# willake/cpu-ray-tracer

Hardware: AMD Instinct MI355X
Metric: Mrays/sec (primary+secondary), 1280x720 64spp path trace — pipelined throughput over 878 consecutive 64-spp windows of one progressive render (single_render = one such render alone) (higher is better)
Workload: dtype f32; 1 GPU; bunny_scene.xml FileScene BVH-SAH path tracer, 1280x720, 64 spp/step (passes=1, depthLimit=5); 1 step = 64 frames = the next spp window of a progressive render; the 878 steps are one crt_render job (14 render kernel launch(es), a wavefront per (tile, 128 consecutive frames), + ordered accumulate), one sync at the end; triangles=4968, parallelism=tile-wave x1

## Files before the change

### cpu-ray-tracer_amd/__init__.py

```python
import ctypes as C
import os
import subprocess

import numpy as np

HERE = os.path.dirname(os.path.abspath(__file__))
REPO = os.path.dirname(HERE)
LIB_PATH = os.environ.get("CRT_LIB_PATH") or os.path.join(HERE, "libcrt_amd.so")

SCENE_FILE, SCENE_TLAS = 0, 1
UPDATE_TRANSFORMS, UPDATE_BOUNDS = 1, 2
ACCEL_KDTREE, ACCEL_GRID = 1, 2
KD_NODE_DTYPE = np.dtype([("aabbMin", "<f4", 3), ("left", "<i4"), ("aabbMax", "<f4", 3), ("right", "<i4"), ("splitDistance", "<f4"), ("splitAxis", "<i4"),
                          ("firstTri", "<u4"), ("triCount", "<u4")])


class CrtError(RuntimeError):
    def __init__(self, code, msg):
        super().__init__("crt error %d: %s" % (code, msg))
        self.code = code


class Config(C.Structure):
    _fields_ = [("width", C.c_int32), ("height", C.c_int32), ("depthLimit", C.c_int32), ("device", C.c_int32),
# ... 428 lines not shown

    def sample_resident_lanes(self, accel=0):
        n = C.c_uint32()
        self._ck(self.L.crt_debug_sample_resident_lanes(self.h, int(accel), C.byref(n)))
        return int(n.value)

    def _positions(self, positions, what):
        import torch
        if not isinstance(positions, torch.Tensor) or positions.device != torch.device("cuda", self.device):
            raise ValueError("%s: positions must be a torch tensor on cuda:%d" % (what, self.device))
        if positions.dtype != torch.float32 or not positions.is_contiguous() or positions.dim() < 2 or tuple(positions.shape[1:]) not in ((3, 3), (9,)):
            raise ValueError("%s: positions must be a contiguous float32 tensor of shape [triCount, 3, 3] or [triCount, 9]" % what)
        return C.c_void_p(positions.data_ptr()), C.c_uint32(positions.shape[0])

    def refit_device(self, bvh, positions, stream=None, root_box=True):
        def run(st):
            ptr, n = self._positions(positions, "refit_device")
            box = (C.c_float * 6)()
            self._ck(self.L.crt_refit_device(self.h, C.c_uint32(bvh), ptr, n, C.c_void_p(st.cuda_stream), box if root_box else None))
            return np.array(box[:], np.float32).reshape(2, 3) if root_box else None
        return self._enqueue(stream, run)

    def _transforms(self, T, what):
        import torch
        if not isinstance(T, torch.Tensor) or T.device != torch.device("cuda", self.device):
            raise ValueError("%s: the transforms must be a torch tensor on cuda:%d" % (what, self.device))
        if T.dtype != torch.float32 or not T.is_contiguous() or T.dim() < 2 or tuple(T.shape[1:]) not in ((16,), (4, 4)):
            raise ValueError("%s: the transforms must be a contiguous float32 tensor of shape [N, 16] or [N, 4, 4]" % what)
        return C.c_void_p(T.data_ptr()), C.c_uint32(T.shape[0])

    def update_transforms_device(self, T, stream=None):
        def run(st):
            ptr, n = self._transforms(T, "update_transforms_device")
            nodes = np.zeros(2 * n.value, TLAS_DTYPE)
            self._ck(self.L.crt_update_transforms_device(self.h, ptr, n, C.c_void_p(st.cuda_stream), _p(nodes)))
            return nodes
        return self._enqueue(stream, run)

    def build_grid_device(self, bvh, positions, stream=None):
        def run(st):
            ptr, n = self._positions(positions, "build_grid_device")
            self._ck(self.L.crt_build_grid_device(self.h, C.c_uint32(bvh), ptr, n, C.c_void_p(st.cuda_stream)))
        return self._enqueue(stream, run)

    def get_grid(self, bvh=0):
        res = np.zeros(3, np.int32); f = np.zeros(9, np.float32); cells, refs = C.c_uint32(), C.c_uint32()
        fp = f.ctypes.data
        self._ck(self.L.crt_get_grid(self.h, C.c_uint32(bvh), _p(res), C.c_void_p(fp), C.c_void_p(fp + 12), C.c_void_p(fp + 24), C.byref(cells), C.byref(refs), None, None))
        start = np.zeros(cells.value + 1, np.uint32); r = np.zeros(max(refs.value, 1), np.int32)
        self._ck(self.L.crt_get_grid(self.h, C.c_uint32(bvh), None, None, None, None, None, None, _p(start), _p(r)))
        return dict(resolution=res, cellSize=f[0:3].copy(), boundsMin=f[3:6].copy(), boundsMax=f[6:9].copy(), cellStart=start, refs=r[:refs.value])

    def _enqueue(self, stream, run):
        import torch
        st = stream if stream is not None else torch.cuda.current_stream(self.device)
        if st.cuda_stream != 0:
            with torch.cuda.stream(st):
                return run(st)
        side = getattr(self, "_side_stream", None)
        if side is None:
            side = self._side_stream = torch.cuda.Stream(device=self.device)
        side.wait_stream(st)
        with torch.cuda.stream(side):
            out = run(side)
        st.wait_stream(side)
        for t in (out if isinstance(out, tuple) else (out,)):
            if isinstance(t, torch.Tensor):
                t.record_stream(st)
        return out

    def counters(self):
        c = CountersS()
        self._ck(self.L.crt_get_counters(self.h, C.byref(c)))
        return {n: int(getattr(c, n)) for n, _ in c._fields_}

    def reset_counters(self):
        self._ck(self.L.crt_reset_counters(self.h))

    def timing(self):
        t = TimingS()
        self._ck(self.L.crt_get_timing(self.h, C.byref(t)))
        return dict(render_kernel_ms=t.render_kernel_ms, resolve_kernel_ms=t.resolve_kernel_ms, render_launches=t.render_launches, pool_launches=t.pool_launches, split_launches=t.split_launches)

    def tile_clocks(self, tile_count):
        a = np.zeros((tile_count, 2), np.uint64)
        self._ck(self.L.crt_get_tile_clocks(self.h, _p(a)))
        return a

    def bind_accumulator(self, device_ptr):
        self._ck(self.L.crt_bind_accumulator(self.h, C.c_void_p(device_ptr)))

    def accumulator_device_ptr(self):
        p = C.c_void_p()
        self._ck(self.L.crt_accumulator_device_ptr(self.h, C.byref(p)))
        return p.value

def hit_fields(hits):
    import torch
    i = hits.view(torch.int32)
    return dict(t=hits[:, 0], u=hits[:, 1], v=hits[:, 2], objIdx=i[:, 3], triIdx=i[:, 4], traversed=i[:, 5], tested=i[:, 6])


def hit_info_fields(info):
    import torch
    return dict(I=info[:, 0:3], material=info.view(torch.int32)[:, 3], N=info[:, 4:7], u=info[:, 7], albedo=info[:, 8:11], v=info[:, 11])


class HostScene:

    def __init__(self, xml_path, kind, base_dir=None):
        self.L = lib()
        h = C.c_void_p()
        rc = self.L.crt_host_scene_load(xml_path.encode(), int(kind), (base_dir or "").encode(), C.byref(h))
        if rc != 0:
            raise CrtError(rc, self.L.crt_host_last_error().decode())
        self.h = h
        self.kind = int(kind)

    def close(self):
        if getattr(self, "h", None):
            self.L.crt_host_scene_free(self.h)
            self.h = None

    def __del__(self):
        try:
            self.close()
        except Exception:
            pass

    def _ck(self, rc):
        if rc != 0:
            raise CrtError(rc, self.L.crt_host_last_error().decode())

    def upload(self, ctx):
        self._ck(self.L.crt_host_scene_upload(self.h, ctx.h))

    def triangle_count(self):
        return self.L.crt_host_scene_triangle_count(self.h)

    def bvh_count(self):
        return self.L.crt_host_scene_bvh_count(self.h)

    def bvh(self, i=0):
        nu, tc, md = C.c_uint32(), C.c_uint32(), C.c_uint32()
        self._ck(self.L.crt_host_scene_bvh_info(self.h, i, C.byref(nu), C.byref(tc), C.byref(md)))
        nodes = np.zeros(nu.value, NODE_DTYPE)
        idx = np.zeros(tc.value, np.uint32)
        tris = np.zeros(tc.value, TRI_DTYPE)
        self._ck(self.L.crt_host_scene_bvh_copy(self.h, i, _p(nodes), _p(idx), _p(tris)))
        return dict(nodes=nodes, triIndices=idx, tris=tris, nodesUsed=nu.value, maxDepth=md.value)

    def move_and_refit(self, i, positions):
        positions = np.ascontiguousarray(positions, np.float32)
        self._ck(self.L.crt_host_scene_bvh_move_and_refit(self.h, int(i), _p(positions), C.c_uint32(positions.shape[0])))

    def refit_device(self, ctx, i, positions, stream=None):
        def run(st):
            ptr, n = ctx._positions(positions, "refit_device")
            self._ck(self.L.crt_host_scene_bvh_refit_device(self.h, ctx.h, int(i), ptr, n, C.c_void_p(st.cuda_stream)))
        return ctx._enqueue(stream, run)

    def set_transforms_device(self, ctx, T, stream=None):
        def run(st):
            ptr, n = ctx._transforms(T, "set_transforms_device")
            if n.value != self.bvh_count():
                raise ValueError("set_transforms_device: %d transforms for %d instances" % (n.value, self.bvh_count()))
# ... 174 lines not shown
        return self.L.crt_host_renderer_spp(self.h)

    @property
    def energy(self):
        return float(self.L.crt_host_renderer_energy(self.h))

    def accumulator(self):
        p = self.L.crt_host_renderer_accumulator(self.h)
        return np.ctypeslib.as_array(p, shape=(self.H, self.W, 4)).copy()

    def screen(self):
        p = self.L.crt_host_renderer_screen(self.h)
        return np.ctypeslib.as_array(p, shape=(self.H, self.W)).copy()

    def context(self):
        return Context.borrow(self.L.crt_host_renderer_ctx(self.h), self.W, self.H)


def load_obj(path):
    L = lib()
    n = C.c_uint32()
    pp, pn, pu = C.POINTER(C.c_float)(), C.POINTER(C.c_float)(), C.POINTER(C.c_float)()
    rc = L.crt_host_obj_load(path.encode(), C.byref(n), C.byref(pp), C.byref(pn), C.byref(pu))
    if rc != 0:
        raise CrtError(rc, L.crt_host_last_error().decode())
    pos = np.ctypeslib.as_array(pp, shape=(n.value, 3)).copy()
    nrm = np.ctypeslib.as_array(pn, shape=(n.value, 3)).copy()
    uv = np.ctypeslib.as_array(pu, shape=(n.value, 2)).copy()
    for q in (pp, pn, pu):
        L.crt_host_free(C.cast(q, C.c_void_p))
    return pos, nrm, uv


def load_image(path):
    L = lib()
    w, h = C.c_int(), C.c_int()
    px = C.POINTER(C.c_uint32)()
    rc = L.crt_host_image_load(path.encode(), C.byref(w), C.byref(h), C.byref(px))
    if rc != 0:
        raise CrtError(rc, L.crt_host_last_error().decode())
    a = np.ctypeslib.as_array(px, shape=(h.value, w.value)).copy()
    L.crt_host_free(C.cast(px, C.c_void_p))
    return a


def host_math_probe(inputs):
    inputs = np.ascontiguousarray(inputs, np.float32).reshape(-1, 12)
    out = np.zeros((len(inputs), 120), np.float32)
    lib().crt_host_math_probe(inputs.ctypes.data_as(C.c_void_p), C.c_uint32(len(inputs)), out.ctypes.data_as(C.c_void_p))
    return out


def host_grid_build(positions):
    pos = np.ascontiguousarray(positions, np.float32).reshape(-1, 9)
    L = lib()
    res = np.zeros(3, np.int32); f = np.zeros(9, np.float32); refs = C.c_uint32()

    def ck(rc):
        if rc != 0:
            raise CrtError(rc, L.crt_host_last_error().decode())
    ck(L.crt_host_grid_build(_p(pos), C.c_uint32(len(pos)), _p(res), _p(f), C.byref(refs), None, None))
    start = np.zeros(int(res.prod()) + 1, np.uint32); r = np.zeros(max(refs.value, 1), np.int32)
    ck(L.crt_host_grid_build(_p(pos), C.c_uint32(len(pos)), None, None, None, _p(start), _p(r)))
    return dict(resolution=res, cellSize=f[0:3].copy(), boundsMin=f[3:6].copy(), boundsMax=f[6:9].copy(), cellStart=start, refs=r[:refs.value])


def host_vertex_dedup(v8):
    v8 = np.ascontiguousarray(v8, np.float32).reshape(-1, 8)
    idx = np.zeros(len(v8), np.uint32); uniq = np.zeros((len(v8), 8), np.float32)
    L = lib(); L.crt_host_vertex_dedup.restype = C.c_uint32
    n = L.crt_host_vertex_dedup(v8.ctypes.data_as(C.c_void_p), C.c_uint32(len(v8)), idx.ctypes.data_as(C.c_void_p), uniq.ctypes.data_as(C.c_void_p))
    return idx, uniq[:n].copy()


def spp_window(rank, frames_per_rank, first_spp=1):
    return first_spp + rank * frames_per_rank


def tile_partition(rank, world, n_tiles):
    count = (n_tiles - rank + world - 1) // world if rank < n_tiles else 0
    return rank, world, count


def reduce_accumulator(tensor, dist, dst=0):
    dist.reduce(tensor, dst=dst, op=dist.ReduceOp.SUM)
    return tensor


def allreduce_accumulator(tensor, dist):
    dist.all_reduce(tensor, op=dist.ReduceOp.SUM)
    return tensor
```

### cpu-ray-tracer_amd/csrc/abi.cpp

```cpp
#include "../../include/crt_abi.h"
#include "device/launch.h"
#include "host/grid_resolution.h"

#include <cmath>
#include <cstdarg>
#include <cstddef>
#include <cstdio>
#include <cstdlib>
#include <cstring>
#include <deque>
#include <string>
#include <algorithm>
#include <vector>
#include <chrono>

static_assert(sizeof(crt_bvh_node) == 32 && sizeof(crt_tri) == 112 && sizeof(crt_tlas_node) == 32, "reference layouts");
static_assert(sizeof(crt::NodePair) == 64 && sizeof(crt::LeafTri) == 48 && sizeof(crt::ShadeTri) == 64 && sizeof(crt::TlasNode) == 32 &&
              sizeof(crt::Instance) == 128 && sizeof(crt::Material) == 32 && offsetof(crt::Instance, T) == 64, "device layouts");
static_assert(sizeof(crt_counters) == sizeof(crt::Counters), "counter layout");
static_assert(sizeof(crt_kd_node) == 48 && sizeof(crt::KdNode) == sizeof(crt_kd_node) && sizeof(crt::AltTri) == 48, "flat KD node (uploaded as it comes), alternative accelerators' triangle record");
static_assert(offsetof(crt::PrimDev, red) == 536 && sizeof(crt::PrimDev) == 552, "PrimDev: 134 floats, then the two texel pointers");
static_assert(sizeof(crt::BlasAltDesc) == 72, "BLAS descriptor");
static_assert(sizeof(crt_shadow_ray) == 28 && sizeof(crt_ray) == 28 && sizeof(crt_hit) == 28, "query records");
static_assert(sizeof(crt_hit_info) == 48 && offsetof(crt_hit_info, material) == 12 && offsetof(crt_hit_info, N) == 16 && offsetof(crt_hit_info, albedo) == 32 && offsetof(crt_hit_info, v) == 44, "crt_hit_info: three 16-byte pieces");
static_assert(sizeof(crt::Instance) == 128 && offsetof(crt::Instance, triCount) == 112, "Instance record");

namespace {

thread_local std::string g_createError;

bool g_hooks = false;
inline const char* hook(const char* name) { return g_hooks ? getenv(name) : nullptr; }

struct EventPair { hipEvent_t a, b; int mode = -1; bool seen = false; };

}

extern "C" uint32_t crt_debug_query_grid(void)
{
    const char* e = hook("CRT_DEBUG_QUERY_GRID");
    const long k = e ? strtol(e, nullptr, 10) : 0;
    return k > 0 ? (uint32_t)(k > 0x7fffffffL ? 0x7fffffffL : k) : 0u;
}

struct crt_ctx {
    crt_config cfg{};
    std::string err;
    hipStream_t stream = nullptr;
    int tilesX = 0, tilesY = 0;
    uint32_t tileFirst = 0, tileStride = 1, tileCount = 0;
    void* dAccOwned = nullptr; void* dAcc = nullptr;
    std::vector<hipStream_t> streams; uint64_t launchSeq = 0;
    struct Region { size_t off, bytes; hipEvent_t freed; bool held = false; };
    std::deque<Region> inflight;
    char* pool = nullptr; size_t poolBytes = 0, poolHead = 0; bool poolCapped = false;
    hipEvent_t mustWait = nullptr;
    std::vector<hipEvent_t> freeEvents;
    std::vector<hipEvent_t> doneEvents;
    struct Ahead { hipEvent_t end; size_t off; const char* slab; uint64_t epoch; uint32_t sppFirst, nf, passes, used; };
    std::deque<Ahead> ahead;
    uint64_t epoch = 1;
    uint64_t tickEpoch = 0; uint32_t tickNextSpp = 0, tickPasses = 0;
    uint32_t aheadFrames = 0;
    hipStream_t aheadStream = nullptr;
    crt::Scene hScene{};
    crt::Counters* dCounters = nullptr;
    uint32_t* dQueryCursor = nullptr;
    int32_t* dInspectCounts = nullptr; void* dInspectWork = nullptr; size_t inspectCap = 0;
    uint32_t* dPixels = nullptr; float* dTileSums = nullptr;
    unsigned long long* dTileClocks = nullptr;
    std::vector<void*> sceneAllocs;
    float meshLo[3] = {0, 0, 0}, meshHi[3] = {0, 0, 0}; bool orderDirty = true;
    uint32_t* dTileOrder = nullptr;
    uint32_t* hTileOrder[2] = {nullptr, nullptr}; hipEvent_t orderCopied[2] = {nullptr, nullptr}; hipEvent_t orderReady = nullptr; int orderFlip = 0;
    bool haveScene = false;
    struct Flat { int32_t kind = 0; uint64_t leafOff = 0, tlasOff = 0, tlasPairOff = 0, instOff = 0, shadeOff = 0; uint32_t tlasNodeCount = 0, maxHeight = 0;
                  uint32_t objects = 0;
                  std::vector<uint64_t> pairBase, triBase; std::vector<uint32_t> nodesUsed, triCount; std::vector<char> geom;
                  std::vector<float> rootBox; } flat;
    char* hStage[2] = {nullptr, nullptr}; size_t stageBytes[2] = {0, 0}; hipEvent_t stageCopied[2] = {nullptr, nullptr}; int stageFlip = 0;
    hipEvent_t sceneReady = nullptr, writeFence = nullptr;
    bool havePrim = false; crt::PrimDev prim{}; uint32_t* dPrimTex = nullptr;
    int renderAccel = 0;
    crt::AltAccelDev alt{}; bool haveKd = false, haveGrid = false; std::vector<void*> altAllocs[2]; crt::AltTri* altTris = nullptr; uint32_t altTriCount = 0;
    crt::TlasAltDev blasAlt[2]{}; bool haveBlas[2] = {false, false}; std::vector<void*> blasAllocs[2];
    bool hasAlt(int kind) const { return (kind == CRT_ACCEL_KDTREE && (haveKd || haveBlas[0])) || (kind == CRT_ACCEL_GRID && (haveGrid || haveBlas[1])); }
    char* dStage = nullptr; size_t stageCap = 0;
    static constexpr int kQuerySlots = 64;
    uint32_t* dQuerySlots = nullptr;
    struct QuerySlot { hipEvent_t done = nullptr; bool pending = false; } qslot[kQuerySlots];
    int qslotNext = 0;
    struct RefitPlan { void* dPlan = nullptr; uint32_t* dLevelOff = nullptr; uint32_t levels = 0, rootCode = 0; bool built = false; };
    std::vector<RefitPlan> refitPlans; std::vector<void*> refitAllocs;
    struct Refit {
        float* dBack = nullptr; float* hBack = nullptr; hipEvent_t done = nullptr;
        void release() { if (done) (void)hipEventDestroy(done); (void)hipFree(dBack); (void)hipHostFree(hBack); *this = Refit{}; }
    } refit;
    float* dRootBox = nullptr;
    struct TlasBuild {
        char* dBuild = nullptr; char* hBack = nullptr; size_t bytes = 0;
        hipEvent_t back = nullptr, done = nullptr, t0 = nullptr, t1 = nullptr; bool timed = false;
        void release() { for (hipEvent_t e : {back, done, t0, t1}) if (e) (void)hipEventDestroy(e); (void)hipFree(dBuild); (void)hipHostFree(hBack); *this = TlasBuild{}; }
    } tlasBuild;
    struct GridBuild {
        crt::GridBuildState* dState = nullptr; crt::GridBuildState* hState = nullptr;
        unsigned long long* dChunks = nullptr; uint32_t* dCursor = nullptr; int32_t* dUnsorted = nullptr; size_t cursorCap = 0, unsortedCap = 0;
        hipEvent_t back = nullptr, done = nullptr, t0 = nullptr, t1 = nullptr; bool built = false, timed = false; uint32_t blocks = 0;
        double waitMs[2] = {0, 0};
        void release() { for (hipEvent_t e : {back, done, t0, t1}) if (e) (void)hipEventDestroy(e); for (void* p : {(void*)dState, (void*)dChunks, (void*)dCursor, (void*)dUnsorted}) (void)hipFree(p); (void)hipHostFree(hState); *this = GridBuild{}; }
    } gridBuild;
    struct Retired { std::vector<void*> ptrs; void* pinned = nullptr; hipEvent_t unread = nullptr; };
    std::deque<Retired> retired; std::vector<hipEvent_t> retiredEvents;
    uint32_t gridRefCount = 0;
    struct BlasGrid { std::vector<crt::BlasAltDesc> desc; std::vector<uint32_t> cells, refs; std::vector<uint8_t> current; bool held = false; } blasGrid;
    hipEvent_t altReady = nullptr;
    static constexpr int kLatStages = 4;
    double tuneMs[kLatStages + 1] = {}; int tuneCount[kLatStages + 1] = {};
    hipEvent_t lastRenderEnd = nullptr;
    int latStage = 0;
    int latBest = 0;
    bool latDone = false;
    bool latConfirming = false; std::vector<int> latQueue;
    bool latWarm = false;
    uint32_t latSlots = 0;
    bool latProbed = false;
    std::vector<uint8_t> latL[kLatStages + 1];
    std::vector<uint32_t> latCost[kLatStages + 1];
    uint32_t* dTileCost = nullptr; uint32_t* hTileCost = nullptr; hipEvent_t costCopied = nullptr; bool costPending = false; int costStage = 0;
    uint32_t* dBlockDesc = nullptr; uint32_t* hBlockDesc = nullptr; uint32_t nBlocks = 0, descCap = 0; hipEvent_t descReady = nullptr;
    uint32_t* dJobCost = nullptr; uint32_t* hJobCost = nullptr; hipEvent_t jobCostCopied = nullptr; bool jobCostPending = false, jobCostValid = false;
    uint32_t recWaves = 0, recResident = 0, recWindows = 0; bool recPool = false;
    double poolWindowTicks = 0;
    std::vector<uint32_t> jobCost;
    std::vector<uint32_t> jobOrder;
    uint32_t* dJobDesc = nullptr; uint32_t* hJobDesc = nullptr; uint32_t jobDescCap = 0, jobBlocks = 0, jobHead = 0; hipEvent_t jobDescReady = nullptr;
    uint32_t planWindows = 0, planFrames = 0; bool planPool = false, planValid = false;
    double jobTrialMs[2] = {0, 0};
    uint32_t jobWaveOff = 0, jobWaveBlocks = 0, jobLongFrames = 0, jobLongWaves = 0, lastLongWaves = 0;
    std::vector<hipEvent_t> splitEvents;
    size_t splitSeq = 0; uint32_t splitLaunches = 0;
    uint64_t poolMinWaves = 65000;
    bool usePool = true;
    uint32_t ldsBytes = 0;
    std::vector<EventPair> evPool; size_t evUsedRender = 0, evUsedAcc = 0;
    std::deque<EventPair> evRender, evAcc;
    double foldedRenderMs = 0, foldedAccMs = 0; uint32_t foldedLaunches = 0, poolLaunches = 0;

    int fail(int code, const char* fmt, ...)
    {
        char buf[1024];
        va_list ap; va_start(ap, fmt); vsnprintf(buf, sizeof(buf), fmt, ap); va_end(ap);
        err = buf; return code;
    }
    int hip(hipError_t e, const char* what)
    {
        if (e == hipSuccess) return 0;
        return fail(CRT_ERR_DEVICE, "%s: %s", what, hipGetErrorString(e));
// ... 15 lines not shown
            for (void* p : r.ptrs) (void)hipFree(p);
            if (r.pinned) (void)hipHostFree(r.pinned);
            retiredEvents.push_back(r.unread); retired.pop_front();
        }
    }
    void freeScene()
    {
        for (void* p : sceneAllocs) (void)hipFree(p);
        sceneAllocs.clear(); haveScene = false; dRootBox = nullptr;
        for (void* p : refitAllocs) (void)hipFree(p);
        refitAllocs.clear(); refitPlans.clear();
        if (dPrimTex) { (void)hipFree(dPrimTex); dPrimTex = nullptr; }
        havePrim = false;
        freeAlt();
    }
};

#define HIPCK(ctx, call) do { hipError_t e_ = (call); if (e_ != hipSuccess) return (ctx)->hip(e_, #call); } while (0)

namespace {

template <class T>
int upload(crt_ctx* c, const std::vector<T>& v, const T** out)
{
    *out = nullptr;
    if (v.empty()) return 0;
    void* d = nullptr;
    HIPCK(c, hipMalloc(&d, v.size() * sizeof(T)));
    c->sceneAllocs.push_back(d);
    HIPCK(c, hipMemcpyAsync(d, v.data(), v.size() * sizeof(T), hipMemcpyHostToDevice, c->stream));
    HIPCK(c, hipStreamSynchronize(c->stream));
    *out = reinterpret_cast<const T*>(d);
    return 0;
}

template <class T>
int upload_array(crt_ctx* c, std::vector<void*>& allocs, const void* src, size_t bytes, const T** out)
{
    *out = nullptr; if (!bytes) return 0;
    void* d = nullptr; HIPCK(c, hipMalloc(&d, bytes)); allocs.push_back(d);
    HIPCK(c, hipMemcpy(d, src, bytes, hipMemcpyHostToDevice)); *out = static_cast<const T*>(d); return 0;
}

int bvh_height(crt_ctx* c, const crt_bvh& b, uint32_t* heightOut)
{
    std::vector<std::pair<uint32_t, uint32_t>> st; st.push_back({0u, 0u});
    uint32_t h = 0; size_t visited = 0;
    while (!st.empty()) {
        auto [n, d] = st.back(); st.pop_back();
        if (++visited > (size_t)b.nodesUsed) return c->fail(CRT_ERR_INVALID, "BVH node graph is not a tree");
        const crt_bvh_node& nd = b.nodes[n];
        if (nd.triCount > 0) { if (d > h) h = d; continue; }
        if (nd.leftFirst == 0 || nd.leftFirst + 1 >= b.nodesUsed) return c->fail(CRT_ERR_INVALID, "BVH child index out of range (node %u)", n);
        st.push_back({nd.leftFirst, d + 1}); st.push_back({nd.leftFirst + 1, d + 1});
    }
    *heightOut = h;
    return 0;
}

int wait_queries(crt_ctx* c)
{
    for (auto& q : c->qslot) if (q.pending) { HIPCK(c, hipEventSynchronize(q.done)); q.pending = false; }
    return 0;
}

hipError_t ensure_event(hipEvent_t* e, unsigned flags = hipEventDisableTiming) { return *e ? hipSuccess : hipEventCreateWithFlags(e, flags); }

int drain_all(crt_ctx* c)
{
    for (auto st : c->streams) HIPCK(c, hipStreamSynchronize(st));
    if (c->aheadStream) HIPCK(c, hipStreamSynchronize(c->aheadStream));
    HIPCK(c, hipStreamSynchronize(c->stream));
    return wait_queries(c);
}

}

extern "C" {

int crt_abi_version(void) { return CRT_ABI_VERSION; }

void crt_debug_enable_hooks(int on) { g_hooks = on != 0; }

int crt_device_count(void)
{
    int n = 0;
    if (hipGetDeviceCount(&n) != hipSuccess) return 0;
    return n;
}

const char* crt_last_error(crt_ctx* ctx) { return ctx ? ctx->err.c_str() : g_createError.c_str(); }

int crt_create(crt_ctx** out, const crt_config* cfg)
{
    if (!out || !cfg) { g_createError = "crt_create: null argument"; return CRT_ERR_INVALID; }
    *out = nullptr;
    setenv("GPU_MAX_HW_QUEUES", "16", 0);
    if (cfg->width < 16 || cfg->height < 16) { g_createError = "crt_create: width and height must be at least one 16x16 tile"; return CRT_ERR_INVALID; }
    int ndev = 0;
    hipError_t e = hipGetDeviceCount(&ndev);
    if (e != hipSuccess || ndev == 0) {
        g_createError = "crt_create: no HIP device visible (this library has no CPU path)";
        return CRT_ERR_NO_DEVICE;
    }
    if (cfg->device < 0 || cfg->device >= ndev) { g_createError = "crt_create: device ordinal out of range"; return CRT_ERR_INVALID; }
    crt_ctx* c = new crt_ctx();
    c->cfg = *cfg;
    if (const char* k = hook("CRT_RENDER_KERNEL")) {
        c->usePool = strcmp(k, "tiles") != 0;
        if (!strcmp(k, "pool_always")) c->poolMinWaves = 0;
    }
    if (c->cfg.depthLimit < 0) c->cfg.depthLimit = 5;
    if (c->cfg.depthLimit > 5) { g_createError = "crt_create: depthLimit > 5 unsupported (throughput stack holds 5 factors; reference default is 5)"; delete c; return CRT_ERR_UNSUPPORTED; }
    if (c->cfg.maxFramesPerLaunch <= 0) c->cfg.maxFramesPerLaunch = c->cfg.collectStats ? 64 : 4096;
    if (c->cfg.maxFramesPerLaunch > 64) c->cfg.maxFramesPerLaunch = c->cfg.maxFramesPerLaunch / 64 * 64;
    if (c->cfg.renderStreams < 0) c->cfg.renderStreams = 0;
    c->tilesX = cfg->width / 16; c->tilesY = cfg->height / 16;
    const int tiles = c->tilesX * c->tilesY;
    int first = cfg->tileFirst, stride = cfg->tileStride <= 0 ? 1 : cfg->tileStride, count = cfg->tileCount;
    if (count < 0) { first = 0; stride = 1; count = tiles; }
    if (first < 0 || (count > 0 && (long long)first + (long long)(count - 1) * stride >= tiles)) {
        g_createError = "crt_create: tile range exceeds the image"; delete c; return CRT_ERR_INVALID;
    }
    c->tileFirst = (uint32_t)first; c->tileStride = (uint32_t)stride; c->tileCount = (uint32_t)count;

    auto bail = [&](hipError_t he, const char* what) {
        g_createError = std::string("crt_create: ") + what + ": " + hipGetErrorString(he);
        crt_destroy(c); return CRT_ERR_DEVICE;
    };
    if ((e = hipSetDevice(cfg->device)) != hipSuccess) return bail(e, "hipSetDevice");
    if ((e = hipStreamCreateWithFlags(&c->stream, hipStreamNonBlocking)) != hipSuccess) return bail(e, "hipStreamCreate");
    const size_t px = (size_t)cfg->width * cfg->height;
    if ((e = hipMalloc(&c->dAccOwned, px * 16)) != hipSuccess) return bail(e, "hipMalloc(accumulator)");
    c->dAcc = c->dAccOwned;
    if ((e = hipMemsetAsync(c->dAcc, 0, px * 16, c->stream)) != hipSuccess) return bail(e, "hipMemset(accumulator)");
    if ((e = hipMalloc((void**)&c->dPixels, px * 4)) != hipSuccess) return bail(e, "hipMalloc(pixels)");
    if ((e = hipMemsetAsync(c->dPixels, 0, px * 4, c->stream)) != hipSuccess) return bail(e, "hipMemset(pixels)");
    if ((e = hipMalloc((void**)&c->dTileSums, (size_t)tiles * 4)) != hipSuccess) return bail(e, "hipMalloc(tileSums)");
    if ((e = hipMemsetAsync(c->dTileSums, 0, (size_t)tiles * 4, c->stream)) != hipSuccess) return bail(e, "hipMemset(tileSums)");
    if ((e = hipMalloc((void**)&c->dCounters, sizeof(crt::Counters))) != hipSuccess) return bail(e, "hipMalloc(counters)");
    if ((e = hipMemsetAsync(c->dCounters, 0, sizeof(crt::Counters), c->stream)) != hipSuccess) return bail(e, "hipMemset(counters)");
    if ((e = hipMalloc((void**)&c->dQueryCursor, 64)) != hipSuccess) return bail(e, "hipMalloc(query cursor)");
    if ((e = hipMalloc((void**)&c->dQuerySlots, crt_ctx::kQuerySlots * 64)) != hipSuccess) return bail(e, "hipMalloc(query cursor slots)");
    if (c->cfg.collectStats && count > 0) {
        if ((e = hipMalloc((void**)&c->dTileClocks, (size_t)count * 144)) != hipSuccess) return bail(e, "hipMalloc(tileClocks)");
        if ((e = hipMemsetAsync(c->dTileClocks, 0, (size_t)count * 144, c->stream)) != hipSuccess) return bail(e, "hipMemset(tileClocks)");
    }
    memset(&c->hScene, 0, sizeof(c->hScene));
    const float aspect = (float)cfg->width / (float)cfg->height;
    crt::Scene& s = c->hScene;
    s.camPos[0] = 0; s.camPos[1] = 0; s.camPos[2] = -2;
    s.topLeft[0] = -aspect; s.topLeft[1] = 1; s.topLeft[2] = 0;
    s.topRight[0] = aspect; s.topRight[1] = 1; s.topRight[2] = 0;
    s.bottomLeft[0] = -aspect; s.bottomLeft[1] = -1; s.bottomLeft[2] = 0;
    s.W = cfg->width; s.H = cfg->height; s.invW = 1.0f / cfg->width; s.invH = 1.0f / cfg->height;
    s.depthLimit = c->cfg.depthLimit;
    crt::set_primary(s);
    if ((e = hipStreamSynchronize(c->stream)) != hipSuccess) return bail(e, "hipStreamSynchronize");
    *out = c;
    return CRT_OK;
}

void crt_destroy(crt_ctx* c)
{
    if (!c) return;
    (void)hipSetDevice(c->cfg.device);
    for (auto st : c->streams) (void)hipStreamSynchronize(st);
    if (c->aheadStream) (void)hipStreamSynchronize(c->aheadStream);
    if (c->stream) (void)hipStreamSynchronize(c->stream);
    for (auto& q : c->qslot) if (q.done) { if (q.pending) (void)hipEventSynchronize(q.done); (void)hipEventDestroy(q.done); }
    if (c->dQuerySlots) (void)hipFree(c->dQuerySlots);
    if (c->altReady) (void)hipEventDestroy(c->altReady);
    if (c->writeFence) (void)hipEventDestroy(c->writeFence);
    c->refit.release(); c->tlasBuild.release();
    c->freeScene();
    c->gridBuild.release();
    for (hipEvent_t e : c->retiredEvents) (void)hipEventDestroy(e);
    for (auto& a : c->ahead) (void)hipEventDestroy(a.end);
    if (c->aheadStream) (void)hipStreamDestroy(c->aheadStream);
    for (auto& ev : c->evPool) { (void)hipEventDestroy(ev.a); (void)hipEventDestroy(ev.b); }
    for (auto& ev : c->evRender) { (void)hipEventDestroy(ev.a); (void)hipEventDestroy(ev.b); }
    for (auto& ev : c->evAcc) { (void)hipEventDestroy(ev.a); (void)hipEventDestroy(ev.b); }
    if (c->dAccOwned) (void)hipFree(c->dAccOwned);
    for (auto st : c->streams) { (void)hipStreamSynchronize(st); (void)hipStreamDestroy(st); }
    for (auto& r : c->inflight) (void)hipEventDestroy(r.freed);
    for (auto e : c->freeEvents) (void)hipEventDestroy(e);
    if (c->mustWait) (void)hipEventDestroy(c->mustWait);
    if (c->pool) (void)hipFree(c->pool);
    for (auto e : c->doneEvents) (void)hipEventDestroy(e);
    if (c->dPixels) (void)hipFree(c->dPixels);
    if (c->dTileSums) (void)hipFree(c->dTileSums);
    if (c->dCounters) (void)hipFree(c->dCounters);
    if (c->dQueryCursor) (void)hipFree(c->dQueryCursor);
    if (c->dInspectCounts) (void)hipFree(c->dInspectCounts);
    if (c->dInspectWork) (void)hipFree(c->dInspectWork);
    if (c->dTileClocks) (void)hipFree(c->dTileClocks);
    if (c->dTileOrder) (void)hipFree(c->dTileOrder);
    if (c->dTileCost) (void)hipFree(c->dTileCost);
    if (c->dJobCost) (void)hipFree(c->dJobCost);
    if (c->dJobDesc) (void)hipFree(c->dJobDesc);
    if (c->hJobDesc) (void)hipHostFree(c->hJobDesc);
    if (c->jobDescReady) (void)hipEventDestroy(c->jobDescReady);
    if (c->hJobCost) (void)hipHostFree(c->hJobCost);
    if (c->jobCostCopied) (void)hipEventDestroy(c->jobCostCopied);
    for (auto e : c->splitEvents) (void)hipEventDestroy(e);
    if (c->hTileCost) (void)hipHostFree(c->hTileCost);
    if (c->costCopied) (void)hipEventDestroy(c->costCopied);
    if (c->dBlockDesc) (void)hipFree(c->dBlockDesc);
    if (c->hBlockDesc) (void)hipHostFree(c->hBlockDesc);
    if (c->descReady) (void)hipEventDestroy(c->descReady);
    if (c->dStage) (void)hipFree(c->dStage);
    for (int k = 0; k < 2; k++) { if (c->hTileOrder[k]) (void)hipHostFree(c->hTileOrder[k]); if (c->orderCopied[k]) (void)hipEventDestroy(c->orderCopied[k]); }
    for (int k = 0; k < 2; k++) { if (c->hStage[k]) (void)hipHostFree(c->hStage[k]); if (c->stageCopied[k]) (void)hipEventDestroy(c->stageCopied[k]); }
    if (c->stream) (void)hipStreamDestroy(c->stream);
    delete c;
}

int crt_upload_scene(crt_ctx* c, const crt_scene_desc* sd)
{
    if (!c || !sd) return CRT_ERR_INVALID;
    c->epoch++;
    HIPCK(c, hipSetDevice(c->cfg.device));
    if (sd->kind != CRT_SCENE_FILE && sd->kind != CRT_SCENE_TLAS) return c->fail(CRT_ERR_INVALID, "unknown scene kind %d", sd->kind);
    if (!sd->bvhs || sd->bvhCount == 0) return c->fail(CRT_ERR_INVALID, "scene has no acceleration structure");
    if (sd->kind == CRT_SCENE_FILE && sd->bvhCount != 1) return c->fail(CRT_ERR_INVALID, "CRT_SCENE_FILE takes exactly one BVH (FileScene::acc)");
    if (sd->kind == CRT_SCENE_TLAS && (sd->bvhCount > 256 || !sd->tlasNodes || sd->tlasNodeCount < 2 * sd->bvhCount))
        return c->fail(CRT_ERR_INVALID, "TLAS scene needs <= 256 BLAS (tlas_bvh.cpp:21) and 2*blasCount TLAS nodes");
    if (sd->textureCount == 0 || !sd->textures) return c->fail(CRT_ERR_INVALID, "floor and skydome textures are required");
    if (sd->floorTexture < 0 || sd->floorTexture >= (int)sd->textureCount || sd->skyTexture < 0 || sd->skyTexture >= (int)sd->textureCount)
        return c->fail(CRT_ERR_INVALID, "floor/sky texture index out of range");
    for (uint32_t i = 0; i < sd->textureCount; i++)
        if (!sd->textures[i].pixels || sd->textures[i].width <= 0 || sd->textures[i].height <= 0) return c->fail(CRT_ERR_INVALID, "texture %u is empty", i);
    if (sd->materialCount > 0 && !sd->materials) return c->fail(CRT_ERR_INVALID, "materialCount is %u but materials is NULL", sd->materialCount);
    for (uint32_t i = 0; i < sd->materialCount; i++)
        if (sd->materials[i].texture >= (int)sd->textureCount) return c->fail(CRT_ERR_INVALID, "material %u: texture index out of range", i);
    if (sd->kind == CRT_SCENE_FILE) {
        if (!sd->objMatIdx || sd->objCount == 0) return c->fail(CRT_ERR_INVALID, "CRT_SCENE_FILE needs objMatIdx");
        for (uint32_t i = 0; i < sd->objCount; i++)
            if (sd->objMatIdx[i] < 0 || sd->objMatIdx[i] >= (int)sd->materialCount) return c->fail(CRT_ERR_INVALID, "objMatIdx entry out of range");
    }

    uint64_t nPairs = 0, nTris = 0;
    uint32_t maxHeight = 0;
    for (uint32_t bi = 0; bi < sd->bvhCount; bi++) {
        const crt_bvh& b = sd->bvhs[bi];
        if (!b.nodes || !b.triangles || !b.triangleIndices || b.nodesUsed == 0 || b.triCount == 0) return c->fail(CRT_ERR_INVALID, "BVH %u is empty", bi);
        if ((b.nodesUsed & 1u) == 0) return c->fail(CRT_ERR_INVALID, "BVH %u: nodesUsed must be odd (root + child pairs)", bi);
        if (sd->kind == CRT_SCENE_TLAS && (b.matIdx < 0 || b.matIdx >= (int)sd->materialCount)) return c->fail(CRT_ERR_INVALID, "BLAS %u: matIdx out of range", bi);
        if (sd->kind == CRT_SCENE_TLAS && b.objIdx != (int)bi + 2)
            return c->fail(CRT_ERR_INVALID, "BLAS %u: objIdx must be %u (TLASFileScene numbers objects from 2, tlas_file_scene.cpp:13,51-53)", bi, bi + 2);
        uint32_t h = 0; int r = bvh_height(c, b, &h); if (r) return r;
        if (h > maxHeight) maxHeight = h;
        nPairs += b.nodesUsed / 2; nTris += b.triCount;
    }
    const uint64_t pairBytes = nPairs ? nPairs * 64 : 64;
    const uint64_t leafOffB = pairBytes, leafBytes = (nTris + 1) * 48;
    const uint64_t tlasOffB = (leafOffB + leafBytes + 63) & ~63ull;
    const uint64_t tlasBytes = (sd->kind == CRT_SCENE_TLAS) ? (uint64_t)sd->tlasNodeCount * 32 : 0;
    const uint64_t tlasPairOffB = (tlasOffB + tlasBytes + 63) & ~63ull;
    const uint64_t tlasPairBytes = (sd->kind == CRT_SCENE_TLAS) ? (uint64_t)sd->tlasNodeCount * 32 : 0;
    const uint64_t instOffB = (tlasPairOffB + tlasPairBytes + 127) & ~127ull;
    const uint64_t instBytes = (sd->kind == CRT_SCENE_TLAS) ? (uint64_t)sd->bvhCount * 128 : 0;
    const uint64_t shadeOffB = (instOffB + instBytes + 63) & ~63ull;
    const uint64_t total = shadeOffB + nTris * 64;
    if (total >= crt::kMaxGeomBytes) return c->fail(CRT_ERR_UNSUPPORTED, "scene geometry needs %llu bytes; this build addresses 4 GiB", (unsigned long long)total);
    if (sd->kind == CRT_SCENE_TLAS && sd->tlasNodeCount > 0x7fffu) return c->fail(CRT_ERR_UNSUPPORTED, "TLAS node index exceeds 15 bits");

    std::vector<char> geom((size_t)total, 0);
    crt::NodePair* pairs = reinterpret_cast<crt::NodePair*>(geom.data());
    crt::LeafTri* leaf = reinterpret_cast<crt::LeafTri*>(geom.data() + leafOffB);
    crt::TlasNode* tlas = reinterpret_cast<crt::TlasNode*>(geom.data() + tlasOffB);
    crt::NodePair* tlasPairs = reinterpret_cast<crt::NodePair*>(geom.data() + tlasPairOffB);
    bool ref16ok = nPairs <= crt::kRef16MaxIndex && nTris < crt::kRef16MaxIndex;
    crt::Instance* inst = reinterpret_cast<crt::Instance*>(geom.data() + instOffB);
    crt::ShadeTri* shade = reinterpret_cast<crt::ShadeTri*>(geom.data() + shadeOffB);

    uint64_t pairBase = 0, triBase = 0; uint32_t rootRef0 = 0, rootRef0_16 = 0;
    for (uint32_t bi = 0; bi < sd->bvhCount; bi++) {
        const crt_bvh& b = sd->bvhs[bi];
        auto ref_of = [&](uint32_t n, uint32_t* ref) -> int {
            const crt_bvh_node& nd = b.nodes[n];
            if (nd.triCount > 0) {
                if ((uint64_t)nd.leftFirst + nd.triCount > b.triCount) return c->fail(CRT_ERR_INVALID, "leaf range out of bounds (BVH %u node %u)", bi, n);
                *ref = (uint32_t)((leafOffB + (triBase + nd.leftFirst) * 48) >> 4);
            } else {
                if ((nd.leftFirst & 1u) == 0) return c->fail(CRT_ERR_INVALID, "interior node %u: children must be allocated pairwise starting at an odd index", n);
                *ref = crt::kRefInterior | (uint32_t)(((pairBase + ((nd.leftFirst - 1u) >> 1)) * 64) >> 4);
            }
            return 0;
        };
        auto ref16_of = [&](uint32_t n) -> uint32_t {
            const crt_bvh_node& nd = b.nodes[n];
            if (nd.triCount > 0) return (uint32_t)((triBase + nd.leftFirst + 1) & crt::kRef16IndexMask);
            return crt::kRef16Interior | (uint32_t)((pairBase + ((nd.leftFirst - 1u) >> 1)) & crt::kRef16IndexMask);
        };
// ... 72 lines not shown
        }
        tlasRoot = tlas[0].ref; tlasRoot16 = tlas[0].ref16;
    }
    std::vector<uint32_t> texOff(sd->textureCount); uint64_t texels = 0;
    for (uint32_t i = 0; i < sd->textureCount; i++) {
        texOff[i] = (uint32_t)texels;
        texels += (uint64_t)sd->textures[i].width * sd->textures[i].height;
        if (texels > 0xffffffffull) return c->fail(CRT_ERR_UNSUPPORTED, "texture pool exceeds 2^32 texels");
    }
    auto bindTex = [&](crt::Material& m, int t) {
        if (t < 0) { m.texOffset = 0; m.texW = 0; m.texH = 0; }
        else { m.texOffset = texOff[t]; m.texW = sd->textures[t].width; m.texH = sd->textures[t].height; }
    };
    std::vector<crt::Material> mats(2 + sd->materialCount);
    memset(mats.data(), 0, mats.size() * sizeof(crt::Material));
    bindTex(mats[0], -1);
    bindTex(mats[1], sd->floorTexture);
    for (uint32_t i = 0; i < sd->materialCount; i++) {
        crt::Material& m = mats[2 + i];
        m.reflectivity = sd->materials[i].reflectivity; m.refractivity = sd->materials[i].refractivity;
        memcpy(m.absorption, sd->materials[i].absorption, 12);
        bindTex(m, sd->materials[i].texture);
    }

    { const int r = drain_all(c); if (r) return r; }
    c->freeScene();
    uint32_t* dTexels = nullptr;
    HIPCK(c, hipMalloc((void**)&dTexels, (size_t)texels * 4)); c->sceneAllocs.push_back(dTexels);
    for (uint32_t i = 0; i < sd->textureCount; i++)
        HIPCK(c, hipMemcpyAsync(dTexels + texOff[i], sd->textures[i].pixels, (size_t)sd->textures[i].width * sd->textures[i].height * 4, hipMemcpyHostToDevice, c->stream));
    HIPCK(c, hipStreamSynchronize(c->stream));

    crt::Scene& s = c->hScene;
    s.kind = sd->kind;
    memcpy(s.lightInvT, sd->lightInvT, 48);
    s.lightNrm[0] = -sd->lightT[1]; s.lightNrm[1] = -sd->lightT[5]; s.lightNrm[2] = -sd->lightT[9];
    s.lightSize = sd->lightSize;
    {
        const float* m = sd->lightT;
        const float ax = -0.5f, ay = 0.0f, az = -0.5f, bx = 0.5f, by = 0.0f, bz = 0.5f;
        const float c1[3] = {m[0] * ax + m[1] * ay + m[2] * az + m[3] * 1.0f, m[4] * ax + m[5] * ay + m[6] * az + m[7] * 1.0f, m[8] * ax + m[9] * ay + m[10] * az + m[11] * 1.0f};
        const float c2[3] = {m[0] * bx + m[1] * by + m[2] * bz + m[3] * 1.0f, m[4] * bx + m[5] * by + m[6] * bz + m[7] * 1.0f, m[8] * bx + m[9] * by + m[10] * bz + m[11] * 1.0f};
        s.lightPos[0] = (c1[0] + c2[0]) * 0.5f - 0.0f; s.lightPos[1] = (c1[1] + c2[1]) * 0.5f - 0.01f; s.lightPos[2] = (c1[2] + c2[2]) * 0.5f - 0.0f;
    }
    memcpy(s.floorN, sd->floorN, 12); s.floorD = sd->floorD; s.floorInvto = sd->floorInvto;
    {
        const float* m = sd->lightInvT;
        s.lightAxis = (m[0] == 1.0f && m[1] == 0.0f && m[2] == 0.0f && m[4] == 0.0f && m[5] == 1.0f && m[6] == 0.0f && m[8] == 0.0f && m[9] == 0.0f && m[10] == 1.0f) ? 1u : 0u;
        s.floorAxisY = (sd->floorN[0] == 0.0f && sd->floorN[1] == 1.0f && sd->floorN[2] == 0.0f) ? 1u : 0u;
        if (hook("CRT_DEBUG_GENERAL_PRIMS")) s.lightAxis = s.floorAxisY = 0u;
    }
    s.floorMat = mats[1];
    s.skyOffset = texOff[sd->skyTexture]; s.skyW = sd->textures[sd->skyTexture].width; s.skyH = sd->textures[sd->skyTexture].height;
    s.texels = dTexels;
    int r;
    const char* dGeom = nullptr;
    if ((r = upload(c, geom, &dGeom))) return r;
    s.geom = dGeom;
    s.tlasOff = (uint32_t)tlasOffB; s.instOff = (uint32_t)instOffB; s.shadeOff = (uint32_t)shadeOffB;
    s.leafOff = (uint32_t)leafOffB; s.tlasPairOff = (uint32_t)tlasPairOffB;
    s.rootRef16 = (sd->kind == CRT_SCENE_TLAS) ? tlasRoot16 : rootRef0_16;
    s.ref16ok = (ref16ok && !hook("CRT_DEBUG_NO_REF16")) ? 1u : 0u;
    if ((r = upload(c, mats, &s.mats))) return r;
    if (sd->kind == CRT_SCENE_TLAS) {
        std::vector<float> boxes;
        for (uint32_t bi = 0; bi < sd->bvhCount; bi++) { const crt_bvh_node& n0 = sd->bvhs[bi].nodes[0]; boxes.insert(boxes.end(), n0.aabbMin, n0.aabbMin + 3); boxes.insert(boxes.end(), n0.aabbMax, n0.aabbMax + 3); }
        const float* d = nullptr;
        if ((r = upload(c, boxes, &d))) return r;
        c->dRootBox = const_cast<float*>(d);
    }
    s.rootRef = (sd->kind == CRT_SCENE_TLAS) ? tlasRoot : rootRef0;
    s.bvhStack = maxHeight > 0 ? maxHeight : 1;
    s.rootIsPair = 0; memset(s.rootPair, 0, sizeof(s.rootPair));
    if (sd->kind == CRT_SCENE_TLAS) {
        if ((tlasRoot & 0xC0000000u) == crt::kRefTlasInterior) {
            memcpy(s.rootPair, &tlas[tlasRoot & 0x7fffu], 32); memcpy(s.rootPair + 8, &tlas[(tlasRoot >> 15) & 0x7fffu], 32);
            s.rootIsPair = 1;
        }
    } else if (rootRef0 & crt::kRefInterior) {
        memcpy(s.rootPair, geom.data() + ((size_t)(rootRef0 & crt::kRefOffsetMask) << 4), 64);
        s.rootIsPair = 1;
    }
    if (hook("CRT_DEBUG_NO_ROOTPAIR")) s.rootIsPair = 0;
    crt::set_primary(s);
    s.stackDepth = s.bvhStack + ((sd->kind == CRT_SCENE_TLAS) ? tlasHeight + 1 : 0);
    c->ldsBytes = s.stackDepth * 64u * 4u; c->latSlots = 0;
    if (const char* e = hook("CRT_DEBUG_EXTRA_LDS")) c->ldsBytes += (uint32_t)atoi(e);
    if (c->ldsBytes + 15u * 256u > 64u * 1024u) return c->fail(CRT_ERR_UNSUPPORTED, "tree height %u (+TLAS %u) needs %u bytes of LDS traversal stack per wave (> 64 KiB)", maxHeight, tlasHeight, c->ldsBytes);
    {
        float lo[3] = {1e30f, 1e30f, 1e30f}, hi[3] = {-1e30f, -1e30f, -1e30f};
        auto grow = [&](const float* mn, const float* mx) { for (int k = 0; k < 3; k++) { if (mn[k] < lo[k]) lo[k] = mn[k]; if (mx[k] > hi[k]) hi[k] = mx[k]; } };
        if (sd->kind == CRT_SCENE_TLAS) grow(sd->tlasNodes[0].aabbMin, sd->tlasNodes[0].aabbMax);
        else grow(sd->bvhs[0].nodes[0].aabbMin, sd->bvhs[0].nodes[0].aabbMax);
        memcpy(c->meshLo, lo, 12); memcpy(c->meshHi, hi, 12); c->orderDirty = true;
    }
    {
        crt_ctx::Flat& f = c->flat;
        f.kind = sd->kind; f.leafOff = leafOffB; f.tlasOff = tlasOffB; f.tlasPairOff = tlasPairOffB; f.instOff = instOffB; f.shadeOff = shadeOffB;
        f.tlasNodeCount = (sd->kind == CRT_SCENE_TLAS) ? sd->tlasNodeCount : 0; f.maxHeight = maxHeight;
        f.objects = (sd->kind == CRT_SCENE_TLAS) ? sd->bvhCount : sd->objCount;
        f.pairBase.clear(); f.triBase.clear(); f.nodesUsed.clear(); f.triCount.clear(); f.rootBox.clear();
        for (uint32_t bi = 0; bi < sd->bvhCount; bi++) { const crt_bvh_node& r = sd->bvhs[bi].nodes[0]; f.rootBox.insert(f.rootBox.end(), r.aabbMin, r.aabbMin + 3); f.rootBox.insert(f.rootBox.end(), r.aabbMax, r.aabbMax + 3); }
        uint64_t pb = 0, tb = 0;
        for (uint32_t bi = 0; bi < sd->bvhCount; bi++) { f.pairBase.push_back(pb); f.triBase.push_back(tb); f.nodesUsed.push_back(sd->bvhs[bi].nodesUsed); f.triCount.push_back(sd->bvhs[bi].triCount); pb += sd->bvhs[bi].nodesUsed / 2; tb += sd->bvhs[bi].triCount; }
        f.geom.swap(geom);
    }
    c->haveScene = true;
    return CRT_OK;
}


static int order_behind_ahead(crt_ctx* c)
{
    for (const auto& a : c->ahead) HIPCK(c, hipStreamWaitEvent(c->stream, a.end, 0));
    return 0;
}

static int order_behind_queries(crt_ctx* c)
{
    for (auto& q : c->qslot) {
        if (!q.pending) continue;
        const hipError_t e = hipEventQuery(q.done);
        if (e == hipSuccess) { q.pending = false; continue; }
        if (e != hipErrorNotReady) return c->hip(e, "hipEventQuery(query)");
        HIPCK(c, hipStreamWaitEvent(c->stream, q.done, 0));
    }
    return 0;
}

static int wait_scene(crt_ctx* c, hipStream_t st)
{
    if (c->sceneReady) HIPCK(c, hipStreamWaitEvent(st, c->sceneReady, 0));
    return 0;
}

static int order_behind_readers(crt_ctx* c)
{
    int r;
    if ((r = order_behind_ahead(c)) || (r = order_behind_queries(c))) return r;
    c->epoch++;
    return 0;
}

static int begin_scene_write(crt_ctx* c, hipStream_t st)
{
    const int r = order_behind_readers(c);
    if (r || st == c->stream) return r;
    HIPCK(c, ensure_event(&c->writeFence));
    HIPCK(c, hipEventRecord(c->writeFence, c->stream));
    HIPCK(c, hipStreamWaitEvent(st, c->writeFence, 0));
    return wait_scene(c, st);
}

static int publish_scene_write(crt_ctx* c, hipStream_t st, hipEvent_t done)
{
    c->sceneReady = done;
    if (st != c->stream) HIPCK(c, hipStreamWaitEvent(c->stream, done, 0));
    return 0;
}

static int end_scene_write(crt_ctx* c, hipStream_t st, hipEvent_t done)
{
    HIPCK(c, hipEventRecord(done, st));
    return publish_scene_write(c, st, done);
}

static int flatten_tlas(crt_ctx* c, const crt_tlas_node* nodes, uint32_t count, uint32_t bvhCount, crt::TlasNode* tlas, crt::NodePair* tlasPairs, uint32_t* heightOut)
{
    uint32_t nTlasPairs = 0;
    for (uint32_t i = 0; i < count; i++) {
        const crt_tlas_node& nd = nodes[i];
        memcpy(tlas[i].lo, nd.aabbMin, 12); memcpy(tlas[i].hi, nd.aabbMax, 12);
        tlas[i].ref = nd.leftRight ? (crt::kRefTlasInterior | (nd.leftRight & 0x7fffu) | (((nd.leftRight >> 16) & 0x7fffu) << 15))
                                   : (crt::kRefTlasLeaf | (nd.BLAS & 0xffffu));
        tlas[i].ref16 = nd.leftRight ? (crt::kRef16TlasBit | nTlasPairs++) : (crt::kRef16TlasLeaf | (nd.BLAS & crt::kRef16IndexMask));
    }
    std::vector<std::pair<uint32_t, uint32_t>> st; st.push_back({0u, 0u}); size_t visited = 0; uint32_t height = 0;
    while (!st.empty()) {
        auto [n, d] = st.back(); st.pop_back();
        if (++visited > (size_t)count) return c->fail(CRT_ERR_INVALID, "TLAS node graph is not a tree");
        const crt_tlas_node& nd = nodes[n];
        if (nd.leftRight == 0) { if (nd.BLAS >= bvhCount) return c->fail(CRT_ERR_INVALID, "TLAS leaf references BLAS %u", nd.BLAS); if (d > height) height = d; continue; }
        const uint32_t l = nd.leftRight & 0xffffu, r = nd.leftRight >> 16;
        if (l >= count || r >= count) return c->fail(CRT_ERR_INVALID, "TLAS child index out of range");
        st.push_back({l, d + 1}); st.push_back({r, d + 1});
    }
    for (uint32_t i = 0; i < count; i++) {
        const crt_tlas_node& nd = nodes[i];
        if (nd.leftRight == 0) continue;
        crt::NodePair& p = tlasPairs[tlas[i].ref16 & crt::kRef16IndexMask];
        memcpy(&p.c[0], &tlas[nd.leftRight & 0xffffu], 32); memcpy(&p.c[1], &tlas[nd.leftRight >> 16], 32);
    }
    *heightOut = height;
    return 0;
}

static void set_root(crt_ctx* c, int kind, const float* lo, const float* hi)
{
    crt::Scene& s = c->hScene; const crt_ctx::Flat& f = c->flat;
    s.rootIsPair = 0; memset(s.rootPair, 0, sizeof(s.rootPair));
    if (kind == CRT_SCENE_TLAS) {
        const crt::TlasNode* tlas = reinterpret_cast<const crt::TlasNode*>(f.geom.data() + f.tlasOff);
        const uint32_t root = tlas[0].ref;
        s.rootRef = root; s.rootRef16 = tlas[0].ref16;
        if ((root & 0xC0000000u) == crt::kRefTlasInterior) { memcpy(s.rootPair, &tlas[root & 0x7fffu], 32); memcpy(s.rootPair + 8, &tlas[(root >> 15) & 0x7fffu], 32); s.rootIsPair = 1; }
    } else if (s.rootRef & crt::kRefInterior) {
        memcpy(s.rootPair, f.geom.data() + ((size_t)(s.rootRef & crt::kRefOffsetMask) << 4), 64);
        s.rootIsPair = 1;
    }
    if (hook("CRT_DEBUG_NO_ROOTPAIR")) s.rootIsPair = 0;
    crt::set_primary(s);
    memcpy(c->meshLo, lo, 12); memcpy(c->meshHi, hi, 12); c->orderDirty = true;
}

static int check_tlas_height(crt_ctx* c, uint32_t tlasHeight)
{
    if ((c->hScene.bvhStack + tlasHeight + 1) * 64u * 4u + 15u * 256u > 64u * 1024u)
        return c->fail(CRT_ERR_UNSUPPORTED, "TLAS height %u needs %u bytes of LDS traversal stack per wave (> 64 KiB)", tlasHeight, (c->hScene.bvhStack + tlasHeight + 1) * 256u);
    return 0;
}

static void adopt_tlas(crt_ctx* c, uint32_t tlasHeight, const float* lo, const float* hi)
{
    crt::Scene& s = c->hScene;
    s.stackDepth = s.bvhStack + tlasHeight + 1;
    c->ldsBytes = s.stackDepth * 64u * 4u; c->latSlots = 0;
    set_root(c, CRT_SCENE_TLAS, lo, hi);
}

static void drop_blas_sets(crt_ctx* c)
{
    for (int k = 0; k < 2; k++) if (c->haveBlas[k]) { c->haveBlas[k] = false; if (c->renderAccel == k + 1) c->renderAccel = 0; }
}

int crt_update_scene(crt_ctx* c, const crt_scene_desc* sd, uint32_t what)
{
    if (!c || !sd) return CRT_ERR_INVALID;
    if (!c->haveScene) return c->fail(CRT_ERR_STATE, "crt_update_scene before crt_upload_scene");
    crt_ctx::Flat& f = c->flat;
    if (sd->kind != f.kind || sd->bvhCount != f.nodesUsed.size() || !sd->bvhs) return c->fail(CRT_ERR_INVALID, "crt_update_scene: scene kind / BVH count differ from the uploaded scene");
    if ((what & ~(uint32_t)(CRT_UPDATE_TRANSFORMS | CRT_UPDATE_BOUNDS)) || what == 0) return c->fail(CRT_ERR_INVALID, "crt_update_scene: unknown update flags");
    if ((what & CRT_UPDATE_TRANSFORMS) && f.kind != CRT_SCENE_TLAS) return c->fail(CRT_ERR_INVALID, "CRT_UPDATE_TRANSFORMS applies to two-level scenes (a FileScene bakes its transforms into the triangles)");
    HIPCK(c, hipSetDevice(c->cfg.device));
    for (uint32_t bi = 0; bi < sd->bvhCount; bi++)
        if (sd->bvhs[bi].nodesUsed != f.nodesUsed[bi] || sd->bvhs[bi].triCount != f.triCount[bi] || !sd->bvhs[bi].nodes || !sd->bvhs[bi].triangles || !sd->bvhs[bi].triangleIndices)
            return c->fail(CRT_ERR_INVALID, "crt_update_scene: BVH %u changed its topology (node / triangle count); upload the scene again", bi);
    if (f.kind == CRT_SCENE_TLAS && (!sd->tlasNodes || sd->tlasNodeCount != f.tlasNodeCount))
        return c->fail(CRT_ERR_INVALID, "crt_update_scene: a two-level scene needs the node array of the TLASBVH::Build that followed the change (tlasNodes, %u nodes as uploaded)", f.tlasNodeCount);
    if (what & CRT_UPDATE_BOUNDS) {
        const crt::LeafTri* leaf = reinterpret_cast<const crt::LeafTri*>(f.geom.data() + f.leafOff);
        for (uint32_t bi = 0; bi < sd->bvhCount; bi++) {
            const crt_bvh& b = sd->bvhs[bi];
            for (uint32_t j = 0; j < b.triCount; j++) {
                const uint32_t ti = b.triangleIndices[j];
                if (ti >= b.triCount) return c->fail(CRT_ERR_INVALID, "BVH %u: triangleIndices[%u] out of range", bi, j);
                if (leaf[f.triBase[bi] + j].shadeIdx != (uint32_t)(f.triBase[bi] + ti)) return c->fail(CRT_ERR_INVALID, "BVH %u: triangleIndices changed; Refit keeps the leaf order — upload the scene again", bi);
            }
        }
    }
    uint32_t tlasHeight = 0;
    std::vector<char> tlasImage;
    if (f.kind == CRT_SCENE_TLAS) {
        tlasImage.assign((size_t)(f.instOff - f.tlasOff), 0);
        int r = flatten_tlas(c, sd->tlasNodes, sd->tlasNodeCount, sd->bvhCount, reinterpret_cast<crt::TlasNode*>(tlasImage.data()),
                             reinterpret_cast<crt::NodePair*>(tlasImage.data() + (f.tlasPairOff - f.tlasOff)), &tlasHeight);
        if (r || (r = check_tlas_height(c, tlasHeight))) return r;
    }
    size_t lo = SIZE_MAX, hi = 0;
    auto touch = [&](size_t a, size_t b) { if (a < lo) lo = a; if (b > hi) hi = b; };
    if (what & CRT_UPDATE_BOUNDS) {
        crt::NodePair* pairs = reinterpret_cast<crt::NodePair*>(f.geom.data());
        crt::LeafTri* leaf = reinterpret_cast<crt::LeafTri*>(f.geom.data() + f.leafOff);
        for (uint32_t bi = 0; bi < sd->bvhCount; bi++) {
            const crt_bvh& b = sd->bvhs[bi];
            for (uint32_t n = 1; n + 1 < b.nodesUsed; n += 2) {
                crt::NodePair& p = pairs[f.pairBase[bi] + ((n - 1) >> 1)];
                for (int k = 0; k < 2; k++) { memcpy(p.c[k].lo, b.nodes[n + k].aabbMin, 12); memcpy(p.c[k].hi, b.nodes[n + k].aabbMax, 12); }
            }
            for (uint32_t j = 0; j < b.triCount; j++) {
                const crt_tri& t = b.triangles[b.triangleIndices[j]];
                crt::LeafTri& lt = leaf[f.triBase[bi] + j];
                for (int k = 0; k < 3; k++) { lt.v0[k] = t.vertex0[k]; lt.e1[k] = t.vertex1[k] - t.vertex0[k]; lt.e2[k] = t.vertex2[k] - t.vertex0[k]; }
            }
        }
        touch(0, (size_t)f.tlasOff);
        for (uint32_t bi = 0; bi < sd->bvhCount; bi++) { memcpy(&f.rootBox[6 * bi], sd->bvhs[bi].nodes[0].aabbMin, 12); memcpy(&f.rootBox[6 * bi + 3], sd->bvhs[bi].nodes[0].aabbMax, 12); }
    }
    if (f.kind == CRT_SCENE_TLAS) {
        if (what & CRT_UPDATE_TRANSFORMS) {
            crt::Instance* inst = reinterpret_cast<crt::Instance*>(f.geom.data() + f.instOff);
            for (uint32_t bi = 0; bi < sd->bvhCount; bi++) { memcpy(inst[bi].invT, sd->bvhs[bi].invT, 48); memcpy(inst[bi].T, sd->bvhs[bi].T, 48); }
        }
        memcpy(f.geom.data() + f.tlasOff, tlasImage.data(), tlasImage.size());
        touch((size_t)f.tlasOff, (size_t)f.shadeOff);
    }
    if (lo >= hi) return CRT_OK;
    const int k = c->stageFlip ^= 1;
    const size_t boxBytes = ((what & CRT_UPDATE_BOUNDS) && c->dRootBox) ? f.rootBox.size() * 4u : 0u;
    const size_t geomBytes = hi - lo, bytes = geomBytes + boxBytes;
    if (c->stageBytes[k] < bytes) {
        if (c->hStage[k]) { HIPCK(c, hipEventSynchronize(c->stageCopied[k])); HIPCK(c, hipHostFree(c->hStage[k])); c->hStage[k] = nullptr; }
        HIPCK(c, hipHostMalloc((void**)&c->hStage[k], bytes, hipHostMallocDefault)); c->stageBytes[k] = bytes;
        HIPCK(c, ensure_event(&c->stageCopied[k]));
    } else HIPCK(c, hipEventSynchronize(c->stageCopied[k]));
    memcpy(c->hStage[k], f.geom.data() + lo, geomBytes);
    if (boxBytes) memcpy(c->hStage[k] + geomBytes, f.rootBox.data(), boxBytes);
    { const int r = begin_scene_write(c, c->stream); if (r) return r; }
    if (what & CRT_UPDATE_BOUNDS) {
        std::fill(c->blasGrid.current.begin(), c->blasGrid.current.end(), (uint8_t)0);
        drop_blas_sets(c);
    }
    HIPCK(c, hipMemcpyAsync(const_cast<char*>(c->hScene.geom) + lo, c->hStage[k], geomBytes, hipMemcpyHostToDevice, c->stream));
    if (boxBytes) HIPCK(c, hipMemcpyAsync(c->dRootBox, c->hStage[k] + geomBytes, boxBytes, hipMemcpyHostToDevice, c->stream));
    { const int r = end_scene_write(c, c->stream, c->stageCopied[k]); if (r) return r; }
    if (f.kind == CRT_SCENE_TLAS) adopt_tlas(c, tlasHeight, sd->tlasNodes[0].aabbMin, sd->tlasNodes[0].aabbMax);
    else set_root(c, f.kind, sd->bvhs[0].nodes[0].aabbMin, sd->bvhs[0].nodes[0].aabbMax);
    return CRT_OK;
}

int crt_set_camera(crt_ctx* c, const float camPos[3], const float tl[3], const float tr[3], const float bl[3])
{
    if (!c || !camPos || !tl || !tr || !bl) return CRT_ERR_INVALID;
    HIPCK(c, hipSetDevice(c->cfg.device));
    crt::Scene& s = c->hScene;
    if (!memcmp(s.camPos, camPos, 12) && !memcmp(s.topLeft, tl, 12) && !memcmp(s.topRight, tr, 12) && !memcmp(s.bottomLeft, bl, 12)) return CRT_OK;
    memcpy(s.camPos, camPos, 12); memcpy(s.topLeft, tl, 12); memcpy(s.topRight, tr, 12); memcpy(s.bottomLeft, bl, 12);
    crt::set_primary(s);
    c->orderDirty = true; c->epoch++;
    return CRT_OK;
}

static int upload_tile_order(crt_ctx* c, const std::vector<uint32_t>& order)
{
    if (!c->dTileOrder) HIPCK(c, hipMalloc((void**)&c->dTileOrder, (size_t)c->tileCount * 4));
    { const int r = order_behind_ahead(c); if (r) return r; }
    const int k = c->orderFlip ^= 1;
    if (!c->hTileOrder[k]) {
        HIPCK(c, hipHostMalloc((void**)&c->hTileOrder[k], (size_t)c->tileCount * 4, hipHostMallocDefault));
        HIPCK(c, ensure_event(&c->orderCopied[k]));
    } else HIPCK(c, hipEventSynchronize(c->orderCopied[k]));
    memcpy(c->hTileOrder[k], order.data(), order.size() * 4);
    HIPCK(c, hipMemcpyAsync(c->dTileOrder, c->hTileOrder[k], order.size() * 4, hipMemcpyHostToDevice, c->stream));
    HIPCK(c, hipEventRecord(c->orderCopied[k], c->stream));
    c->orderReady = c->orderCopied[k];
    return 0;
}

static int update_tile_order(crt_ctx* c)
{
    if (!c->orderDirty || c->tileCount == 0) return 0;
    const crt::Scene& s = c->hScene;
    double R[3], Dn[3], N[3];
    for (int k = 0; k < 3; k++) { R[k] = (double)s.topRight[k] - s.topLeft[k]; Dn[k] = (double)s.bottomLeft[k] - s.topLeft[k]; }
    N[0] = R[1] * Dn[2] - R[2] * Dn[1]; N[1] = R[2] * Dn[0] - R[0] * Dn[2]; N[2] = R[0] * Dn[1] - R[1] * Dn[0];
    const double rr = R[0] * R[0] + R[1] * R[1] + R[2] * R[2], dd = Dn[0] * Dn[0] + Dn[1] * Dn[1] + Dn[2] * Dn[2];
    double E[3]; for (int k = 0; k < 3; k++) E[k] = (double)s.topLeft[k] - s.camPos[k];
    const double num = E[0] * N[0] + E[1] * N[1] + E[2] * N[2];
    auto rect_of = [&](const float* P8, int r[4]) -> bool {
        double u0 = 1e30, u1 = -1e30, v0 = 1e30, v1 = -1e30;
        for (int i = 0; i < 8; i++) {
            const float* P = P8 + 3 * i;
            double d[3] = {P[0] - s.camPos[0], P[1] - s.camPos[1], P[2] - s.camPos[2]};
            const double den = d[0] * N[0] + d[1] * N[1] + d[2] * N[2];
            const double t = den != 0 ? num / den : -1;
            if (!(t > 0) || rr == 0 || dd == 0) return false;
            double Q[3]; for (int k = 0; k < 3; k++) Q[k] = s.camPos[k] + t * d[k] - s.topLeft[k];
            const double u = (Q[0] * R[0] + Q[1] * R[1] + Q[2] * R[2]) / rr, v = (Q[0] * Dn[0] + Q[1] * Dn[1] + Q[2] * Dn[2]) / dd;
            if (u < u0) u0 = u; if (u > u1) u1 = u; if (v < v0) v0 = v; if (v > v1) v1 = v;
        }
        r[0] = (int)floor(u0 * c->cfg.width / 16.0) - 1; r[1] = (int)floor(u1 * c->cfg.width / 16.0) + 1;
        r[2] = (int)floor(v0 * c->cfg.height / 16.0) - 1; r[3] = (int)floor(v1 * c->cfg.height / 16.0) + 1;
        return true;
    };
    float world[24];
    for (int i = 0; i < 8; i++) { world[3 * i] = (i & 1) ? c->meshHi[0] : c->meshLo[0]; world[3 * i + 1] = (i & 2) ? c->meshHi[1] : c->meshLo[1]; world[3 * i + 2] = (i & 4) ? c->meshHi[2] : c->meshLo[2]; }
    int wr[4] = {0, c->tilesX - 1, 0, c->tilesY - 1};
    (void)rect_of(world, wr);
    std::vector<uint32_t> first, second, rest;
    for (uint32_t i = 0; i < c->tileCount; i++) {
        const uint32_t tile = c->tileFirst + i * c->tileStride;
        const int tx = (int)(tile % (uint32_t)c->tilesX), ty = (int)(tile / (uint32_t)c->tilesX);
        const bool inRect = tx >= wr[0] && tx <= wr[1] && ty >= wr[2] && ty <= wr[3];
        if (inRect) first.push_back(i); else rest.push_back(i);
    }
    for (int k = 0; k <= crt_ctx::kLatStages; k++) { c->tuneCount[k] = 0; c->tuneMs[k] = 0; }
    c->latStage = 0; c->latBest = 0; c->latDone = false; c->latWarm = false; c->latConfirming = false; c->latQueue.clear(); c->costPending = false; c->latProbed = false;
    first.insert(first.end(), rest.begin(), rest.end());
    c->jobCostValid = false; c->jobCostPending = false; c->planValid = false;
    { const int r = upload_tile_order(c, first); if (r) return r; }
    c->orderDirty = false;
    return 0;
}

static size_t sample_bytes_per_window(const crt_ctx* c, uint32_t passes) { return (size_t)c->tileCount * 256u * 64u * passes * 16u; }
static size_t window_bytes(const crt_ctx* c, uint32_t passes) { return sample_bytes_per_window(c, passes) + (c->usePool ? crt_pool_scratch_bytes_per_window(c->tileCount) : 0); }

static uint32_t block_desc(uint32_t tile, uint32_t laneBase, uint32_t lanes, uint32_t window) { uint32_t lg = 0; while ((1u << lg) < lanes) lg++; return tile | (laneBase << 16) | (lg << 22) | (window << 25); }
static const uint32_t kLatLanes[7] = {64u, 32u, 16u, 8u, 4u, 2u, 1u};
static const double kLatG[7] = {1.0, 0.93, 0.88, 0.79, 0.69, 0.57, 0.48};
static int lat_index(uint32_t L) { int k = 0; while (k < 6 && kLatLanes[k] != L) k++; return k; }

static uint8_t next_lanes(uint8_t lanes, uint32_t cost, double T)
{
    int k = lat_index(lanes); const double unit = (double)cost / kLatG[k];
    while (k < 6 && unit * kLatG[k] > T) k++;
    while (k > 0 && unit * kLatG[k - 1] <= 0.9 * T) k--;
    return (uint8_t)kLatLanes[k];
}
extern "C" int crt_debug_next_lanes(const uint8_t* lanes, const uint32_t* cost, uint32_t n, double T, uint8_t* out)
{
    if (!lanes || !cost || !out) return CRT_ERR_INVALID;
    for (uint32_t i = 0; i < n; i++) { if (lanes[i] == 0 || lanes[i] > 64 || (64 % lanes[i]) != 0) return CRT_ERR_INVALID; out[i] = next_lanes(lanes[i], cost[i], T); }
    return CRT_OK;
}

static double solve_block_table(const std::vector<uint8_t>& lanes, const std::vector<uint32_t>& cost, double budget, std::vector<uint8_t>& out)
{
    const size_t n = cost.size();
    double topUnit = 0; for (size_t i = 0; i < n; i++) topUnit = std::max(topUnit, (double)cost[i] / kLatG[lat_index(lanes[i])]);
    out.assign(n, 64);
    if (topUnit <= 0) return 0;
    auto waves = [&](double T) { double w = 0; for (size_t i = 0; i < n; i++) w += 64.0 / next_lanes(lanes[i], cost[i], T); return w; };
    double lo = kLatG[6] * topUnit, hi = topUnit;
    if (waves(lo) > budget) { for (int it = 0; it < 14; it++) { const double mid = 0.5 * (lo + hi); if (waves(mid) <= budget) hi = mid; else lo = mid; } lo = hi; }
    for (size_t i = 0; i < n; i++) out[i] = next_lanes(lanes[i], cost[i], lo);
    return lo;
}
extern "C" int crt_debug_solve_block_table(const uint8_t* lanes, const uint32_t* cost, uint32_t n, double budget, uint8_t* out, double* T)
{
    if (!lanes || !cost || !out) return CRT_ERR_INVALID;
    for (uint32_t i = 0; i < n; i++) if (lanes[i] == 0 || lanes[i] > 64 || (64 % lanes[i]) != 0) return CRT_ERR_INVALID;
    std::vector<uint8_t> L; const double t = solve_block_table(std::vector<uint8_t>(lanes, lanes + n), std::vector<uint32_t>(cost, cost + n), budget, L);
    if (n) memcpy(out, L.data(), n);
    if (T) *T = t;
    return CRT_OK;
}
static double lat_budget(crt_ctx* c)
{
    if (!c->latSlots) c->latSlots = crt_render_resident_waves(c->cfg.device, c->hScene.kind, c->ldsBytes);
    double share = 0.98;
    if (const char* e = hook("CRT_LAT_BUDGET")) { const double v = atof(e); if (v > 0) share = v; }
    return share * (double)c->latSlots;
}

static int upload_block_table(crt_ctx* c, const std::vector<uint8_t>& lanes, const std::vector<uint32_t>& cost)
{
    const uint32_t n = c->tileCount;
    std::vector<uint32_t> order(n);
    for (uint32_t i = 0; i < n; i++) order[i] = i;
    std::stable_sort(order.begin(), order.end(), [&](uint32_t a, uint32_t b) { return cost[a] > cost[b]; });
    std::vector<uint32_t> table; table.reserve((size_t)n * 2);
    for (uint32_t r = 0; r < n; r++) {
        const uint32_t tl = order[r], L = lanes[tl];
        for (uint32_t base = 0; base < 64u; base += L) table.push_back(block_desc(tl, base, L, 0u));
    }
    if (table.size() > 0x7fffffffull) return c->fail(CRT_ERR_INVALID, "block table too large");
    if (hook("CRT_LAT_VERBOSE")) fprintf(stderr, "[crt] latency table: %zu wavefronts for %u tiles (slowest tile of the base stage %.2f ms)\n", table.size(), n, n ? cost[order[0]] * 1e-5 : 0.0);
    if (c->descCap < table.size()) {
        if (c->dBlockDesc) (void)hipFree(c->dBlockDesc);
        if (c->hBlockDesc) (void)hipHostFree(c->hBlockDesc);
        c->dBlockDesc = nullptr; c->hBlockDesc = nullptr; c->descCap = 0;
        const size_t cap = table.size() + table.size() / 2;
        HIPCK(c, hipMalloc((void**)&c->dBlockDesc, cap * 4));
        HIPCK(c, hipHostMalloc((void**)&c->hBlockDesc, cap * 4, hipHostMallocDefault));
        c->descCap = (uint32_t)cap;
    } else if (c->descReady) HIPCK(c, hipEventSynchronize(c->descReady));
    HIPCK(c, ensure_event(&c->descReady));
    memcpy(c->hBlockDesc, table.data(), table.size() * 4);
    { const int r = order_behind_ahead(c); if (r) return r; }
    HIPCK(c, hipMemcpyAsync(c->dBlockDesc, c->hBlockDesc, table.size() * 4, hipMemcpyHostToDevice, c->stream));
    HIPCK(c, hipEventRecord(c->descReady, c->stream));
    c->nBlocks = (uint32_t)table.size();
    return 0;
// ... 392 lines not shown
        c->evRender.back().mode = c->latDone ? -1 : stage;
        if (L.wantCost && !c->latDone) c->costStage = stage;
    }
    if (L.wantCost) {
        if (!c->dTileCost) {
            HIPCK(c, hipMalloc((void**)&c->dTileCost, (size_t)c->tileCount * 4));
            HIPCK(c, hipHostMalloc((void**)&c->hTileCost, (size_t)c->tileCount * 4, hipHostMallocDefault));
            HIPCK(c, ensure_event(&c->costCopied));
        }
        else HIPCK(c, hipStreamWaitEvent(L.st, c->costCopied, 0));
        HIPCK(c, hipMemsetAsync(c->dTileCost, 0, (size_t)c->tileCount * 4, L.st));
    }
    return 0;
}

static int planner_prepare(crt_ctx* c, Launch& L)
{
    int r;
    if (L.nf > 64u && !c->cfg.collectStats) {
        if (c->jobCostPending && hipEventQuery(c->jobCostCopied) == hipSuccess) { c->jobCostPending = false; if ((r = adopt_job_costs(c))) return r; HIPCK(c, hipStreamWaitEvent(L.st, c->orderReady, 0)); }
        L.wantJobCost = !c->jobCostValid && !c->jobCostPending && L.nf >= 128u;
        if (L.wantJobCost) {
            if (!c->dJobCost) {
                HIPCK(c, hipMalloc((void**)&c->dJobCost, job_cost_bytes(c)));
                HIPCK(c, hipHostMalloc((void**)&c->hJobCost, job_cost_bytes(c), hipHostMallocDefault));
                HIPCK(c, ensure_event(&c->jobCostCopied));
            } else HIPCK(c, hipStreamWaitEvent(L.st, c->jobCostCopied, 0));
            HIPCK(c, hipMemsetAsync(c->dJobCost, 0, job_cost_bytes(c), L.st));
        }
    }
    const uint64_t minWaves = c->poolMinWaves != 65000u ? c->poolMinWaves : (c->jobCostValid ? 43000u : 65000u);
    L.pool = c->usePool && c->hScene.ref16ok && (uint64_t)c->tileCount * L.windows >= minWaves && (c->poolMinWaves == 0 || L.nf > 64u);
    if (L.nf > 64u && c->jobCostValid) {
        if ((r = install_job_plan(c, L.windows, L.nf, L.pool))) return r;
        int use = 1;
        if ((c->jobBlocks || c->jobLongWaves) && !hook("CRT_PLAN_NO_TRIAL")) {
            if (c->jobTrialMs[1] > 0 && c->jobTrialMs[0] > 0) use = c->jobTrialMs[1] <= c->jobTrialMs[0] ? 1 : 0;
            else if (c->jobTrialMs[1] > 0 && c->jobTrialMs[0] == 0) use = 0;
            c->evRender.back().mode = 100 + use;
        }
        if (use) { L.head = c->jobHead; L.jobBlocks = c->jobBlocks; if (L.pool && c->jobLongWaves) { L.waveTab = c->dJobDesc + c->jobWaveOff; L.waveBlocks = c->jobWaveBlocks; L.longFrames = c->jobLongFrames; L.longWaves = c->jobLongWaves; } }
    }
    if (L.pool) if (const uint32_t S = crt_pool_streams(L.nf); const uint32_t n = forced_wave_frames(S)) {
        L.waveFrames = n; L.waveTab = nullptr; L.waveBlocks = 0;
        L.longWaves = n > S ? (c->tileCount - L.head) * (L.nf / n + ((L.nf % n) > S ? 1u : 0u)) : 0u;
    }
    if (L.jobBlocks || L.waveTab) HIPCK(c, hipStreamWaitEvent(L.st, c->jobDescReady, 0));
    if (L.wantJobCost) {
        L.jobClk = reinterpret_cast<unsigned long long*>(reinterpret_cast<char*>(c->dJobCost) + job_cost_clk_offset(c));
        c->recPool = L.pool; c->recWindows = L.windows;
        const uint32_t perWave = L.pool ? std::max(crt_pool_streams(L.nf), L.waveFrames) : 64u;
        c->recWaves = L.pool ? c->tileCount * ((L.nf + perWave - 1u) / perWave) : c->tileCount * L.windows;
        c->recResident = L.pool ? 4096u : 5120u;
    }
    return 0;
}

static hipError_t launch_render_kernels(crt_ctx* c, const Launch& L)
{
    hipStream_t st = L.st;
    hipError_t le = hipSuccess;
    auto join = [&](hipStream_t other) -> hipError_t {
        if (other == st) return hipSuccess;
        hipError_t e = hipSuccess;
        if (c->splitEvents.size() < 32) { hipEvent_t ne; e = hipEventCreateWithFlags(&ne, hipEventDisableTiming); if (e == hipSuccess) c->splitEvents.push_back(ne); }
        if (e == hipSuccess) { hipEvent_t je = c->splitEvents[c->splitSeq++ % c->splitEvents.size()]; e = hipEventRecord(je, other); if (e == hipSuccess) e = hipStreamWaitEvent(st, je, 0); }
        return e;
    };
    auto launch_table = [&](const uint32_t* desc, uint32_t nBlocks, uint32_t* cost) -> hipError_t {
        return crt_launch_render(&c->hScene, L.slab, c->dCounters, c->dTileClocks, c->dTileOrder, c->tileFirst, c->tileStride, c->tileCount, (uint32_t)c->tilesX,
                                 L.sppFirst, L.nf, L.passes, c->ldsBytes, 0, desc, nBlocks, cost, 0u, nullptr, st);
    };
    if (L.pool) {
        void* scratch = (char*)L.slab + (size_t)L.windows * sample_bytes_per_window(c, L.passes);
        hipStream_t st2 = st;
        if (L.jobBlocks) {
            le = launch_table(c->dJobDesc, L.jobBlocks, nullptr);
            st2 = c->streams[(size_t)(c->launchSeq++ % c->streams.size())];
            if (le == hipSuccess && st2 != st) le = hipStreamWaitEvent(st2, L.ev.a, 0);
        }
        if (le == hipSuccess)
            le = crt_launch_render_pool(&c->hScene, L.slab, scratch, c->dCounters, c->dTileClocks, c->dTileOrder, c->tileFirst, c->tileStride, c->tileCount, (uint32_t)c->tilesX,
                                        L.sppFirst, L.nf, L.passes, c->cfg.collectStats, L.jobBlocks ? L.head : 0u, L.waveFrames, L.waveTab, L.waveBlocks, L.longFrames,
                                        L.wantJobCost ? c->dJobCost : nullptr, L.jobClk, st2);
        if (le == hipSuccess) c->lastLongWaves = L.longWaves;
        if (L.jobBlocks && le == hipSuccess) le = join(st2);
    } else if (L.jobBlocks) {
        le = launch_table(c->dJobDesc, L.jobBlocks, nullptr);
    } else if (L.blockDesc && L.nBlocks) {
        le = launch_table(L.blockDesc, L.nBlocks, L.wantCost ? c->dTileCost : nullptr);
    } else {
        le = crt_launch_render(&c->hScene, L.slab, c->dCounters, c->dTileClocks, c->dTileOrder, c->tileFirst, c->tileStride, c->tileCount, (uint32_t)c->tilesX,
                               L.sppFirst, L.nf, L.passes, c->ldsBytes, c->cfg.collectStats, nullptr, 0u,
                               L.wantCost ? c->dTileCost : (L.wantJobCost ? c->dJobCost : nullptr), 0u, L.jobClk, st);
    }
    if (L.jobBlocks && le == hipSuccess) c->splitLaunches++;
    return le;
}

static int probe_tile_costs(crt_ctx* c, hipStream_t st)
{
    const uint32_t n = c->tileCount;
    if (!c->dTileCost) {
        HIPCK(c, hipMalloc((void**)&c->dTileCost, (size_t)n * 4));
        HIPCK(c, hipHostMalloc((void**)&c->hTileCost, (size_t)n * 4, hipHostMallocDefault));
        HIPCK(c, ensure_event(&c->costCopied));
    } else HIPCK(c, hipEventSynchronize(c->costCopied));
    const auto tp0 = std::chrono::steady_clock::now();
    HIPCK(c, crt_launch_probe(&c->hScene, c->tileFirst, c->tileStride, n, (uint32_t)c->tilesX, c->dTileCost, st));
    HIPCK(c, hipMemcpyAsync(c->hTileCost, c->dTileCost, (size_t)n * 4, hipMemcpyDeviceToHost, st));
    HIPCK(c, hipEventRecord(c->costCopied, st));
    HIPCK(c, hipStreamSynchronize(st));
    const auto tp1 = std::chrono::steady_clock::now();
    std::vector<uint32_t>& est = c->latCost[0]; est.assign(c->hTileCost, c->hTileCost + n);
    for (uint32_t i = 0; i < n; i++) est[i] += 18u * crt_probe_paths();
    std::vector<uint8_t>& L = c->latL[0]; L.assign(n, 64);
    solve_block_table(std::vector<uint8_t>(n, 64), est, lat_budget(c), L);
    c->latProbed = true;
    bool any = false; for (uint32_t i = 0; i < n; i++) any = any || L[i] != 64;
    if (!any) { c->latProbed = false; return 0; }
    const auto tp2 = std::chrono::steady_clock::now();
    const int r = upload_block_table(c, L, est);
    if (hook("CRT_LAT_VERBOSE")) { const auto tp3 = std::chrono::steady_clock::now(); auto ms = [](auto a, auto b) { return std::chrono::duration<double, std::milli>(b - a).count(); };
        fprintf(stderr, "[crt] cost probe: launch + wait %.3f ms, table solved in %.3f ms, uploaded in %.3f ms\n", ms(tp0, tp1), ms(tp1, tp2), ms(tp2, tp3)); }
    return r;
}

static int launch_frames(crt_ctx* c, uint32_t sppFirst, uint32_t nf, uint32_t passes, hipStream_t st, crt_ctx::Ahead* ahead)
{
    const size_t windowBytes = window_bytes(c, passes);
    size_t off = 0; int r;
    if ((r = take_region(c, (size_t)((nf + 63u) / 64u) * windowBytes, st, &off))) return r;
    if (c->orderReady) HIPCK(c, hipStreamWaitEvent(st, c->orderReady, 0));
    if ((r = wait_scene(c, st))) return r;
    void* slab = c->pool + off;
    EventPair ev;
    harvest_tuning(c);
    fold_completed(c, c->evRender, &c->foldedRenderMs, &c->foldedLaunches); fold_completed(c, c->evAcc, &c->foldedAccMs, nullptr);
    if ((r = take_event(c, c->evRender, &ev))) return r;
    struct PairGuard { crt_ctx* c; bool armed; ~PairGuard() { if (armed && !c->evRender.empty()) { c->evPool.push_back(c->evRender.back()); c->evRender.pop_back(); } } } pairGuard{c, true};
    Launch L; L.st = st; L.ev = ev; L.slab = slab; L.sppFirst = sppFirst; L.nf = nf; L.passes = passes; L.windows = (nf + 63u) / 64u;
    if ((r = tuner_prepare(c, L))) return r;
    if ((r = planner_prepare(c, L))) return r;
    HIPCK(c, hipEventRecord(ev.a, st));
    const bool pool = L.pool, wantCost = L.wantCost, wantJobCost = L.wantJobCost;
    const hipError_t le = hook("CRT_DEBUG_FAIL_LAUNCH") ? hipErrorInvalidConfiguration  : launch_render_kernels(c, L);
    if (le != hipSuccess) {
        return c->hip(le, pool ? "launch of render_pool_kernel" : "launch of render_tiles_kernel");
    }
    if (pool) c->poolLaunches++;
    HIPCK(c, hipEventRecord(ev.b, st));
    pairGuard.armed = false;
    c->lastRenderEnd = ev.b;
    if (wantJobCost) {
        HIPCK(c, hipMemcpyAsync(c->hJobCost, c->dJobCost, job_cost_bytes(c), hipMemcpyDeviceToHost, st));
        HIPCK(c, hipEventRecord(c->jobCostCopied, st));
        c->jobCostPending = true;
    }
    if (wantCost && !pool && !c->latDone) {
        HIPCK(c, hipMemcpyAsync(c->hTileCost, c->dTileCost, (size_t)c->tileCount * 4, hipMemcpyDeviceToHost, st));
        HIPCK(c, hipEventRecord(c->costCopied, st));
        c->costPending = true;
    }
    crt_ctx::Region reg; reg.off = off; reg.bytes = (size_t)((nf + 63u) / 64u) * windowBytes;
    if (c->freeEvents.empty()) HIPCK(c, hipEventCreateWithFlags(&reg.freed, hipEventDisableTiming));
    else { reg.freed = c->freeEvents.back(); c->freeEvents.pop_back(); }
    if (ahead) {
        hipEvent_t end = nullptr;
        if (c->doneEvents.empty()) { const hipError_t e = hipEventCreateWithFlags(&end, hipEventDisableTiming); if (e != hipSuccess) { c->freeEvents.push_back(reg.freed); return c->hip(e, "hipEventCreate"); } }
        else { end = c->doneEvents.back(); c->doneEvents.pop_back(); }
        const hipError_t e = hipEventRecord(end, st);
        if (e != hipSuccess) { c->doneEvents.push_back(end); c->freeEvents.push_back(reg.freed); return c->hip(e, "hipEventRecord"); }
        reg.held = true;
        c->inflight.push_back(reg);
        *ahead = crt_ctx::Ahead{end, off, (const char*)slab, c->epoch, sppFirst, nf, passes, 0u};
        return 0;
    }
    HIPCK(c, hipStreamWaitEvent(c->stream, ev.b, 0));
    if ((r = take_event(c, c->evAcc, &ev))) return r;
    HIPCK(c, hipEventRecord(ev.a, c->stream));
    HIPCK(c, crt_launch_accumulate(slab, c->dAcc, c->tileFirst, c->tileStride, c->tileCount, (uint32_t)c->tilesX, (uint32_t)c->cfg.width, nf, passes, c->stream));
    HIPCK(c, hipEventRecord(ev.b, c->stream));
    HIPCK(c, hipEventRecord(reg.freed, c->stream));
    c->inflight.push_back(reg);
    return 0;
}

int crt_render(crt_ctx* c, uint32_t spp_first, uint32_t frames, uint32_t passes)
{
    if (!c) return CRT_ERR_INVALID;
    if (!c->haveScene && !c->havePrim) return c->fail(CRT_ERR_STATE, "crt_render before crt_upload_scene");
    if (passes < 1 || passes > 4) return c->fail(CRT_ERR_INVALID, "passes must be 1..4 (the reference's UI range, renderer.cpp:178)");
    HIPCK(c, hipSetDevice(c->cfg.device));
    { int r = discard_ahead(c); if (r) return r; }
    if (c->tileCount == 0 || frames == 0) return CRT_OK;
    { int r = update_tile_order(c); if (r) return r; }
    if (c->streams.empty()) {
        int n = c->cfg.renderStreams;
        if (n <= 0) n = 7;
        if (n > 16) n = 16;
        if (c->cfg.collectStats) n = 1;
        c->streams.resize((size_t)n);
        for (auto& st : c->streams) HIPCK(c, hipStreamCreateWithFlags(&st, hipStreamNonBlocking));
    }
    uint32_t maxF = 0;
    { int r = ensure_pool(c, frames, passes, &maxF); if (r) return r; }
    const size_t windowBytes = window_bytes(c, passes);
    if (c->renderAccel != 0 || c->havePrim) {
        for (uint32_t f0 = 0; f0 < frames; f0 += maxF) {
            const uint32_t nf = (frames - f0 < maxF) ? frames - f0 : maxF;
            size_t off = 0; int r;
            if ((r = take_region(c, (size_t)((nf + 63u) / 64u) * windowBytes, c->stream, &off))) return r;
            if ((r = wait_scene(c, c->stream))) return r;
            void* slab = c->pool + off;
            if (c->havePrim) HIPCK(c, crt_launch_render_prim(&c->hScene, &c->prim, slab, c->dCounters, c->tileFirst, c->tileStride, c->tileCount, (uint32_t)c->tilesX, spp_first + f0 * passes, nf, passes, c->stream));
            else HIPCK(c, crt_launch_render_alt(c->renderAccel, &c->hScene, &c->alt, &c->blasAlt[c->renderAccel - 1], slab, c->dCounters, c->tileFirst, c->tileStride, c->tileCount, (uint32_t)c->tilesX, spp_first + f0 * passes, nf, passes, c->stream));
            HIPCK(c, crt_launch_accumulate(slab, c->dAcc, c->tileFirst, c->tileStride, c->tileCount, (uint32_t)c->tilesX, (uint32_t)c->cfg.width, nf, passes, c->stream));
            crt_ctx::Region reg; reg.off = off; reg.bytes = (size_t)((nf + 63u) / 64u) * windowBytes;
            if (c->freeEvents.empty()) HIPCK(c, hipEventCreateWithFlags(&reg.freed, hipEventDisableTiming));
            else { reg.freed = c->freeEvents.back(); c->freeEvents.pop_back(); }
            HIPCK(c, hipEventRecord(reg.freed, c->stream));
            c->inflight.push_back(reg);
        }
        return CRT_OK;
    }
    for (uint32_t f0 = 0; f0 < frames; f0 += maxF) {
        const uint32_t nf = (frames - f0 < maxF) ? frames - f0 : maxF;
        const int r = launch_frames(c, spp_first + f0 * passes, nf, passes, c->streams[(size_t)(c->launchSeq++ % c->streams.size())], nullptr);
        if (r) return r > 0 ? c->fail(CRT_ERR_DEVICE, "slab ring blocked by a render-ahead region") : r;
    }
    return CRT_OK;
}

int crt_sync(crt_ctx* c)
{
    if (!c) return CRT_ERR_INVALID;
    HIPCK(c, hipSetDevice(c->cfg.device));
    HIPCK(c, hipStreamSynchronize(c->stream));
    for (auto st : c->streams) HIPCK(c, hipStreamSynchronize(st));
    if (c->aheadStream) HIPCK(c, hipStreamSynchronize(c->aheadStream));
    return CRT_OK;
}

int crt_clear(crt_ctx* c)
{
    if (!c) return CRT_ERR_INVALID;
    HIPCK(c, hipSetDevice(c->cfg.device));
    HIPCK(c, hipMemsetAsync(c->dAcc, 0, (size_t)c->cfg.width * c->cfg.height * 16, c->stream));
    return CRT_OK;
}

int crt_read_accumulator(crt_ctx* c, float* host)
{
    if (!c || !host) return CRT_ERR_INVALID;
    HIPCK(c, hipSetDevice(c->cfg.device));
    HIPCK(c, hipMemcpyAsync(host, c->dAcc, (size_t)c->cfg.width * c->cfg.height * 16, hipMemcpyDeviceToHost, c->stream));
    HIPCK(c, hipStreamSynchronize(c->stream));
    return CRT_OK;
}

static int read_screen(crt_ctx* c, uint32_t* hostPixels, float* energy)
{
    const int tiles = c->tilesX * c->tilesY;
    if (hostPixels) HIPCK(c, hipMemcpyAsync(hostPixels, c->dPixels, (size_t)c->cfg.width * c->cfg.height * 4, hipMemcpyDeviceToHost, c->stream));
    std::vector<float> sums(tiles);
    HIPCK(c, hipMemcpyAsync(sums.data(), c->dTileSums, (size_t)tiles * 4, hipMemcpyDeviceToHost, c->stream));
    HIPCK(c, hipStreamSynchronize(c->stream));
    if (energy) { float e = 0; for (int i = 0; i < tiles; i++) e += sums[i]; *energy = e; }
    return CRT_OK;
}

int crt_resolve_screen(crt_ctx* c, float scale, uint32_t* hostPixels, float* energy)
{
    if (!c) return CRT_ERR_INVALID;
    HIPCK(c, hipSetDevice(c->cfg.device));
    HIPCK(c, crt_launch_resolve(c->dAcc, c->dPixels, c->dTileSums, c->tileFirst, c->tileStride, c->tileCount, (uint32_t)c->tilesX, (uint32_t)c->cfg.width, scale, c->stream));
    return read_screen(c, hostPixels, energy);
}

// ... 991 lines not shown
    for (auto st : c->streams) HIPCK(c, hipStreamSynchronize(st));
    if (c->aheadStream) HIPCK(c, hipStreamSynchronize(c->aheadStream));
    harvest_tuning(c);
    memset(out, 0, sizeof(*out));
    out->render_kernel_ms = (float)c->foldedRenderMs; out->resolve_kernel_ms = (float)c->foldedAccMs;
    for (auto& ev : c->evRender) { float ms = 0; HIPCK(c, hipEventElapsedTime(&ms, ev.a, ev.b)); out->render_kernel_ms += ms; }
    for (auto& ev : c->evAcc) { float ms = 0; HIPCK(c, hipEventElapsedTime(&ms, ev.a, ev.b)); out->resolve_kernel_ms += ms; }
    out->render_launches = (uint32_t)c->evRender.size() + c->foldedLaunches;
    out->pool_launches = c->poolLaunches; out->split_launches = c->splitLaunches;
    c->foldedRenderMs = c->foldedAccMs = 0; c->foldedLaunches = 0; c->poolLaunches = 0; c->splitLaunches = 0;
    for (auto& ev : c->evRender) c->evPool.push_back(ev);
    for (auto& ev : c->evAcc) c->evPool.push_back(ev);
    c->evRender.clear(); c->evAcc.clear();
    return CRT_OK;
}

int crt_get_tile_clocks(crt_ctx* c, uint64_t* out)
{
    if (!c || !out) return CRT_ERR_INVALID;
    if (!c->dTileClocks) return c->fail(CRT_ERR_STATE, "tile clocks are recorded only by a collectStats context");
    HIPCK(c, hipSetDevice(c->cfg.device));
    HIPCK(c, hipMemcpyAsync(out, c->dTileClocks, (size_t)c->tileCount * 16, hipMemcpyDeviceToHost, c->stream));
    HIPCK(c, hipStreamSynchronize(c->stream));
    return CRT_OK;
}

extern "C" int crt_debug_live_events(crt_ctx* c) { return c ? (int)(2 * (c->evRender.size() + c->evAcc.size() + c->evPool.size())) : -1; }

extern "C" int crt_debug_check_reciprocals(crt_ctx* c, uint64_t* out)
{
    if (!c || !out) return CRT_ERR_INVALID;
    HIPCK(c, hipSetDevice(c->cfg.device));
    unsigned long long* d = nullptr;
    HIPCK(c, hipMalloc(&d, 32));
    hipError_t e = hipMemsetAsync(d, 0, 32, c->stream);
    if (e == hipSuccess) e = crt_launch_check_reciprocals(d, c->stream);
    if (e == hipSuccess) e = hipMemcpyAsync(out, d, 32, hipMemcpyDeviceToHost, c->stream);
    if (e == hipSuccess) e = hipStreamSynchronize(c->stream);
    (void)hipFree(d);
    HIPCK(c, e);
    return CRT_OK;
}

extern "C" int crt_debug_check_sqrt(crt_ctx* c, uint64_t* out)
{
    if (!c || !out) return CRT_ERR_INVALID;
    HIPCK(c, hipSetDevice(c->cfg.device));
    unsigned long long* d = nullptr;
    HIPCK(c, hipMalloc(&d, 16));
    hipError_t e = hipMemsetAsync(d, 0, 16, c->stream);
    if (e == hipSuccess) e = crt_launch_check_sqrt(d, c->stream);
    if (e == hipSuccess) e = hipMemcpyAsync(out, d, 16, hipMemcpyDeviceToHost, c->stream);
    if (e == hipSuccess) e = hipStreamSynchronize(c->stream);
    (void)hipFree(d);
    HIPCK(c, e);
    return CRT_OK;
}

extern "C" int crt_debug_primary_block(crt_ctx* c, float* out, float* camera, float* lightFloor)
{
    if (!c || !out) return CRT_ERR_INVALID;
    const crt::Scene& s = c->hScene;
    static_assert(offsetof(crt::Scene, primRoot) == offsetof(crt::Scene, rootPair) + 64 && offsetof(crt::Scene, primDown) + 12 == offsetof(crt::Scene, rootPair) + 64 + 4 * crt::kPrimFloats, "primary block");
    memcpy(out, s.rootPair, 64 + 4 * crt::kPrimFloats);
    if (camera) memcpy(camera, s.camPos, 48);
    if (lightFloor) { lightFloor[0] = s.lightInvT[7]; lightFloor[1] = s.lightInvT[3]; lightFloor[2] = s.lightInvT[11]; lightFloor[3] = s.floorD; }
    return CRT_OK;
}
extern "C" int crt_debug_primary_block_host(int op, const float* in, float* out)
{
    static crt::Scene s{};
    if (!in || !out || op < 0 || op > 2) return CRT_ERR_INVALID;
    if (op == 0) {
        s = crt::Scene{};
        s.camPos[2] = -2; s.topLeft[0] = -1; s.topLeft[1] = 1; s.topRight[0] = 1; s.topRight[1] = 1; s.bottomLeft[0] = -1; s.bottomLeft[1] = -1;
        memcpy(s.lightInvT, in, 48); s.floorD = in[12]; memcpy(s.rootPair, in + 13, 64); s.rootIsPair = 1;
    } else if (op == 1) { memcpy(s.camPos, in, 12); memcpy(s.topLeft, in + 3, 12); memcpy(s.topRight, in + 6, 12); memcpy(s.bottomLeft, in + 9, 12); }
    else memcpy(s.rootPair, in, 64);
    crt::set_primary(s);
    memcpy(out, s.rootPair, 64 + 4 * crt::kPrimFloats);
    return CRT_OK;
}

static int device_probe(crt_ctx* c, int op, const void* in, void* out, uint32_t n)
{
    static const uint8_t words[18][2] = {{1, 1}, {1, 1}, {2, 1}, {1, 1}, {2, 1}, {6, 7}, {1, 18}, {4, 1}, {5, 3}, {13, 2}, {16, 4}, {2, 2}, {2, 2}, {2, 2}, {2, 2}, {4, 2}, {2, 1}, {5, 3}};
    if (!c || !in || !out || op < 0 || op > 17 || n > (1u << 25)) return CRT_ERR_INVALID;
    if (n == 0) return CRT_OK;
    const size_t inBytes = (size_t)n * words[op][0] * 4, outBytes = (size_t)n * words[op][1] * 4;
    HIPCK(c, hipSetDevice(c->cfg.device));
    char* d = nullptr;
    HIPCK(c, hipMalloc((void**)&d, inBytes + outBytes));
    hipError_t e = hipMemcpyAsync(d, in, inBytes, hipMemcpyHostToDevice, c->stream);
    if (e == hipSuccess) e = (op <= 10 || op == 17) ? crt_launch_probe_f32(op, d, d + inBytes, n, c->stream) : crt_launch_probe_f64(op, d, d + inBytes, n, c->stream);
    if (e == hipSuccess) e = hipMemcpyAsync(out, d + inBytes, outBytes, hipMemcpyDeviceToHost, c->stream);
    if (e == hipSuccess) e = hipStreamSynchronize(c->stream);
    (void)hipFree(d);
    HIPCK(c, e);
    return CRT_OK;
}
extern "C" int crt_debug_device_probe(crt_ctx* c, int op, const void* in, void* out, uint32_t n) { return (op > 16) ? CRT_ERR_INVALID : device_probe(c, op, in, out, n); }
extern "C" int crt_debug_sky_probe(crt_ctx* c, const void* in, void* out, uint32_t n) { return device_probe(c, 17, in, out, n); }

extern "C" int crt_debug_plan_job(const uint32_t* cost, uint32_t n, uint32_t windows, uint32_t frames, int pool, double poolWindowTicks,
                                  uint32_t* table, uint32_t tableCap, uint32_t* head, uint32_t* order)
{
    if (!cost || !n || !table || !head || !order) return CRT_ERR_INVALID;
    crt_ctx c;
    c.tileCount = n; c.jobCostValid = true; c.poolWindowTicks = poolWindowTicks;
    c.streams.assign(2, nullptr);
    c.jobCost.assign(cost, cost + n);
    c.jobOrder.resize(n);
    for (uint32_t i = 0; i < n; i++) c.jobOrder[i] = i;
    std::stable_sort(c.jobOrder.begin(), c.jobOrder.end(), [&](uint32_t a, uint32_t b) { return c.jobCost[a] > c.jobCost[b]; });
    std::vector<uint32_t> t; uint32_t h = 0;
    plan_job(&c, windows, frames, pool != 0, t, &h);
    c.streams.clear();
    if (t.size() > tableCap) return CRT_ERR_INVALID;
    memcpy(table, t.data(), t.size() * 4); memcpy(order, c.jobOrder.data(), (size_t)n * 4); *head = h;
    return (int)t.size();
}

extern "C" long long crt_debug_pool_wave_plan(const uint32_t* cost, uint32_t nr, uint32_t frames, double perCost, double startTicks, uint32_t resident, double safety, double guard,
                                              double share, uint32_t* wf, uint32_t* longFrames, double* start, double* aim)
{
    if (!nr || !frames || !wf || !longFrames) return CRT_ERR_INVALID;
    PoolWaveTerms tm; if (safety > 0) tm.safety = safety; if (guard > 0) tm.guard = guard; if (share > 0) tm.share = share;
    std::vector<uint32_t> w; std::vector<double> st;
    const uint64_t waves = pool_wave_plan(cost, nr, frames, crt_pool_streams(frames), perCost, startTicks, resident, tm, w, longFrames, &st, aim);
    memcpy(wf, w.data(), (size_t)nr * 4);
    if (start) memcpy(start, st.data(), (size_t)nr * 8);
    return (long long)waves;
}
extern "C" int crt_debug_pool_long_waves(crt_ctx* c) { return c ? (int)c->lastLongWaves : -1; }
extern "C" void crt_debug_pool_wave_terms(double* out) { const PoolWaveTerms tm; out[0] = tm.poolLong; out[1] = tm.load; out[2] = tm.safety; out[3] = tm.guard; out[4] = tm.share; }

extern "C" int crt_debug_tile_costs(crt_ctx* c, uint32_t* out)
{
    if (!c || !out || !c->dTileCost) return CRT_ERR_INVALID;
    HIPCK(c, hipSetDevice(c->cfg.device));
    HIPCK(c, hipDeviceSynchronize());
    HIPCK(c, hipMemcpy(out, c->dTileCost, (size_t)c->tileCount * 4, hipMemcpyDeviceToHost));
    return CRT_OK;
}

extern "C" int crt_debug_lat_stage(crt_ctx* c, int stage, uint8_t* lanes, uint32_t* cost)
{
    if (!c || stage < 0 || stage > crt_ctx::kLatStages) return CRT_ERR_INVALID;
    if (c->latL[stage].size() != c->tileCount || c->latCost[stage].size() != c->tileCount) return CRT_ERR_STATE;
    if (lanes) memcpy(lanes, c->latL[stage].data(), c->tileCount);
    if (cost) memcpy(cost, c->latCost[stage].data(), (size_t)c->tileCount * 4);
    return c->latStage;
}

extern "C" int crt_debug_tile_stamps(crt_ctx* c, uint64_t* out)
{
    if (!c || !out || !c->dTileClocks) return CRT_ERR_INVALID;
    HIPCK(c, hipSetDevice(c->cfg.device));
    HIPCK(c, hipMemcpyAsync(out, c->dTileClocks + 2 * (size_t)c->tileCount, (size_t)c->tileCount * 128, hipMemcpyDeviceToHost, c->stream));
    HIPCK(c, hipStreamSynchronize(c->stream));
    return CRT_OK;
}

int crt_bind_accumulator(crt_ctx* c, void* p)
{
    if (!c) return CRT_ERR_INVALID;
// ... 15 lines not shown
```

### cpu-ray-tracer_amd/csrc/device/dev_common.h

```cpp
#pragma once
#include <hip/hip_runtime.h>
#include <stddef.h>
#include <stdint.h>
#include "layout.h"

namespace crt {

struct f3 { float x, y, z; };
__device__ __forceinline__ f3 mk3(float x, float y, float z) { f3 r; r.x = x; r.y = y; r.z = z; return r; }
__device__ __forceinline__ f3 operator+(f3 a, f3 b) { return mk3(a.x + b.x, a.y + b.y, a.z + b.z); }
__device__ __forceinline__ f3 operator-(f3 a, f3 b) { return mk3(a.x - b.x, a.y - b.y, a.z - b.z); }
__device__ __forceinline__ f3 operator-(f3 a) { return mk3(-a.x, -a.y, -a.z); }
__device__ __forceinline__ f3 operator*(f3 a, f3 b) { return mk3(a.x * b.x, a.y * b.y, a.z * b.z); }
__device__ __forceinline__ f3 operator*(f3 a, float b) { return mk3(a.x * b, a.y * b, a.z * b); }
__device__ __forceinline__ f3 operator*(float b, f3 a) { return mk3(b * a.x, b * a.y, b * a.z); }
__device__ __forceinline__ float dot3(f3 a, f3 b) { return a.x * b.x + a.y * b.y + a.z * b.z; }
__device__ __forceinline__ f3 cross3(f3 a, f3 b) { return mk3(a.y * b.z - a.z * b.y, a.z * b.x - a.x * b.z, a.x * b.y - a.y * b.x); }
#ifdef CRT_IEEE_DIV
__device__ __forceinline__ float rcp_nr(float x) { return 1.0f / x; }
#else
__device__ __forceinline__ float rcp_nr(float x) { const float r = __builtin_amdgcn_rcpf(x); return __builtin_fmaf(__builtin_fmaf(-x, r, 1.0f), r, r); }
#endif
__device__ __forceinline__ float rcp_exact(float x)
{
// ... 147 lines not shown
}
__device__ __forceinline__ uint32_t init_seed(uint32_t base) { return wang_hash((base + 1u) * 17u); }
__device__ __forceinline__ float rnd(uint32_t& s)
{
    s ^= s << 13; s ^= s >> 17; s ^= s << 5;
    return (float)s * 2.3283064365387e-10f;
}
__device__ __forceinline__ float rnd_pm1(uint32_t& s)
{
    s ^= s << 13; s ^= s >> 17; s ^= s << 5;
    return __builtin_fmaf((float)s, 4.656612873077392578125e-10f, -1.0f);
}


struct Hit { float t, u, v; int objIdx, triIdx; };
struct Cnt { uint32_t rays, primary, interior, leaf, tri, tlas, visits, meshhits; };

typedef float rec4 __attribute__((ext_vector_type(4)));
__device__ __forceinline__ rec4 ld4(const void* p) { return *reinterpret_cast<const rec4*>(p); }
__device__ __forceinline__ rec4 ldg(const char* __restrict__ base, uint32_t byteOff) { return *reinterpret_cast<const rec4*>(base + byteOff); }
static_assert(kMaxGeomBytes == (1ull << 32), "ldp: byteOff + 63 < 2^32");
template <uint32_t PIECE> __device__ __forceinline__ rec4 ldp(const char* __restrict__ base, uint32_t byteOff)
{
#ifndef CRT_DIET_NO_RECPTR
    __builtin_assume(byteOff <= 0xffffffffu - 63u);
#endif
    return ldg(base, byteOff + 16u * PIECE);
}
__device__ __forceinline__ bool finite3(f3 v)
{
    const uint32_t m = 0x7f800000u;
    return ((asu(v.x) & m) != m) && ((asu(v.y) & m) != m) && ((asu(v.z) & m) != m);
}

__device__ __forceinline__ float box_exact_rel(f3 lo, f3 hi, f3 rD, float tray)
{
    float tx1 = lo.x * rD.x, tx2 = hi.x * rD.x;
    float tmin = min_std(tx1, tx2), tmax = max_std(tx1, tx2);
    float ty1 = lo.y * rD.y, ty2 = hi.y * rD.y;
    tmin = max_std(tmin, min_std(ty1, ty2)); tmax = min_std(tmax, max_std(ty1, ty2));
    float tz1 = lo.z * rD.z, tz2 = hi.z * rD.z;
    tmin = max_std(tmin, min_std(tz1, tz2)); tmax = min_std(tmax, max_std(tz1, tz2));
    return (tmax >= tmin && tmin < tray && tmax > 0) ? tmin : 1e30f;
}
__device__ __forceinline__ float box_exact(rec4 lo, rec4 hi, f3 O, f3 rD, float tray)
{
    return box_exact_rel(mk3(lo.x - O.x, lo.y - O.y, lo.z - O.z), mk3(hi.x - O.x, hi.y - O.y, hi.z - O.z), rD, tray);
}
__device__ __forceinline__ float vmin(float a, float b) { float r; asm("v_min_f32 %0, %1, %2" : "=v"(r) : "v"(a), "v"(b)); return r; }
__device__ __forceinline__ float vmax(float a, float b) { float r; asm("v_max_f32 %0, %1, %2" : "=v"(r) : "v"(a), "v"(b)); return r; }
__device__ __forceinline__ float vmin3(float a, float b, float c) { float r; asm("v_min3_f32 %0, %1, %2, %3" : "=v"(r) : "v"(a), "v"(b), "v"(c)); return r; }
__device__ __forceinline__ float vmax3(float a, float b, float c) { float r; asm("v_max3_f32 %0, %1, %2, %3" : "=v"(r) : "v"(a), "v"(b), "v"(c)); return r; }
__device__ __forceinline__ float box_fast_rel(f3 lo, f3 hi, f3 rD, float tray)
{
    float tx1 = lo.x * rD.x, tx2 = hi.x * rD.x;
    float ty1 = lo.y * rD.y, ty2 = hi.y * rD.y;
    float tz1 = lo.z * rD.z, tz2 = hi.z * rD.z;
    float tmin = vmax3(vmin(tx1, tx2), vmin(ty1, ty2), vmin(tz1, tz2));
    float tmax = vmin3(vmax(tx1, tx2), vmax(ty1, ty2), vmax(tz1, tz2));
    return (tmax >= tmin && tmin < tray && tmax > 0) ? tmin : 1e30f;
}
__device__ __forceinline__ float box_fast(rec4 lo, rec4 hi, f3 O, f3 rD, float tray)
{
    return box_fast_rel(mk3(lo.x - O.x, lo.y - O.y, lo.z - O.z), mk3(hi.x - O.x, hi.y - O.y, hi.z - O.z), rD, tray);
}

__device__ __forceinline__ void hit_tri(rec4 a, rec4 b, rec4 c, f3 O, f3 D, Hit& h)
{
    const f3 v0 = mk3(a.x, a.y, a.z), e1 = mk3(b.x, b.y, b.z), e2 = mk3(c.x, c.y, c.z);
    const f3 hh = cross3(D, e2);
    const float det = dot3(e1, hh);
    const float f = rcp_exact_large(det);
    const f3 s = O - v0;
    const float u = f * dot3(s, hh);
    const f3 q = cross3(s, e1);
    const float v = f * dot3(D, q);
    const float t = f * dot3(e2, q);
    const bool ok = !(det > -0.0001f && det < 0.0001f) && !(u < 0 || u > 1) && !(v < 0 || u + v > 1) && (t > 0.0001f) && (t < h.t);
    if (ok) { h.t = t; h.u = u; h.v = v; h.triIdx = (int)asu(a.w); h.objIdx = (int)asu(b.w); }
}

struct LightFloor { float lightInvT[12]; float lightSize; uint32_t lightAxis, floorAxisY; float floorN[3]; float floorD; float preOy, preOx, preOz, preNum; };
template <bool PRE = false>
__device__ __forceinline__ void hit_light_floor(const LightFloor& sc, f3 O, f3 D, Hit& h)
{
    {
        const float* c = sc.lightInvT;
        float Oy, Dy;
        if (sc.lightAxis) { Oy = PRE ? sc.preOy : O.y + c[7]; Dy = D.y; }
        else { Oy = c[4] * O.x + c[5] * O.y + c[6] * O.z + c[7]; Dy = c[4] * D.x + c[5] * D.y + c[6] * D.z; }
        const float t = Oy / -Dy;
        if (t < h.t && t > 0) {
            float Ox, Oz, Dx, Dz;
            if (sc.lightAxis) { Ox = PRE ? sc.preOx : O.x + c[3]; Oz = PRE ? sc.preOz : O.z + c[11]; Dx = D.x; Dz = D.z; }
            else {
                Ox = c[0] * O.x + c[1] * O.y + c[2] * O.z + c[3];
                Oz = c[8] * O.x + c[9] * O.y + c[10] * O.z + c[11];
                Dx = c[0] * D.x + c[1] * D.y + c[2] * D.z;
                Dz = c[8] * D.x + c[9] * D.y + c[10] * D.z;
            }
            const float Ix = Ox + t * Dx, Iz = Oz + t * Dz;
            const float size = sc.lightSize;
            if (Ix > -size && Ix < size && Iz > -size && Iz < size) { h.t = t; h.objIdx = 0; }
        }
    }
    {
        float num, den;
        if (sc.floorAxisY) { num = PRE ? sc.preNum : O.y + sc.floorD; den = D.y; }
        else { const f3 N = mk3(sc.floorN[0], sc.floorN[1], sc.floorN[2]); num = dot3(O, N) + sc.floorD; den = dot3(D, N); }
        const float t = -num / den;
        if (t < h.t && t > 0) { h.t = t; h.objIdx = 1; }
    }
}

__device__ __forceinline__ void hit_light_floor(const Scene& sc, f3 O, f3 D, Hit& h)
{
    LightFloor lf;
#pragma unroll
    for (int i = 0; i < 12; i++) lf.lightInvT[i] = sc.lightInvT[i];
    lf.lightSize = sc.lightSize; lf.lightAxis = sc.lightAxis; lf.floorAxisY = sc.floorAxisY;
    lf.floorN[0] = sc.floorN[0]; lf.floorN[1] = sc.floorN[1]; lf.floorN[2] = sc.floorN[2]; lf.floorD = sc.floorD;
    lf.preOy = lf.preOx = lf.preOz = lf.preNum = 0.0f;
    hit_light_floor(lf, O, D, h);
}

__device__ __forceinline__ bool quad_occluded(const Scene& sc, f3 O, f3 D, float tmax)
{
    const float* c = sc.lightInvT;
    const float Oy = c[4] * O.x + c[5] * O.y + c[6] * O.z + c[7];
    const float Dy = c[4] * D.x + c[5] * D.y + c[6] * D.z;
    const float t = Oy / -Dy;
    if (!(t < tmax && t > 0)) return false;
    const float Ox = c[0] * O.x + c[1] * O.y + c[2] * O.z + c[3];
    const float Oz = c[8] * O.x + c[9] * O.y + c[10] * O.z + c[11];
    const float Dx = c[0] * D.x + c[1] * D.y + c[2] * D.z;
    const float Dz = c[8] * D.x + c[9] * D.y + c[10] * D.z;
    const float Ix = Ox + t * Dx, Iz = Oz + t * Dz;
    const float size = sc.lightSize;
    return Ix > -size && Ix < size && Iz > -size && Iz < size;
}

static_assert(offsetof(Scene, topLeft) == offsetof(Scene, camPos) + 12 && offsetof(Scene, bottomLeft) == offsetof(Scene, camPos) + 36 && offsetof(Scene, invW) == offsetof(Scene, camPos) + 48 && offsetof(Scene, invH) == offsetof(Scene, camPos) + 52, "camera block");
static_assert(offsetof(Scene, lightSize) == offsetof(Scene, lightInvT) + 60 && offsetof(Scene, floorN) == offsetof(Scene, lightInvT) + 76 && offsetof(Scene, floorD) == offsetof(Scene, lightInvT) + 88 && offsetof(Scene, floorInvto) == offsetof(Scene, floorN) + 16, "light / floor block");
static_assert(offsetof(Scene, floorAxisY) == offsetof(Scene, lightAxis) + 4 && offsetof(Scene, skyW) == offsetof(Scene, skyOffset) + 4 && offsetof(Scene, skyH) == offsetof(Scene, skyOffset) + 8, "flag / sky words");
static_assert(offsetof(Scene, primRoot) == offsetof(Scene, rootPair) + 64 && offsetof(Scene, primFloor) == offsetof(Scene, primLight) + 12 && offsetof(Scene, primDown) == offsetof(Scene, primRight) + 12, "camera-relative block");
static_assert(offsetof(Material, absorption) == 8 && offsetof(Material, texOffset) == 20 && offsetof(Material, texW) == 24 && offsetof(Material, texH) == 28, "Material words");
typedef const float __attribute__((address_space(4)))* kernarg_f;
__device__ __forceinline__ kernarg_f scene_floats(size_t byteOffset)
{
    const char __attribute__((address_space(4)))* p = (const char __attribute__((address_space(4)))*)__builtin_amdgcn_kernarg_segment_ptr() + byteOffset;
    asm volatile("" : "+s"(p));
    return (kernarg_f)p;
}

__device__ __forceinline__ void to_object_space(rec4 r0, rec4 r1, rec4 r2, f3 O, f3 D, f3& Oo, f3& Do, f3& rDo)
{
    Oo = mk3((O.x * r0.x + O.y * r0.y) + (O.z * r0.z + 1.0f * r0.w),
             (O.x * r1.x + O.y * r1.y) + (O.z * r1.z + 1.0f * r1.w),
             (O.x * r2.x + O.y * r2.y) + (O.z * r2.z + 1.0f * r2.w));
    Do = mk3((D.x * r0.x + D.y * r0.y) + D.z * r0.z,
             (D.x * r1.x + D.y * r1.y) + D.z * r1.z,
             (D.x * r2.x + D.y * r2.y) + D.z * r2.z);
    rDo = rcp_exact3(Do);
}

__device__ __forceinline__ void traverse_bvh_seq(const Scene& sc, uint32_t rootRef, f3 O, f3 D, f3 rD, Hit& h, uint32_t* stk, Cnt& cn,
                                                 int& traversed, int& tested)
{
    const char* __restrict__ g = sc.geom;
    uint32_t cur = rootRef, sp = 0;
    for (;;) {
        traversed++;
        const uint32_t off = (cur & kRefOffsetMask) << 4;
        if (cur & kRefInterior) {
            cn.interior++;
            const rec4 alo = ldg(g, off), ahi = ldg(g, off + 16), blo = ldg(g, off + 32), bhi = ldg(g, off + 48);
            float d1 = box_exact(alo, ahi, O, rD, h.t), d2 = box_exact(blo, bhi, O, rD, h.t);
            uint32_t r1 = asu(alo.w), r2 = asu(blo.w);
            if (d1 > d2) { float td = d1; d1 = d2; d2 = td; uint32_t tr = r1; r1 = r2; r2 = tr; }
            if (d1 == 1e30f) { if (sp == 0) break; cur = stk[(--sp) * 64]; }
            else { cur = r1; if (d2 != 1e30f) { stk[sp * 64] = r2; sp++; } }
        } else {
            cn.leaf++;
            uint32_t o = off;
            for (;;) {
                const rec4 a = ldg(g, o), b = ldg(g, o + 16), c = ldg(g, o + 32);
                tested++; cn.tri++;
                hit_tri(a, b, c, O, D, h);
                if (asu(c.w) <= 1u) break;
// ... 83 lines not shown
```

### cpu-ray-tracer_amd/csrc/device/launch.h

```cpp
#pragma once
#include "layout.h"

#include <hip/hip_runtime.h>

extern "C" {

hipError_t crt_launch_check_reciprocals(unsigned long long* out, hipStream_t stream);
hipError_t crt_launch_check_sqrt(unsigned long long* out, hipStream_t stream);
hipError_t crt_launch_render(const crt::Scene* sc, void* slab, crt::Counters* counters, unsigned long long* tileClocks, const uint32_t* tileOrder, uint32_t tileFirst, uint32_t tileStride,
    uint32_t tileCount, uint32_t tilesX, uint32_t sppFirst, uint32_t frames, uint32_t passes, uint32_t ldsBytes, int collectStats, const uint32_t* blockDesc, uint32_t nBlocks, uint32_t* tileCost,
    uint32_t rankCount, unsigned long long* launchClk, hipStream_t stream);
uint32_t crt_render_resident_waves(int device, int kind, uint32_t ldsBytes);
hipError_t crt_launch_accumulate(const void* slab, void* acc, uint32_t tileFirst, uint32_t tileStride, uint32_t tileCount, uint32_t tilesX, uint32_t W, uint32_t frames, uint32_t passes,
    hipStream_t stream);
hipError_t crt_launch_find_nearest(const crt::Scene* sc, const void* rays, void* hits, uint32_t n, crt::Counters* counters, uint32_t ldsBytes, uint32_t* cursor, hipStream_t stream);
hipError_t crt_launch_is_occluded(const crt::Scene* sc, const void* rays, int32_t* occluded, uint32_t n, uint32_t ldsBytes, uint32_t* cursor, hipStream_t stream);
hipError_t crt_launch_whitted(const crt::Scene* sc, int accel, const crt::AltAccelDev* alt, const crt::TlasAltDev* tl, void* acc, uint32_t* pixels, crt::Counters* counters, uint32_t ldsBytes,
    hipStream_t stream);
size_t crt_whitted_inspect_work_bytes(uint32_t pixelCount);
hipError_t crt_launch_whitted_inspect(const crt::Scene* sc, int accel, const crt::AltAccelDev* alt, const crt::TlasAltDev* tl, int inspect, int32_t peakIn, void* acc, uint32_t* pixels,
    crt::Counters* counters, int32_t* trav, int32_t* tested, void* work, uint32_t ldsBytes, hipStream_t stream);
hipError_t crt_launch_resolve(const void* acc, uint32_t* pixels, float* tileSums, uint32_t tileFirst, uint32_t tileStride, uint32_t tileCount, uint32_t tilesX, uint32_t W, float scale,
    hipStream_t stream);
hipError_t crt_launch_commit_frame(const void* slabWindow, uint32_t frameInWindow, uint32_t passes, void* acc, uint32_t* pixels, float* tileSums, uint32_t tileFirst, uint32_t tileStride,
    uint32_t tileCount, uint32_t tilesX, uint32_t W, float scale, hipStream_t stream);

uint32_t crt_pool_streams(uint32_t frames);
size_t crt_pool_scratch_bytes_per_window(uint32_t tileCount);
hipError_t crt_launch_render_pool(const crt::Scene* sc, void* slab, void* facScratch, crt::Counters* counters, unsigned long long* tileClocks, const uint32_t* tileOrder, uint32_t tileFirst,
    uint32_t tileStride, uint32_t tileCount, uint32_t tilesX, uint32_t sppFirst, uint32_t frames, uint32_t passes, int collectStats, uint32_t rankFirst, uint32_t waveFrames,
    const uint32_t* waveTab, uint32_t tabBlocks, uint32_t longFrames, uint32_t* tileCost, unsigned long long* launchClk, hipStream_t stream);
uint32_t crt_pool_lds_bytes(uint32_t stackDepth, uint32_t streams);
int crt_debug_pool_stamps(unsigned long long* out, int reset);
int crt_debug_pool_density(unsigned long long* out, int reset);
size_t crt_debug_pool_timeline(unsigned long long* out, size_t cap);

uint32_t crt_probe_paths(void);
hipError_t crt_launch_probe(const crt::Scene* sc, uint32_t tileFirst, uint32_t tileStride, uint32_t tileCount, uint32_t tilesX, uint32_t* tileCost, hipStream_t stream);
hipError_t crt_launch_render_alt(int accel, const crt::Scene* sc, const crt::AltAccelDev* acc, const crt::TlasAltDev* tl, void* slab, crt::Counters* counters, uint32_t tileFirst, uint32_t tileStride,
    uint32_t tileCount, uint32_t tilesX, uint32_t sppFirst, uint32_t frames, uint32_t passes, hipStream_t stream);
hipError_t crt_launch_sample_query(int accel, const crt::Scene* sc, const crt::AltAccelDev* acc, const crt::TlasAltDev* tl, const void* rays, uint32_t* seeds, float* rgb, uint32_t n,
    crt::Counters* counters, uint32_t* cursor, uint32_t* residentLanes, hipStream_t stream);

hipError_t crt_launch_find_nearest_prim(const crt::PrimDev* p, const void* rays, void* hits, uint32_t n, hipStream_t stream);
hipError_t crt_launch_render_prim(const crt::Scene* sc, const crt::PrimDev* p, void* slab, crt::Counters* counters, uint32_t tileFirst, uint32_t tileStride, uint32_t tileCount, uint32_t tilesX,
    uint32_t sppFirst, uint32_t frames, uint32_t passes, hipStream_t stream);
hipError_t crt_launch_sample_query_prim(const crt::Scene* sc, const crt::PrimDev* p, const void* rays, uint32_t* seeds, float* rgb, uint32_t n, crt::Counters* counters, uint32_t* cursor,
    uint32_t* residentLanes, hipStream_t stream);
hipError_t crt_launch_probe_f64(int op, const void* in, void* out, uint32_t n, hipStream_t stream);

hipError_t crt_launch_find_nearest_alt(int kind, const crt::Scene* sc, const crt::AltAccelDev* acc, const void* rays, void* hits, uint32_t n, uint32_t* cursor, hipStream_t stream);
hipError_t crt_launch_is_occluded_alt(int kind, const crt::Scene* sc, const crt::AltAccelDev* acc, const void* rays, int32_t* occluded, uint32_t n, uint32_t* cursor, hipStream_t stream);
hipError_t crt_launch_tlas_alt_query(int kind, bool occl, const crt::Scene* sc, const crt::TlasAltDev* tl, const void* rays, void* out, uint32_t n, uint32_t* cursor, hipStream_t stream);

hipError_t crt_launch_hit_info(const crt::Scene* sc, const void* rays, const void* hits, void* out, uint32_t n, uint32_t objects, uint32_t fileTris, hipStream_t stream);
hipError_t crt_launch_sky_color(const crt::Scene* sc, const void* rays, float* rgb, uint32_t n, hipStream_t stream);
hipError_t crt_launch_refit(char* geom, uint32_t leafOff, uint32_t pairBase, uint32_t triBase, uint32_t triCount, const float* pos, const void* plan, const uint32_t* levelOff, uint32_t levels,
    uint32_t rootCode, float* out, hipStream_t stream);
hipError_t crt_launch_probe_f32(int op, const void* in, void* out, uint32_t n, hipStream_t stream);

uint32_t crt_grid_build_blocks(int device);
size_t crt_grid_scan_chunks(uint32_t cells);
hipError_t crt_launch_grid_bounds(const float* pos, uint32_t triCount, crt::GridBuildState* state, uint32_t maxBlocks, hipStream_t stream);
hipError_t crt_launch_grid_count(const float* pos, uint32_t triCount, const crt::GridParams* g, uint32_t cells, uint32_t* counts, unsigned long long* chunkSums, crt::GridBuildState* state,
    uint32_t maxBlocks, hipStream_t stream);
hipError_t crt_launch_grid_fill(const float* pos, uint32_t triCount, const crt::GridParams* g, uint32_t cells, const uint32_t* cellStart, uint32_t* cursor, int32_t* unsorted, int32_t* refs,
    uint32_t total, const char* geom, uint32_t leafOff, uint32_t triBase, int globalIdx, crt::AltTri* tris, uint32_t maxBlocks, hipStream_t stream);

hipError_t crt_launch_tlas_build(const char* geom, uint32_t instOff, const float* T, const float* rootBox, uint32_t blasCount, uint32_t pairRel, uint32_t instRel, void* out,
    hipStream_t stream);

uint32_t crt_debug_query_grid(void);

}

namespace crt {

inline uint32_t bounded_query_grid(uint32_t grid) { const uint32_t k = crt_debug_query_grid(); return (k != 0u && k < grid) ? k : grid; }

inline uint32_t query_grid(uint32_t n, uint32_t ldsBytes)
{
    uint32_t perCu = ldsBytes ? (160u * 1024u) / ldsBytes : 16u; if (perCu > 16u) perCu = 16u; if (perCu < 4u) perCu = 4u;
    const uint32_t need = (n + 63u) / 64u, fill = 256u * perCu;
    return bounded_query_grid(need < fill ? need : fill);
}

inline bool query_launch_begin(uint32_t n, uint32_t* cursor, hipStream_t stream, hipError_t* status)
{
    *status = hipSuccess;
    if (n == 0) return false;
    if (!cursor) { *status = hipErrorInvalidValue; return false; }
    if (hipMemsetAsync(cursor, 0, 4, stream) != hipSuccess) { *status = hipGetLastError(); return false; }
    return true;
}

}
```

### cpu-ray-tracer_amd/csrc/device/layout.h

```cpp
#pragma once
#include <stdint.h>

namespace crt {

constexpr uint32_t kRefInterior = 0x80000000u;
constexpr uint32_t kRefTlasBit = 0x40000000u;
constexpr uint32_t kRefTlasInterior = 0x40000000u;
constexpr uint32_t kRefTlasLeaf = 0xC0000000u;
constexpr uint32_t kRefReturn = 0xFFFFFFFFu;
constexpr uint32_t kRefDone = 0u;
constexpr uint32_t kRefOffsetMask = 0x3fffffffu;
constexpr uint64_t kMaxGeomBytes = 1ull << 32;

constexpr uint32_t kRef16Interior = 0x8000u, kRef16TlasBit = 0x4000u, kRef16TlasLeaf = 0xC000u, kRef16TagMask = 0xC000u, kRef16IndexMask = 0x3fffu;
constexpr uint32_t kRef16Return = 0xFFFFu, kRef16MaxIndex = 0x3ffeu;

struct alignas(16) NodeChild { float lo[3]; uint32_t ref; float hi[3]; uint32_t ref16; };
struct alignas(64) NodePair { NodeChild c[2]; };

struct alignas(16) LeafTri {
    float v0[3]; uint32_t shadeIdx;
    float e1[3]; int32_t objIdx;
    float e2[3]; uint32_t remain;
};

struct alignas(16) ShadeTri {
    float n0[3], n1[3], n2[3];
    float uv0[2], uv1[2], uv2[2];
    int32_t mat;
};

struct alignas(16) TlasNode { float lo[3]; uint32_t ref; float hi[3]; uint32_t ref16; };

struct alignas(16) Instance {
    float invT[12];
    uint32_t shadeBase;
    uint32_t rootRef16;
    uint32_t rootRef;
    int32_t objIdx;
    float T[12];
    uint32_t triCount;
    uint32_t pad[3];
};

struct alignas(16) Material {
    float reflectivity, refractivity;
    float absorption[3];
    uint32_t texOffset;
    int32_t texW, texH;
};

struct Scene {
    int32_t kind;
    int32_t depthLimit;
    float camPos[3], topLeft[3], topRight[3], bottomLeft[3];
    float invW, invH;
    int32_t W, H;
    float lightInvT[12]; float lightNrm[3]; float lightSize;
    float lightPos[3];
    float floorN[3]; float floorD; float floorInvto;
    Material floorMat;
    uint32_t skyOffset; int32_t skyW, skyH;
    const char* geom;
    uint32_t tlasOff, instOff, shadeOff;
    uint32_t leafOff, tlasPairOff;
    uint32_t rootRef16, ref16ok;
    const uint32_t* texels;
    const Material* mats;
    uint32_t rootRef;
    uint32_t stackDepth;
    uint32_t bvhStack;
    uint32_t lightAxis, floorAxisY;
    uint32_t rootIsPair;
    float rootPair[16];
    float primRoot[12];
    float primLight[3];
    float primFloor;
    float primRight[3], primDown[3];
};
constexpr uint32_t kPrimFloats = 22u;

inline void set_primary(Scene& s)
{
    const float* O = s.camPos;
    for (int c = 0; c < 2; c++)
        for (int k = 0; k < 3; k++) {
            s.primRoot[6 * c + k] = s.rootPair[8 * c + k] - O[k];
            s.primRoot[6 * c + 3 + k] = s.rootPair[8 * c + 4 + k] - O[k];
        }
    s.primLight[0] = O[1] + s.lightInvT[7]; s.primLight[1] = O[0] + s.lightInvT[3]; s.primLight[2] = O[2] + s.lightInvT[11];
    s.primFloor = O[1] + s.floorD;
    for (int k = 0; k < 3; k++) { s.primRight[k] = s.topRight[k] - s.topLeft[k]; s.primDown[k] = s.bottomLeft[k] - s.topLeft[k]; }
}

struct Counters { unsigned long long v[8]; };

struct alignas(16) RefitPlanRec { uint32_t pair, child[2], pad; };
constexpr uint32_t kPlanInterior = 0x80000000u;

struct alignas(64) TlasBuildHeader {
    uint32_t status;
    uint32_t step;
    uint32_t height;
    uint32_t searches;
    uint32_t staleA;
    uint32_t pad[11];
};
constexpr uint32_t kTlasBuildOk = 0u, kTlasBuildNoCandidate = 1u, kTlasBuildNoEnd = 2u;
constexpr uint32_t kTlasMaxBlas = 256u;

#if defined(__HIPCC__)
#define CRT_HOST_DEVICE __host__ __device__
#else
#define CRT_HOST_DEVICE
#endif
template <class TriCountOf>
CRT_HOST_DEVICE inline bool hit_record_ok(int32_t objIdx, int32_t triIdx, uint32_t objects, TriCountOf&& triCountOf)
{
    if (objIdx < 2) return objIdx >= -1;
    if ((uint32_t)(objIdx - 2) >= objects) return false;
    return triIdx >= 0 && (uint32_t)triIdx < triCountOf((uint32_t)(objIdx - 2));
}

struct KdNode { float lo[3]; int32_t left; float hi[3]; int32_t right; float splitDistance; int32_t splitAxis; uint32_t firstTri, triCount; };
struct AltTri { float v0[3]; uint32_t triIdx; float e1[3]; int32_t objIdx; float e2[3]; uint32_t pad; };
struct AltAccelDev {
    const KdNode* kdNodes; const uint32_t* kdRefs; uint32_t kdStack;
    const AltTri* tris;
    int32_t res[3]; float cell[3]; float lo[3], hi[3]; const uint32_t* cellStart; const int32_t* cellRefs;
};

struct BlasAltDesc {
    uint32_t nodeBase, refBase, triBase;
    uint32_t cellBase, cellRefBase;
    int32_t objIdx;
    int32_t res[3]; float cell[3]; float lo[3], hi[3];
};
struct TlasAltDev {
    const BlasAltDesc* desc;
    const void* kdNodes; const uint32_t* kdRefs; const void* tris;
    const uint32_t* cellStart; const int32_t* cellRefs;
    uint32_t kdStack;
};

struct GridParams { int32_t res[3]; float cell[3]; float lo[3]; };
struct alignas(16) GridBuildState { unsigned long long key[6]; unsigned long long total; uint32_t nonFinite; uint32_t pad; };

struct PrimDev {
    float quadInvT[12], quadNrm[3], quadSize;
    float spherePos[3], pad0;
    float cubeInvM[12], cubeM[12], cubeMin[3], cubeMax[3];
    float torusInvT[12], torusT[12], rt2, rc2, r2, pad1;
    float refl[11], refr[11], absorb[33];
    float pad2;
    const uint32_t* red; const uint32_t* blue;
};

}
```

### cpu-ray-tracer_amd/csrc/device/render_pool.hip

```cpp
#include <type_traits>
#include "dev_common.h"
#include "launch.h"

namespace crt {

enum : uint32_t {
    F_OX = 0, F_OY, F_OZ, F_DX, F_DY, F_DZ,
    F_RX, F_RY, F_RZ,
    F_T,
    F_SEED, F_META,
    F_U, F_V,
    F_COUNT,
    F_CUR = F_U, F_PEND = F_V,
    F_TRI = F_RX
};
constexpr uint32_t kMetaItemMask = 0x7ffu, kMetaDepthShift = 11u, kMetaInside = 1u << 14, kMetaFresh = 1u << 15, kMetaObjShift = 16u, kMetaLowMask = 0xffffu;
constexpr uint32_t kQueueMask = 127u;

#ifndef CRT_POOL_MIN_WAVES
#define CRT_POOL_MIN_WAVES 4
#endif
#ifndef CRT_POOL_SHADE_MIN
#define CRT_POOL_SHADE_MIN 64
#endif
#ifndef CRT_POOL_NODE_STEPS
#define CRT_POOL_NODE_STEPS 2
#endif
#ifndef CRT_POOL_NODE2_MIN
#define CRT_POOL_NODE2_MIN 16
#endif
#ifndef CRT_POOL_STARVE
#define CRT_POOL_STARVE 40
#endif

#ifdef CRT_POOL_STAMPS
__device__ unsigned long long g_poolStamps[16];
#define CRT_PSTAMP(var) unsigned long long var; asm volatile("s_memtime %0\n\ts_waitcnt lgkmcnt(0)" : "=s"(var) :: "memory")
#define CRT_PACC(i, a, b) (pst[i] += (b) - (a))
#else
#define CRT_PSTAMP(var)
#define CRT_PACC(i, a, b)
#endif
#ifdef CRT_POOL_DENS
__device__ unsigned long long g_poolDens[48];
#define CRT_DENS(i, v) (dens[i] += (uint32_t)(v))
#define CRT_DENS_MASK(i, pred) (dens[i] += (uint32_t)__popcll(__builtin_amdgcn_ballot_w64(pred)))
#define CRT_LIVE_BUCKET(n) ((n) >= 112u ? 0u : (n) >= 96u ? 1u : (n) >= 64u ? 2u : 3u)
#else
#define CRT_DENS(i, v)
#define CRT_DENS_MASK(i, pred)
#endif
#ifdef CRT_POOL_TIMELINE
__device__ unsigned long long* g_poolTimeline = nullptr;
#endif
__device__ __forceinline__ bool lane_in(uint64_t m) { return __builtin_amdgcn_inverse_ballot_w64(m); }
__device__ __forceinline__ uint64_t finite3_mask(f3 v)
{
#ifdef CRT_DIET_NO_MASKS
    const uint32_t m = 0x7f800000u;
    return __builtin_amdgcn_ballot_w64((asu(v.x) & m) != m) & __builtin_amdgcn_ballot_w64((asu(v.y) & m) != m) & __builtin_amdgcn_ballot_w64((asu(v.z) & m) != m);
#else
    const float inf = __builtin_inff();
    return __builtin_amdgcn_fcmpf(__builtin_fabsf(v.x), inf, 4) & __builtin_amdgcn_fcmpf(__builtin_fabsf(v.y), inf, 4) & __builtin_amdgcn_fcmpf(__builtin_fabsf(v.z), inf, 4);
#endif
}
__device__ __forceinline__ uint32_t rank_in(uint64_t m) { return __builtin_amdgcn_mbcnt_hi((uint32_t)(m >> 32), __builtin_amdgcn_mbcnt_lo((uint32_t)m, 0u)); }

template <int KIND, bool COUNT, int S>
__global__ __launch_bounds__(64, CRT_POOL_MIN_WAVES) void render_pool_kernel(const Scene sc, float4* __restrict__ slab, float* __restrict__ facScratch, Counters* __restrict__ counters,
                                                             unsigned long long* __restrict__ tileClocks, const uint32_t* __restrict__ tileOrder,
                                                             uint32_t tileFirst, uint32_t tileStride, uint32_t tileCount, uint32_t tilesX,
                                                             uint32_t sppFirst, uint32_t frames, uint32_t passes, uint32_t groups, uint32_t waveFrames, const uint32_t* __restrict__ waveTab, uint32_t tabBlocks, uint32_t longFrames,
                                                             uint32_t rankFirst, uint32_t* __restrict__ tileCost, unsigned long long* __restrict__ launchClk)
{
    extern __shared__ uint32_t lds[];
    const uint32_t lane = threadIdx.x;
#ifdef CRT_POOL_TIMELINE
    const unsigned long long tl0 = wall_clock64();
#endif
    const unsigned long long clk0 = (COUNT || tileCost) ? wall_clock64() : 0ull;
    if (launchClk && lane == 0) { atomicMax(&launchClk[0], ~clk0); atomicMax(&launchClk[1], clk0); }
    uint32_t rank0, grp, wf = waveFrames, first = 0u, limit = frames;
    if (waveTab) {
        if (blockIdx.x < tabBlocks) {
            uint32_t lo = 0u, hi = tileCount - rankFirst;
            while (hi - lo > 1u) { const uint32_t mid = (lo + hi) >> 1; if (waveTab[2u * mid] <= blockIdx.x) lo = mid; else hi = mid; }
            rank0 = lo; grp = blockIdx.x - waveTab[2u * lo]; wf = waveTab[2u * lo + 1u]; limit = longFrames;
        } else { const uint32_t b = blockIdx.x - tabBlocks; rank0 = b / groups; grp = b - rank0 * groups; wf = (uint32_t)S; first = longFrames; }
    } else { rank0 = blockIdx.x / groups; grp = blockIdx.x - rank0 * groups; }
    const uint32_t rank = rank0 + rankFirst;
    if (rank >= tileCount) return;
    const uint32_t tl = tileOrder ? tileOrder[rank] : rank;
    const uint32_t frame0 = first + grp * wf;
    if (frame0 >= limit) return;
    const uint32_t nOwn = (limit - frame0 < wf) ? limit - frame0 : wf;
    const uint32_t nStreams = nOwn < (uint32_t)S ? nOwn : (uint32_t)S;
    const uint32_t tile = tileFirst + tl * tileStride;
    const uint32_t tx = tile % tilesX, ty = tile / tilesX;
    const char* __restrict__ geom = sc.geom;
    float* __restrict__ fac = facScratch + (size_t)blockIdx.x * (15u * (uint32_t)S);

    char* const ldsB = reinterpret_cast<char*>(lds);
    const uint32_t laneB = lane * 2u;
    uint32_t* st = lds + (sc.stackDepth + 1u) * 32u;
    float* stf = reinterpret_cast<float*>(st);
    uint8_t* qEnd = reinterpret_cast<uint8_t*>(st + F_COUNT * S);
    uint8_t* qBnc = qEnd + 128, * qRdy = qEnd + 256;
    uint16_t* slotFrame = reinterpret_cast<uint16_t*>(qEnd + 384);
    auto stk_top = [&](uint32_t at) -> uint32_t { return *reinterpret_cast<const uint16_t*>(ldsB + at); };
    auto stk_put = [&](uint32_t at, uint32_t v) { *reinterpret_cast<uint16_t*>(ldsB + at) = (uint16_t)v; };

    Cnt cn; cn.rays = cn.primary = cn.interior = cn.leaf = cn.tri = cn.tlas = cn.visits = cn.meshhits = 0;
    uint32_t trips = 0;
#ifdef CRT_POOL_DENS
    uint32_t dens[48]; for (int i = 0; i < 48; i++) dens[i] = 0;
    uint32_t live = nStreams; unsigned long long liveClk = wall_clock64();
#endif
    const uint32_t items = 256u * passes;
    const uint32_t rowLen = 64u * passes;
    const f3 nil3 = mk3(0.0f, 0.0f, 0.0f);

    for (uint32_t s = lane; s < nStreams; s += 64u) {
        st[F_SEED * S + s] = init_seed(tx + ty * (uint32_t)sc.W + (sppFirst + (frame0 + s) * passes) * 1799u);
        st[F_META * S + s] = kMetaFresh;
        qEnd[s] = (uint8_t)s;
        if (S > 64) slotFrame[s] = (uint16_t)s;
    }
    uint32_t nextFrame = nStreams;
    uint32_t endH = 0, endT = nStreams, bncH = 0, bncT = 0, rdyH = 0, rdyT = 0;

    uint64_t mRes = 0ull;
    uint64_t mFinite = ~0ull;
    uint32_t sid = 0, cur = kRefDone, spB = laneB, metaLo = 0u;
    f3 tO = nil3, tD = nil3, trD = nil3;
    Hit h; h.t = 1e34f; h.u = 0; h.v = 0; h.objIdx = -1; h.triIdx = -1;
    rec4 q0 = {0, 0, 0, 0}, q1 = q0, q2 = q0, q3 = q0;

    auto new_ray = [&](auto primary, bool act, uint32_t s, f3 v, bool norm, f3 O, uint32_t seed, uint32_t meta) {
#ifdef CRT_DIET_NO_CAMREL
        constexpr bool PRIM = false;
#else
        constexpr bool PRIM = decltype(primary)::value;
#endif
        f3 D = v, rD = v; Hit nh; nh.t = 1e34f; nh.u = 0; nh.v = 0; nh.objIdx = -1; nh.triIdx = -1;
        uint32_t ncur = kRefDone, pend = 0u;
        if (act) {
            const float inv = rcp_exact(sqrt_exact(dot3(v, v)));
            D = norm ? v * inv : v;
            rD = rcp_exact3(D);
            cn.rays++;
            {
                const kernarg_f lp = scene_floats(offsetof(Scene, lightInvT));
                const kernarg_f ax = scene_floats(offsetof(Scene, lightAxis));
                LightFloor lf;
#pragma unroll
                for (int i = 0; i < 12; i++) lf.lightInvT[i] = lp[i];
                lf.lightSize = lp[15]; lf.floorN[0] = lp[19]; lf.floorN[1] = lp[20]; lf.floorN[2] = lp[21]; lf.floorD = lp[22];
                lf.lightAxis = asu(ax[0]); lf.floorAxisY = asu(ax[1]);
                lf.preOy = lf.preOx = lf.preOz = lf.preNum = 0.0f;
                if constexpr (PRIM) {
                    constexpr size_t pl = (offsetof(Scene, primLight) - offsetof(Scene, lightInvT)) / 4;
                    lf.preOy = lp[pl]; lf.preOx = lp[pl + 1]; lf.preOz = lp[pl + 2]; lf.preNum = lp[pl + 3];
                }
                hit_light_floor<PRIM>(lf, O, D, nh);
            }
            if (sc.rootIsPair) {
                const kernarg_f rp = scene_floats(offsetof(Scene, rootPair));
                const rec4 a0 = {rp[0], rp[1], rp[2], rp[3]}, a1 = {rp[4], rp[5], rp[6], rp[7]};
                const rec4 b0 = {rp[8], rp[9], rp[10], rp[11]}, b1 = {rp[12], rp[13], rp[14], rp[15]};
                float d1, d2;
                const bool allFinite = (__builtin_amdgcn_ballot_w64(true) & ~finite3_mask(rD)) == 0ull;
                if constexpr (PRIM) {
                    const f3 ra0 = mk3(rp[16], rp[17], rp[18]), ra1 = mk3(rp[19], rp[20], rp[21]), rb0 = mk3(rp[22], rp[23], rp[24]), rb1 = mk3(rp[25], rp[26], rp[27]);
                    if (allFinite) { d1 = box_fast_rel(ra0, ra1, rD, nh.t); d2 = box_fast_rel(rb0, rb1, rD, nh.t); }
                    else { d1 = box_exact_rel(ra0, ra1, rD, nh.t); d2 = box_exact_rel(rb0, rb1, rD, nh.t); }
                } else if (allFinite) { d1 = box_fast(a0, a1, O, rD, nh.t); d2 = box_fast(b0, b1, O, rD, nh.t); }
                else { d1 = box_exact(a0, a1, O, rD, nh.t); d2 = box_exact(b0, b1, O, rD, nh.t); }
                const bool sw = d1 > d2;
                const float dn = sw ? d2 : d1, df = sw ? d1 : d2;
                const uint32_t rn = sw ? asu(b1.w) : asu(a1.w), rf = sw ? asu(a1.w) : asu(b1.w);
                const bool hitN = dn != 1e30f;
                pend = (hitN && df != 1e30f) ? rf : 0u;
                ncur = hitN ? rn : kRefDone;
                if (COUNT) { if (KIND == 0) cn.interior++; else cn.tlas++; }
            } else ncur = sc.rootRef16;
            if (COUNT && KIND == 0 && (ncur & kRef16TagMask) == 0u && ncur != kRefDone) cn.leaf++;
            stf[F_OX * S + s] = O.x; stf[F_OY * S + s] = O.y; stf[F_OZ * S + s] = O.z;
            stf[F_DX * S + s] = D.x; stf[F_DY * S + s] = D.y; stf[F_DZ * S + s] = D.z;
            stf[F_RX * S + s] = rD.x; stf[F_RY * S + s] = rD.y; stf[F_RZ * S + s] = rD.z;
            stf[F_T * S + s] = nh.t;
            st[F_SEED * S + s] = seed; st[F_META * S + s] = meta | ((uint32_t)(nh.objIdx + 1) << kMetaObjShift);
            st[F_CUR * S + s] = ncur; st[F_PEND * S + s] = pend;
        }
        const uint32_t depth = (meta >> kMetaDepthShift) & 7u;
        const uint64_t mAct = __builtin_amdgcn_ballot_w64(act);
        const uint64_t mW = mAct & __builtin_amdgcn_ballot_w64(ncur != kRefDone);
        const uint64_t mStop = __builtin_amdgcn_ballot_w64((uint32_t)(nh.objIdx + 1) <= 1u) | __builtin_amdgcn_ballot_w64((int)depth >= sc.depthLimit);
        const uint64_t mE = mAct & ~mW & mStop, mB = mAct & ~mW & ~mStop;
        CRT_DENS(20, __popcll(mAct)); CRT_DENS(19, __popcll(mW));
        if (lane_in(mW)) qRdy[(rdyT + rank_in(mW)) & kQueueMask] = (uint8_t)s;
        if (lane_in(mE)) qEnd[(endT + rank_in(mE)) & kQueueMask] = (uint8_t)s;
        if (lane_in(mB)) qBnc[(bncT + rank_in(mB)) & kQueueMask] = (uint8_t)s;
        rdyT += (uint32_t)__popcll(mW); endT += (uint32_t)__popcll(mE); bncT += (uint32_t)__popcll(mB);
    };
    auto world_ray = [&]() {
        tO = mk3(stf[F_OX * S + sid], stf[F_OY * S + sid], stf[F_OZ * S + sid]);
        tD = mk3(stf[F_DX * S + sid], stf[F_DY * S + sid], stf[F_DZ * S + sid]);
        trD = mk3(stf[F_RX * S + sid], stf[F_RY * S + sid], stf[F_RZ * S + sid]);
    };

    uint64_t mNode2 = 0ull;
    auto node_step = [&](uint64_t m) {
        const bool allFinite = (m & ~mFinite) == 0ull;
        if (lane_in(m)) {
            if (COUNT) { if (KIND == 1 && (cur & kRef16TlasBit) != 0u) cn.tlas++; else cn.interior++; }
            const uint32_t top = stk_top(spB);
            float d1, d2;
            if (__builtin_expect(allFinite, 1)) { d1 = box_fast(q0, q1, tO, trD, h.t); d2 = box_fast(q2, q3, tO, trD, h.t); }
            else { d1 = box_exact(q0, q1, tO, trD, h.t); d2 = box_exact(q2, q3, tO, trD, h.t); }
            const bool sw = d1 > d2;
            const float dn = sw ? d2 : d1, df = sw ? d1 : d2;
            const uint32_t rn = sw ? asu(q3.w) : asu(q1.w), rf = sw ? asu(q1.w) : asu(q3.w);
            stk_put(spB + 128u, rf);
            const bool hitN = dn != 1e30f, push = hitN && df != 1e30f;
            const bool pop = !hitN && spB != laneB;
            cur = hitN ? rn : (pop ? top : kRefDone);
            spB = spB + (push ? 128u : 0u) - (pop ? 128u : 0u);
            if (COUNT && (cur & kRef16TagMask) == 0u && cur != kRefDone) cn.leaf++;
        }
    };
    auto load_records = [&](uint64_t m) {
        const uint32_t idx = cur & kRef16IndexMask;
        const bool inter = (cur & kRef16Interior) != 0u;
        uint32_t oa = idx * (inter ? 64u : 48u) + (inter ? 0u : sc.leafOff - 48u);
        if (KIND == 1 && (cur & kRef16TlasBit) != 0u)
            oa = (cur & kRef16Interior) ? sc.instOff + idx * 128u : sc.tlasPairOff + idx * 64u;
        if (lane_in(m)) { q0 = ldp<0>(geom, oa); q1 = ldp<1>(geom, oa); q2 = ldp<2>(geom, oa); q3 = ldp<3>(geom, oa); }
    };

    auto tri_step = [&](uint64_t m) {
        CRT_DENS(3, 1); CRT_DENS(4, __popcll(m));
        if (lane_in(m)) {
            if (COUNT) cn.tri++;
            const uint32_t top = stk_top(spB);
            hit_tri(q0, q1, q2, tO, tD, h);
            const bool more = asu(q2.w) > 1u;
            const bool pop = !more && spB != laneB;
            const uint32_t next = more ? cur + 1u : (pop ? top : kRefDone);
            spB -= pop ? 128u : 0u;
            if (COUNT && !more && (next & kRef16TagMask) == 0u && next != kRefDone) cn.leaf++;
            cur = next;
        }
    };

#ifdef CRT_POOL_STAMPS
    unsigned long long pst[12] = {0, 0, 0, 0, 0, 0, 0, 0, 0, 0, 0, 0};
#endif
    for (;;) {
        CRT_PSTAMP(p0);
        if (mRes != 0ull) {
            uint64_t mNode, mTlas = 0ull;
            if (KIND == 0) mNode = mRes & __builtin_amdgcn_ballot_w64(cur > 0x7fffu);
            else { mTlas = mRes & __builtin_amdgcn_ballot_w64(cur >= kRef16TlasLeaf); mNode = mRes & __builtin_amdgcn_ballot_w64(cur - kRef16TlasBit < 0x8000u); }
            const uint64_t mTri = mRes & ~(mNode | mTlas);
            asm volatile("" : "+v"(q0), "+v"(q1), "+v"(q2), "+v"(q3));
            CRT_DENS(22, __popcll(mRes));
            if (mNode) { CRT_DENS(1, 1); CRT_DENS(2, __popcll(mNode)); }

            if (KIND == 1 && mTlas) { CRT_DENS(23, 1); CRT_DENS(24, __popcll(mTlas)); }
            uint64_t mBack = 0ull;
            if (KIND == 1 && mTlas != 0ull) {
                if (lane_in(mTlas)) {
                    if (COUNT) { cn.tlas++; cn.visits++; }
                    const f3 O = mk3(stf[F_OX * S + sid], stf[F_OY * S + sid], stf[F_OZ * S + sid]);
                    const f3 D = mk3(stf[F_DX * S + sid], stf[F_DY * S + sid], stf[F_DZ * S + sid]);
                    to_object_space(q0, q1, q2, O, D, tO, tD, trD);
                    spB += 128u; stk_put(spB, kRef16Return);
                    const uint32_t next = asu(q3.y);
                    if (COUNT && (next & kRef16TagMask) == 0u && next != kRefDone) cn.leaf++;
                    cur = next;
                }
                mFinite = (mFinite & ~mTlas) | (mTlas & finite3_mask(trD));
            }
            if (mNode != 0ull) node_step(mNode);
#if CRT_POOL_NODE_STEPS > 1
            uint64_t mLeafNow = 0ull;
// ... 42 lines not shown
                }
                if (lane_in(mE)) qEnd[(endT + rank_in(mE)) & kQueueMask] = (uint8_t)sid;
                if (lane_in(mB)) qBnc[(bncT + rank_in(mB)) & kQueueMask] = (uint8_t)sid;
                endT += (uint32_t)__popcll(mE); bncT += (uint32_t)__popcll(mB);
                mRes &= ~mFin;
            }
            asm volatile("" ::: "memory");
        }
        CRT_PSTAMP(p1); CRT_PACC(0, p0, p1);
        if (__builtin_expect(mRes == 0ull, 0)) {
            if ((endT - endH) + (bncT - bncH) + (rdyT - rdyH) == 0u) break;
        }
        if (COUNT) trips++;
        CRT_DENS(0, 1);
#ifdef CRT_POOL_DENS
        dens[32u + CRT_LIVE_BUCKET(live)]++;
#endif
        {
            const uint32_t nRdy = rdyT - rdyH;
            const uint64_t mFree = ~mRes;
            if (nRdy != 0u) if (mFree != 0ull) {
                const uint32_t myRank = rank_in(mFree);
                const uint64_t mTake = mFree & __builtin_amdgcn_ballot_w64(myRank < nRdy);
                CRT_DENS(7, 1); CRT_DENS(8, __popcll(mTake));
                if (lane_in(mTake)) {
                    sid = qRdy[(rdyH + myRank) & kQueueMask];
                    tO = mk3(stf[F_OX * S + sid], stf[F_OY * S + sid], stf[F_OZ * S + sid]);
                    tD = mk3(stf[F_DX * S + sid], stf[F_DY * S + sid], stf[F_DZ * S + sid]);
                    trD = mk3(stf[F_RX * S + sid], stf[F_RY * S + sid], stf[F_RZ * S + sid]);
                    const uint32_t meta = st[F_META * S + sid];
                    h.t = stf[F_T * S + sid]; h.objIdx = (int)(meta >> kMetaObjShift) - 1; h.u = 0; h.v = 0; h.triIdx = -1;
                    metaLo = meta & kMetaLowMask;
                    cur = st[F_CUR * S + sid];
                    const uint32_t pend = st[F_PEND * S + sid];
                    stk_put(laneB + 128u, pend);
                    spB = laneB + (pend ? 128u : 0u);
                }
                mFinite = (mFinite & ~mTake) | (mTake & finite3_mask(trD));
                mRes |= mTake;
                rdyH += (uint32_t)__popcll(mTake);
            }
            if (mRes != 0ull) {
                CRT_DENS(21, 1);
                const uint32_t idx = cur & kRef16IndexMask;
                const bool inter = (cur & kRef16Interior) != 0u;
                uint32_t oa = idx * (inter ? 64u : 48u) + (inter ? 0u : sc.leafOff - 48u);
                if (KIND == 1 && (cur & kRef16TlasBit) != 0u)
                    oa = (cur & kRef16Interior) ? sc.instOff + idx * 128u : sc.tlasPairOff + idx * 64u;
                if (!lane_in(mRes)) oa = 0u;
                q0 = ldp<0>(geom, oa); q1 = ldp<1>(geom, oa); q2 = ldp<2>(geom, oa); q3 = ldp<3>(geom, oa);
            }
        }
        asm volatile("" ::: "memory");
        {
            const uint32_t nEnd = endT - endH, nBnc = bncT - bncH, nRdy = rdyT - rdyH, nRes = (uint32_t)__popcll(mRes);
            const bool starving = nRes + nRdy < (uint32_t)CRT_POOL_STARVE;
            bool runEnd = false, runBnc = false;
            if ((nEnd | nBnc) >= (uint32_t)CRT_POOL_SHADE_MIN || starving) {
                runEnd = nEnd >= (uint32_t)CRT_POOL_SHADE_MIN || (starving && nEnd > 0u && nEnd >= nBnc);
                runBnc = nBnc >= (uint32_t)CRT_POOL_SHADE_MIN || (starving && nBnc > nEnd);
            }

            CRT_PSTAMP(p2b); CRT_PACC(1, p1, p2b);
            if (runEnd) {
                const uint32_t n = nEnd < 64u ? nEnd : 64u;
                const bool act = lane < n;
                const uint32_t s = act ? qEnd[(endH + lane) & kQueueMask] : 0u;
                endH += n;
                uint32_t meta = 0, seed = 0; int obj = -1; f3 D = nil3;
                if (act) { meta = st[F_META * S + s]; seed = st[F_SEED * S + s]; obj = (int)(meta >> kMetaObjShift) - 1; D = mk3(stf[F_DX * S + s], stf[F_DY * S + s], stf[F_DZ * S + s]); }
                const bool first = (meta & kMetaFresh) != 0u;
                const int depth = (int)((meta >> kMetaDepthShift) & 7u);
                uint32_t item = meta & kMetaItemMask;
                const bool ended = act && !first, miss = ended && obj == -1;
#ifdef CRT_POOL_DENS
                dens[36u + CRT_LIVE_BUCKET(live)]++;
#endif
                CRT_DENS(9, 1); CRT_DENS(10, n); CRT_DENS_MASK(11, miss); CRT_DENS_MASK(13, act && first); CRT_DENS_MASK(25, ended && depth > 0); CRT_DENS_MASK(26, ended && depth > 1); CRT_DENS_MASK(27, ended && depth > 2);
                if (ended && obj >= 2) cn.meshhits++;
                float fk[15];
#pragma unroll
                for (int k = 0; k < 5; k++) {
                    fk[3 * k] = fk[3 * k + 1] = fk[3 * k + 2] = 0.0f;
                    if (ended && depth > k) {
#pragma unroll
                        for (int j = 0; j < 3; j++) fk[3 * k + j] = __hip_atomic_load(fac + (3 * k + j) * S + s, __ATOMIC_RELAXED, __HIP_MEMORY_SCOPE_AGENT);
                    }
                }
                uint32_t skyTexel = 0u;
                if (miss) {
                    float phi, theta; sky_angles(D, phi, theta);
                    const kernarg_f sk = scene_floats(offsetof(Scene, skyOffset));
                    skyTexel = sc.texels[tex_index(asu(sk[0]), (int)asu(sk[1]), (int)asu(sk[2]), phi * CRT_INV2PI, theta * CRT_INVPI)];
                }
                bool gen = act && first;
                size_t sampleAt = 0;
                if (ended) {
                    uint32_t pix = item, pass = 0;
                    if (passes != 1u) { pix = item / passes; pass = item - pix * passes; }
                    const uint32_t fr = frame0 + (S > 64 ? (uint32_t)slotFrame[s] : s);
                    sampleAt = (((size_t)(fr >> 6) * tileCount + tl) * 256u + pix) * rowLen + ((fr & 63u) * passes + pass);
                    item++;
                    gen = item < items;
                }
                if (S > 64) if (nextFrame < nOwn) {
                    const uint64_t mDone = __builtin_amdgcn_ballot_w64(ended) & ~__builtin_amdgcn_ballot_w64(gen);
                    if (mDone != 0ull) {
                        const uint32_t f = nextFrame + rank_in(mDone);
                        const uint64_t mTake = mDone & __builtin_amdgcn_ballot_w64(f < nOwn);
                        if (lane_in(mTake)) {
                            slotFrame[s] = (uint16_t)f;
                            seed = init_seed(tx + ty * (uint32_t)sc.W + (sppFirst + (frame0 + f) * passes) * 1799u);
                            item = 0u; gen = true;
                        }
                        nextFrame += (uint32_t)__popcll(mTake);
                    }
                }
#ifdef CRT_POOL_DENS
                {
                    const uint32_t gone = (uint32_t)__popcll(__builtin_amdgcn_ballot_w64(ended) & ~__builtin_amdgcn_ballot_w64(gen));
                    if (gone) { const unsigned long long now = wall_clock64(); dens[44u + CRT_LIVE_BUCKET(live)] += (uint32_t)(now - liveClk); liveClk = now; live -= gone; }
                }
#endif
                const kernarg_f cam = scene_floats(offsetof(Scene, camPos));
                const f3 camPos = mk3(cam[0], cam[1], cam[2]);
                f3 v = camPos;
                if (gen) {
                    const uint32_t pix = (passes == 1u) ? item : item / passes;
                    const int x = (int)(tx * 16u + (pix & 15u)), y = (int)(ty * 16u + (pix >> 4));
                    const float jy = rnd(seed);
                    const float jx = rnd(seed);
                    const float u = ((float)x + jx) * cam[12], vv = ((float)y + jy) * cam[13];
                    const f3 TL = mk3(cam[3], cam[4], cam[5]);
#ifdef CRT_DIET_NO_CAMREL
                    const f3 TR = mk3(cam[6], cam[7], cam[8]), BL = mk3(cam[9], cam[10], cam[11]);
                    const f3 right = TR - TL, down = BL - TL;
#else
                    constexpr size_t pc = (offsetof(Scene, primRight) - offsetof(Scene, camPos)) / 4;
                    const f3 right = mk3(cam[pc], cam[pc + 1], cam[pc + 2]), down = mk3(cam[pc + 3], cam[pc + 4], cam[pc + 5]);
#endif
                    const f3 P = TL + u * right + vv * down;
                    v = P - camPos;
                    cn.primary++;
                }
                CRT_DENS_MASK(12, gen);
                CRT_PSTAMP(e1); CRT_PACC(2, p2b, e1);
                new_ray(std::true_type{}, gen, s, v, true, camPos, seed, item);
                CRT_PSTAMP(e2); CRT_PACC(3, e1, e2);
                if (ended) {
                    f3 L = miss ? tex_unpack(skyTexel) : ((depth >= sc.depthLimit) ? mk3(0, 0, 0) : mk3(24, 24, 22));
#pragma unroll
                    for (int k = 4; k >= 0; k--)
                        if (depth > k) L = mk3(fk[3 * k], fk[3 * k + 1], fk[3 * k + 2]) * L;
                    slab[sampleAt] = make_float4(L.x, L.y, L.z, 0.0f);
                }
#ifdef CRT_POOL_STAMPS
                { CRT_PSTAMP(e3); CRT_PACC(4, e2, e3); pst[10]++; }
#endif
                asm volatile("" :: "v"(fk[0]), "v"(fk[1]), "v"(fk[2]), "v"(fk[3]), "v"(fk[4]), "v"(fk[5]), "v"(fk[6]), "v"(fk[7]), "v"(fk[8]), "v"(fk[9]), "v"(fk[10]), "v"(fk[11]), "v"(fk[12]), "v"(fk[13]), "v"(fk[14]), "v"(skyTexel));
            }
            CRT_PSTAMP(p3);
            asm volatile("" ::: "memory");
            if (runBnc) {
                const uint32_t n = nBnc < 64u ? nBnc : 64u;
                const bool act = lane < n;
                const uint32_t s = act ? qBnc[(bncH + lane) & kQueueMask] : 0u;
                bncH += n;
                f3 O = nil3, D = nil3; float ht = 0, hu = 0, hv = 0; int obj = 1; uint32_t tri = 0, seed = 0, meta = 0;
                if (act) {
                    tri = st[F_TRI * S + s];
                    O = mk3(stf[F_OX * S + s], stf[F_OY * S + s], stf[F_OZ * S + s]);
                    D = mk3(stf[F_DX * S + s], stf[F_DY * S + s], stf[F_DZ * S + s]);
                    ht = stf[F_T * S + s]; hu = stf[F_U * S + s]; hv = stf[F_V * S + s];
                    seed = st[F_SEED * S + s]; meta = st[F_META * S + s]; obj = (int)(meta >> kMetaObjShift) - 1;
                }
                const bool mesh = act && obj >= 2;
#ifdef CRT_POOL_DENS
                dens[40u + CRT_LIVE_BUCKET(live)]++;
#endif
                CRT_DENS(14, 1); CRT_DENS(15, n); CRT_DENS_MASK(16, mesh);
                rec4 s0 = {0, 0, 0, 0}, s1 = s0, s2 = s0, s3 = s0;
                if (mesh) { const uint32_t so = sc.shadeOff + tri * 64u; s0 = ldp<0>(geom, so); s1 = ldp<1>(geom, so); s2 = ldp<2>(geom, so); s3 = ldp<3>(geom, so); cn.meshhits++; }
                const bool inside = (meta & kMetaInside) != 0u;
                const int depth = (int)((meta >> kMetaDepthShift) & 7u);
                const uint32_t item = meta & kMetaItemMask;
                float tu = 0, tv = 0; uint32_t tOff = 0; int tW = 0, tH = 0;
                f3 I = O, N = O, absorb = O; float refl = 0, refr = 0;
                f3 v = O, pre = O; bool norm = false, diffuse = false, newInside = false;
                if (act) {
                    I = O + ht * D;
                    if (obj == 1) {
                        const kernarg_f fl = scene_floats(offsetof(Scene, floorN));
                        const kernarg_f fm = scene_floats(offsetof(Scene, floorMat));
                        N = mk3(fl[0], fl[1], fl[2]);
                        if (N.y == 1) {
                            float u = I.x, vv = I.z;
                            u *= fl[4]; vv *= fl[4];
                            tu = u - __builtin_floorf(u); tv = vv - __builtin_floorf(vv);
                        }
                        refl = fm[0]; refr = fm[1];
                        absorb = mk3(fm[2], fm[3], fm[4]);
                        tOff = asu(fm[5]); tW = (int)asu(fm[6]); tH = (int)asu(fm[7]);
                    } else {
                        const f3 n0 = mk3(s0.x, s0.y, s0.z), n1 = mk3(s0.w, s1.x, s1.y), n2 = mk3(s1.z, s1.w, s2.x);
                        const float w = 1 - hu - hv;
                        const f3 Nn = w * n0 + hu * n1 + hv * n2;
                        tu = w * s2.y + hu * s2.w + hv * s3.y;
                        tv = w * s2.z + hu * s3.x + hv * s3.z;
                        const rec4* mp = reinterpret_cast<const rec4*>(sc.mats + (int)asu(s3.w));
                        const rec4 m0 = mp[0], m1 = mp[1];
                        refl = m0.x; refr = m0.y; absorb = mk3(m0.z, m0.w, m1.x);
                        tOff = asu(m1.y); tW = (int)asu(m1.z); tH = (int)asu(m1.w);
                        if (KIND == 0) {
                            N = normalize3(Nn);
                        } else {
                            const uint32_t io = sc.instOff + (uint32_t)(obj - 2) * 128u + 64u;
                            const rec4 r0 = ldp<0>(geom, io), r1 = ldp<1>(geom, io), r2 = ldp<2>(geom, io);
                            N = normalize3(mk3(r0.x * Nn.x + r0.y * Nn.y + r0.z * Nn.z + r0.w * 0.0f,
                                               r1.x * Nn.x + r1.y * Nn.y + r1.z * Nn.z + r1.w * 0.0f,
                                               r2.x * Nn.x + r2.y * Nn.y + r2.z * Nn.z + r2.w * 0.0f));
                        }
                    }
                    if (dot3(N, D) > 0) N = -N;
                    uint32_t texel = 0x00ffffffu;
                    if (tW > 0) texel = sc.texels[tex_index(tOff, tW, tH, tu, tv)];
                    f3 medium = mk3(1, 1, 1);
                    if (inside) {
                        const f3 ab = absorb * -ht;
                        medium = mk3(crt_expf(ab.x), crt_expf(ab.y), crt_expf(ab.z));
                    }
                    CRT_PSTAMP(b1); CRT_PACC(5, p3, b1);
                    const float r = rnd(seed);
                    const bool mirror = r < refl, dielectric = !mirror && r < refl + refr;
                    if (mirror) {
                        v = D - 2.0f * N * dot3(N, D);
                    } else if (dielectric) {
// ... 33 lines not shown
                    __hip_atomic_store(fd + S, factor.y, __ATOMIC_RELAXED, __HIP_MEMORY_SCOPE_AGENT);
                    __hip_atomic_store(fd + 2 * S, factor.z, __ATOMIC_RELAXED, __HIP_MEMORY_SCOPE_AGENT);
                    O = I + nv * CRT_EPS;
                    CRT_PSTAMP(b3); CRT_PACC(7, b2, b3);
                }
                CRT_PSTAMP(b4);
                new_ray(std::false_type{}, act, s, v, false, O, seed, item | ((uint32_t)(depth + 1) << kMetaDepthShift) | (newInside ? kMetaInside : 0u));
#ifdef CRT_POOL_STAMPS
                { CRT_PSTAMP(b5); CRT_PACC(8, b4, b5); pst[11]++; }
#endif
                asm volatile("" :: "v"(s0), "v"(s1), "v"(s2), "v"(s3));
            }
#ifdef CRT_POOL_STAMPS
            pst[9]++;
#endif
        }
    }
#ifdef CRT_POOL_STAMPS
    if (lane == 0) for (int i = 0; i < 12; i++) atomicAdd(&g_poolStamps[i], pst[i]);
#endif
#ifdef CRT_POOL_DENS
    dens[44u + CRT_LIVE_BUCKET(live)] += (uint32_t)(wall_clock64() - liveClk);
    if (lane == 0) for (int i = 0; i < 48; i++) if (dens[i]) atomicAdd(&g_poolDens[i], (unsigned long long)dens[i]);
#endif

#ifdef CRT_POOL_TIMELINE
    if (lane == 0 && g_poolTimeline) { uint32_t hw; asm volatile("s_getreg_b32 %0, hwreg(HW_REG_HW_ID)" : "=s"(hw)); g_poolTimeline[3 * (size_t)blockIdx.x] = tl0; g_poolTimeline[3 * (size_t)blockIdx.x + 1] = wall_clock64(); g_poolTimeline[3 * (size_t)blockIdx.x + 2] = hw; }
#endif
    if (tileCost && lane == 0 && nOwn == (uint32_t)S) atomicMax(&tileCost[tl], (uint32_t)((wall_clock64() - clk0) * 64ull / (uint32_t)S));
    if (launchClk && lane == 0) { const unsigned long long now = wall_clock64(), last = __hip_atomic_load(&launchClk[1], __ATOMIC_RELAXED, __HIP_MEMORY_SCOPE_AGENT), from = last > clk0 ? last : clk0; if (now > from) atomicAdd(&launchClk[2], now - from); }
    if (COUNT && tileClocks && lane == 0 && nOwn == frames) {
        tileClocks[2 * tl] = wall_clock64() - clk0;
        tileClocks[2 * tl + 1] = trips;
    }
    uint32_t vals[8] = {cn.rays, cn.primary, cn.interior, cn.leaf, cn.tri, cn.tlas, cn.visits, cn.meshhits};
#pragma unroll
    for (int i = 0; i < 8; i++) {
        if (!COUNT && i >= 2 && i != 7) continue;
        uint32_t sum = wave_sum(vals[i]);
        if (lane == 0 && sum) atomicAdd(&counters->v[i], (unsigned long long)sum);
    }
}

}

#ifndef CRT_POOL_STREAMS
#define CRT_POOL_STREAMS 128
#endif
extern "C" uint32_t crt_pool_streams(uint32_t frames) { return frames > 64u ? (uint32_t)CRT_POOL_STREAMS : 64u; }
#ifndef CRT_POOL_EXTRA_LDS
#define CRT_POOL_EXTRA_LDS 0
#endif
extern "C" uint32_t crt_pool_lds_bytes(uint32_t stackDepth, uint32_t streams) { return (stackDepth + 1u) * 64u * 2u + crt::F_COUNT * streams * 4u + 3u * 128u + (streams > 64u ? 2u * streams : 0u) + (uint32_t)CRT_POOL_EXTRA_LDS; }
extern "C" size_t crt_pool_scratch_bytes_per_window(uint32_t tileCount) { return (size_t)tileCount * 128u * 15u * 4u; }

#ifdef CRT_POOL_STAMPS
extern "C" int crt_debug_pool_stamps(unsigned long long* out, int reset)
{
    if (out && hipMemcpyFromSymbol(out, HIP_SYMBOL(crt::g_poolStamps), 128) != hipSuccess) return -1;
    if (reset) { unsigned long long z[16] = {}; if (hipMemcpyToSymbol(HIP_SYMBOL(crt::g_poolStamps), z, 128) != hipSuccess) return -1; }
    return 0;
}
#endif
#ifdef CRT_POOL_DENS
extern "C" int crt_debug_pool_density(unsigned long long* out, int reset)
{
    if (out && hipMemcpyFromSymbol(out, HIP_SYMBOL(crt::g_poolDens), 384) != hipSuccess) return -1;
    if (reset) { unsigned long long z[48] = {}; if (hipMemcpyToSymbol(HIP_SYMBOL(crt::g_poolDens), z, 384) != hipSuccess) return -1; }
    return 0;
}
#endif
#ifdef CRT_POOL_TIMELINE
static unsigned long long* g_timelineHost = nullptr; static size_t g_timelineCount = 0;
extern "C" size_t crt_debug_pool_timeline(unsigned long long* out, size_t cap)
{
    const size_t n = g_timelineCount < cap ? g_timelineCount : cap;
    if (out && n) (void)hipMemcpy(out, g_timelineHost, n * 24, hipMemcpyDeviceToHost);
    return g_timelineCount;
}
#endif
extern "C" hipError_t crt_launch_render_pool(const crt::Scene* sc, void* slab, void* facScratch, crt::Counters* counters, unsigned long long* tileClocks, const uint32_t* tileOrder,
                                             uint32_t tileFirst, uint32_t tileStride, uint32_t tileCount, uint32_t tilesX, uint32_t sppFirst,
                                             uint32_t frames, uint32_t passes, int collectStats, uint32_t rankFirst, uint32_t waveFrames, const uint32_t* waveTab, uint32_t tabBlocks, uint32_t longFrames,
                                             uint32_t* tileCost, unsigned long long* launchClk, hipStream_t stream)
{
    if (tileCount == 0 || frames == 0) return hipSuccess;
    if (!sc->ref16ok) return hipErrorInvalidValue;
    const uint32_t S = crt_pool_streams(frames);
    const uint32_t wf = (S == 64u || waveFrames < S) ? S : waveFrames;
    if (wf % S != 0u || wf > 0xff80u) return hipErrorInvalidValue;
    if (S == 64u) waveTab = nullptr;
    if (waveTab && (tabBlocks == 0u || longFrames == 0u || longFrames > frames)) return hipErrorInvalidValue;
    const uint32_t groups = waveTab ? (frames - longFrames + S - 1u) / S : (frames + wf - 1u) / wf;
    if ((unsigned long long)tileCount * ((frames + S - 1u) / S) > 0x7fffffffull) return hipErrorInvalidValue;
    if (rankFirst >= tileCount) return hipSuccess;
    dim3 grid(waveTab ? tabBlocks + (tileCount - rankFirst) * groups : (tileCount - rankFirst) * groups), block(64);
#ifdef CRT_POOL_TIMELINE
    { static unsigned long long* buf = nullptr; static size_t cap = 0;
      if (cap < (size_t)grid.x) { if (buf) (void)hipFree(buf); (void)hipMalloc((void**)&buf, (size_t)grid.x * 24); cap = grid.x; (void)hipMemcpyToSymbol(HIP_SYMBOL(crt::g_poolTimeline), &buf, sizeof(buf)); }
      (void)hipMemsetAsync(buf, 0, (size_t)grid.x * 24, stream); g_timelineHost = buf; g_timelineCount = grid.x; }
#endif
    const uint32_t ldsBytes = crt_pool_lds_bytes(sc->stackDepth, S);
#define CRT_LAUNCH(K, C, SS) hipLaunchKernelGGL((crt::render_pool_kernel<K, C, SS>), grid, block, ldsBytes, stream, *sc, (float4*)slab, (float*)facScratch, counters, tileClocks, tileOrder, tileFirst, tileStride, tileCount, tilesX, sppFirst, frames, passes, groups, wf, waveTab, tabBlocks, longFrames, rankFirst, tileCost, launchClk)
#define CRT_LAUNCH_S(K, C) do { if (S == 64u) CRT_LAUNCH(K, C, 64); else CRT_LAUNCH(K, C, CRT_POOL_STREAMS); } while (0)
    if (sc->kind == 0) { if (collectStats) CRT_LAUNCH_S(0, true); else CRT_LAUNCH_S(0, false); }
    else { if (collectStats) CRT_LAUNCH_S(1, true); else CRT_LAUNCH_S(1, false); }
#undef CRT_LAUNCH_S
#undef CRT_LAUNCH
    return hipGetLastError();
}
```

Baseline: 30530 Mrays/s.

## Classify screen tiles on host to skip light, floor and BVH tests for primary rays

Adds a host-side, conservative per-tile classifier. It projects the root BVH boxes onto the screen and checks the tile-corner ray directions against the light and floor planes, then uploads one class byte per tile. The render kernel reads the class uniformly per wave and skips the light, floor or root BVH tests for camera rays in tiles that provably cannot hit them. Full sky tiles also skip the reciprocal direction and the throughput product. The cost is extra host work and an upload whenever the camera or scene changes, plus a risk of wrong skips if the conservative bounds are off.

```diff
diff --git a/cpu-ray-tracer_amd/__init__.py b/cpu-ray-tracer_amd/__init__.py
--- a/cpu-ray-tracer_amd/__init__.py
+++ b/cpu-ray-tracer_amd/__init__.py
@@ -534,6 +534,19 @@
         self._ck(self.L.crt_get_timing(self.h, C.byref(t)))
         return dict(render_kernel_ms=t.render_kernel_ms, resolve_kernel_ms=t.resolve_kernel_ms, render_launches=t.render_launches, pool_launches=t.pool_launches, split_launches=t.split_launches)
 
+    def tile_classes(self):
+        self.L.crt_debug_tile_classes.restype = C.c_int
+        self.L.crt_debug_tile_classes.argtypes = [C.c_void_p, C.c_void_p, C.c_uint32]
+        n = self.L.crt_debug_tile_classes(self.h, None, 0)
+        if n < 0:
+            self._ck(n)
+        out = np.zeros(n, np.uint8)
+        if n:
+            rc = self.L.crt_debug_tile_classes(self.h, _p(out), n)
+            if rc < 0:
+                self._ck(rc)
+        return out
+
     def tile_clocks(self, tile_count):
         a = np.zeros((tile_count, 2), np.uint64)
         self._ck(self.L.crt_get_tile_clocks(self.h, _p(a)))
@@ -874,6 +887,25 @@
     return rank, world, count
 
 
+TILE_NO_LIGHT, TILE_NO_FLOOR, TILE_NO_TREE = 1, 2, 4
+TILE_SKY = 7
+
+
+def tile_classes_host(camera, light_offsets, light_size, floor_d, root_pair, width, height, tile_first=0, tile_stride=1, tile_count=-1, flags=7):
+    if tile_count < 0:
+        tile_first, tile_stride, tile_count = 0, 1, (width // 16) * (height // 16)
+    v = np.concatenate([np.asarray(camera, np.float32).reshape(12), np.asarray(light_offsets, np.float32).reshape(3), np.array([light_size, floor_d], np.float32),
+                        np.asarray(root_pair, np.float32).reshape(16)]).astype(np.float32)
+    out = np.zeros(tile_count, np.uint8)
+    L = lib()
+    L.crt_debug_tile_classes_host.restype = C.c_int
+    L.crt_debug_tile_classes_host.argtypes = [C.c_void_p, C.c_uint32, C.c_int, C.c_int, C.c_uint32, C.c_uint32, C.c_uint32, C.c_void_p]
+    rc = L.crt_debug_tile_classes_host(_p(v), flags, width, height, tile_first, tile_stride, tile_count, _p(out))
+    if rc != 0:
+        raise CrtError(rc, "crt_debug_tile_classes_host: invalid argument")
+    return out
+
+
 def reduce_accumulator(tensor, dist, dst=0):
     dist.reduce(tensor, dst=dst, op=dist.ReduceOp.SUM)
     return tensor
diff --git a/cpu-ray-tracer_amd/csrc/abi.cpp b/cpu-ray-tracer_amd/csrc/abi.cpp
--- a/cpu-ray-tracer_amd/csrc/abi.cpp
+++ b/cpu-ray-tracer_amd/csrc/abi.cpp
@@ -1,5 +1,6 @@
 #include "../../include/crt_abi.h"
 #include "device/launch.h"
+#include "device/tile_class.h"
 #include "host/grid_resolution.h"
 
 #include <cmath>
@@ -73,6 +74,9 @@
     float meshLo[3] = {0, 0, 0}, meshHi[3] = {0, 0, 0}; bool orderDirty = true;
     uint32_t* dTileOrder = nullptr;
     uint32_t* hTileOrder[2] = {nullptr, nullptr}; hipEvent_t orderCopied[2] = {nullptr, nullptr}; hipEvent_t orderReady = nullptr; int orderFlip = 0;
+    bool classDirty = true;
+    uint8_t* dTileClass = nullptr;
+    uint8_t* hTileClass[2] = {nullptr, nullptr}; hipEvent_t classCopied[2] = {nullptr, nullptr}; int classFlip = 0;
     bool haveScene = false;
     struct Flat { int32_t kind = 0; uint64_t leafOff = 0, tlasOff = 0, tlasPairOff = 0, instOff = 0, shadeOff = 0; uint32_t tlasNodeCount = 0, maxHeight = 0;
                   uint32_t objects = 0;
@@ -254,6 +258,8 @@
 
 void crt_debug_enable_hooks(int on) { g_hooks = on != 0; }
 
+static void primary_changed(crt_ctx* c) { crt::set_primary(c->hScene); c->classDirty = true; }
+
 int crt_device_count(void)
 {
     int n = 0;
@@ -327,7 +333,7 @@
     s.bottomLeft[0] = -aspect; s.bottomLeft[1] = -1; s.bottomLeft[2] = 0;
     s.W = cfg->width; s.H = cfg->height; s.invW = 1.0f / cfg->width; s.invH = 1.0f / cfg->height;
     s.depthLimit = c->cfg.depthLimit;
-    crt::set_primary(s);
+    primary_changed(c);
     if ((e = hipStreamSynchronize(c->stream)) != hipSuccess) return bail(e, "hipStreamSynchronize");
     *out = c;
     return CRT_OK;
@@ -368,6 +374,7 @@
     if (c->dInspectWork) (void)hipFree(c->dInspectWork);
     if (c->dTileClocks) (void)hipFree(c->dTileClocks);
     if (c->dTileOrder) (void)hipFree(c->dTileOrder);
+    if (c->dTileClass) (void)hipFree(c->dTileClass);
     if (c->dTileCost) (void)hipFree(c->dTileCost);
     if (c->dJobCost) (void)hipFree(c->dJobCost);
     if (c->dJobDesc) (void)hipFree(c->dJobDesc);
@@ -383,6 +390,7 @@
     if (c->descReady) (void)hipEventDestroy(c->descReady);
     if (c->dStage) (void)hipFree(c->dStage);
     for (int k = 0; k < 2; k++) { if (c->hTileOrder[k]) (void)hipHostFree(c->hTileOrder[k]); if (c->orderCopied[k]) (void)hipEventDestroy(c->orderCopied[k]); }
+    for (int k = 0; k < 2; k++) { if (c->hTileClass[k]) (void)hipHostFree(c->hTileClass[k]); if (c->classCopied[k]) (void)hipEventDestroy(c->classCopied[k]); }
     for (int k = 0; k < 2; k++) { if (c->hStage[k]) (void)hipHostFree(c->hStage[k]); if (c->stageCopied[k]) (void)hipEventDestroy(c->stageCopied[k]); }
     if (c->stream) (void)hipStreamDestroy(c->stream);
     delete c;
@@ -621,7 +629,7 @@
         s.rootIsPair = 1;
     }
     if (hook("CRT_DEBUG_NO_ROOTPAIR")) s.rootIsPair = 0;
-    crt::set_primary(s);
+    primary_changed(c);
     s.stackDepth = s.bvhStack + ((sd->kind == CRT_SCENE_TLAS) ? tlasHeight + 1 : 0);
     c->ldsBytes = s.stackDepth * 64u * 4u; c->latSlots = 0;
     if (const char* e = hook("CRT_DEBUG_EXTRA_LDS")) c->ldsBytes += (uint32_t)atoi(e);
@@ -748,7 +756,7 @@
         s.rootIsPair = 1;
     }
     if (hook("CRT_DEBUG_NO_ROOTPAIR")) s.rootIsPair = 0;
-    crt::set_primary(s);
+    primary_changed(c);
     memcpy(c->meshLo, lo, 12); memcpy(c->meshHi, hi, 12); c->orderDirty = true;
 }
 
@@ -864,7 +872,7 @@
     crt::Scene& s = c->hScene;
     if (!memcmp(s.camPos, camPos, 12) && !memcmp(s.topLeft, tl, 12) && !memcmp(s.topRight, tr, 12) && !memcmp(s.bottomLeft, bl, 12)) return CRT_OK;
     memcpy(s.camPos, camPos, 12); memcpy(s.topLeft, tl, 12); memcpy(s.topRight, tr, 12); memcpy(s.bottomLeft, bl, 12);
-    crt::set_primary(s);
+    primary_changed(c);
     c->orderDirty = true; c->epoch++;
     return CRT_OK;
 }
@@ -928,6 +936,24 @@
     c->jobCostValid = false; c->jobCostPending = false; c->planValid = false;
     { const int r = upload_tile_order(c, first); if (r) return r; }
     c->orderDirty = false;
+    return 0;
+}
+
+static int update_tile_class(crt_ctx* c)
+{
+    if (!c->classDirty || c->tileCount == 0) return 0;
+    if (!c->dTileClass) HIPCK(c, hipMalloc((void**)&c->dTileClass, (size_t)c->tileCount));
+    { const int r = order_behind_ahead(c); if (r) return r; }
+    const int k = c->classFlip ^= 1;
+    if (!c->hTileClass[k]) {
+        HIPCK(c, hipHostMalloc((void**)&c->hTileClass[k], (size_t)c->tileCount, hipHostMallocDefault));
+        HIPCK(c, ensure_event(&c->classCopied[k]));
+    } else HIPCK(c, hipEventSynchronize(c->classCopied[k]));
+    crt::classify_tiles(c->hScene, c->cfg.width, c->cfg.height, (uint32_t)c->tilesX, c->tileFirst, c->tileStride, c->tileCount, c->hTileClass[k]);
+    HIPCK(c, hipMemcpyAsync(c->dTileClass, c->hTileClass[k], (size_t)c->tileCount, hipMemcpyHostToDevice, c->stream));
+    HIPCK(c, hipEventRecord(c->classCopied[k], c->stream));
+    c->orderReady = c->classCopied[k];
+    c->classDirty = false;
     return 0;
 }
 
@@ -1486,7 +1512,8 @@
         if (le == hipSuccess)
             le = crt_launch_render_pool(&c->hScene, L.slab, scratch, c->dCounters, c->dTileClocks, c->dTileOrder, c->tileFirst, c->tileStride, c->tileCount, (uint32_t)c->tilesX,
                                         L.sppFirst, L.nf, L.passes, c->cfg.collectStats, L.jobBlocks ? L.head : 0u, L.waveFrames, L.waveTab, L.waveBlocks, L.longFrames,
-                                        L.wantJobCost ? c->dJobCost : nullptr, L.jobClk, st2);
+                                        L.wantJobCost ? c->dJobCost : nullptr, L.jobClk,
+                                        (c->classDirty || hook("CRT_DEBUG_NO_TILE_CLASS")) ? nullptr : c->dTileClass , st2);
         if (le == hipSuccess) c->lastLongWaves = L.longWaves;
         if (L.jobBlocks && le == hipSuccess) le = join(st2);
     } else if (L.jobBlocks) {
@@ -1599,6 +1626,7 @@
     { int r = discard_ahead(c); if (r) return r; }
     if (c->tileCount == 0 || frames == 0) return CRT_OK;
     { int r = update_tile_order(c); if (r) return r; }
+    { int r = update_tile_class(c); if (r) return r; }
     if (c->streams.empty()) {
         int n = c->cfg.renderStreams;
         if (n <= 0) n = 7;
@@ -2756,6 +2784,35 @@
     return CRT_OK;
 }
 
+extern "C" int crt_debug_tile_classes(crt_ctx* c, uint8_t* out, uint32_t cap)
+{
+    if (!c || (!out && cap)) return CRT_ERR_INVALID;
+    HIPCK(c, hipSetDevice(c->cfg.device));
+    { const int r = update_tile_class(c); if (r) return r; }
+    const uint32_t n = cap < c->tileCount ? cap : c->tileCount;
+    if (n) {
+        HIPCK(c, hipMemcpyAsync(out, c->dTileClass, n, hipMemcpyDeviceToHost, c->stream));
+        HIPCK(c, hipStreamSynchronize(c->stream));
+    }
+    return (int)c->tileCount;
+}
+extern "C" int crt_debug_tile_classes_host(const float* in, uint32_t flags, int W, int H, uint32_t tileFirst, uint32_t tileStride, uint32_t tileCount, uint8_t* out)
+{
+    if (!in || !out || W < 16 || H < 16 || tileStride == 0) return CRT_ERR_INVALID;
+    const uint32_t tilesX = (uint32_t)(W / 16), tiles = tilesX * (uint32_t)(H / 16);
+    if (tileCount && (unsigned long long)tileFirst + (unsigned long long)(tileCount - 1) * tileStride >= tiles) return CRT_ERR_INVALID;
+    crt::Scene s{};
+    memcpy(s.camPos, in, 12); memcpy(s.topLeft, in + 3, 12); memcpy(s.topRight, in + 6, 12); memcpy(s.bottomLeft, in + 9, 12);
+    s.W = W; s.H = H; s.invW = 1.0f / W; s.invH = 1.0f / H;
+    s.lightInvT[0] = s.lightInvT[5] = s.lightInvT[10] = 1.0f; s.lightInvT[3] = in[12]; s.lightInvT[7] = in[13]; s.lightInvT[11] = in[14];
+    s.lightSize = in[15]; s.floorN[1] = 1.0f; s.floorD = in[16];
+    memcpy(s.rootPair, in + 17, 64);
+    s.lightAxis = flags & 1u; s.floorAxisY = (flags >> 1) & 1u; s.rootIsPair = (flags >> 2) & 1u;
+    crt::set_primary(s);
+    crt::classify_tiles(s, W, H, tilesX, tileFirst, tileStride, tileCount, out);
+    return CRT_OK;
+}
+
 static int device_probe(crt_ctx* c, int op, const void* in, void* out, uint32_t n)
 {
     static const uint8_t words[18][2] = {{1, 1}, {1, 1}, {2, 1}, {1, 1}, {2, 1}, {6, 7}, {1, 18}, {4, 1}, {5, 3}, {13, 2}, {16, 4}, {2, 2}, {2, 2}, {2, 2}, {2, 2}, {4, 2}, {2, 1}, {5, 3}};
diff --git a/cpu-ray-tracer_amd/csrc/device/dev_common.h b/cpu-ray-tracer_amd/csrc/device/dev_common.h
--- a/cpu-ray-tracer_amd/csrc/device/dev_common.h
+++ b/cpu-ray-tracer_amd/csrc/device/dev_common.h
@@ -253,9 +253,9 @@
 
 struct LightFloor { float lightInvT[12]; float lightSize; uint32_t lightAxis, floorAxisY; float floorN[3]; float floorD; float preOy, preOx, preOz, preNum; };
 template <bool PRE = false>
-__device__ __forceinline__ void hit_light_floor(const LightFloor& sc, f3 O, f3 D, Hit& h)
-{
-    {
+__device__ __forceinline__ void hit_light_floor(const LightFloor& sc, f3 O, f3 D, Hit& h, bool skipLight = false, bool skipFloor = false)
+{
+    if (!skipLight) {
         const float* c = sc.lightInvT;
         float Oy, Dy;
         if (sc.lightAxis) { Oy = PRE ? sc.preOy : O.y + c[7]; Dy = D.y; }
@@ -275,7 +275,7 @@
             if (Ix > -size && Ix < size && Iz > -size && Iz < size) { h.t = t; h.objIdx = 0; }
         }
     }
-    {
+    if (!skipFloor) {
         float num, den;
         if (sc.floorAxisY) { num = PRE ? sc.preNum : O.y + sc.floorD; den = D.y; }
         else { const f3 N = mk3(sc.floorN[0], sc.floorN[1], sc.floorN[2]); num = dot3(O, N) + sc.floorD; den = dot3(D, N); }
diff --git a/cpu-ray-tracer_amd/csrc/device/launch.h b/cpu-ray-tracer_amd/csrc/device/launch.h
--- a/cpu-ray-tracer_amd/csrc/device/launch.h
+++ b/cpu-ray-tracer_amd/csrc/device/launch.h
@@ -29,7 +29,8 @@
 size_t crt_pool_scratch_bytes_per_window(uint32_t tileCount);
 hipError_t crt_launch_render_pool(const crt::Scene* sc, void* slab, void* facScratch, crt::Counters* counters, unsigned long long* tileClocks, const uint32_t* tileOrder, uint32_t tileFirst,
     uint32_t tileStride, uint32_t tileCount, uint32_t tilesX, uint32_t sppFirst, uint32_t frames, uint32_t passes, int collectStats, uint32_t rankFirst, uint32_t waveFrames,
-    const uint32_t* waveTab, uint32_t tabBlocks, uint32_t longFrames, uint32_t* tileCost, unsigned long long* launchClk, hipStream_t stream);
+    const uint32_t* waveTab, uint32_t tabBlocks, uint32_t longFrames, uint32_t* tileCost, unsigned long long* launchClk,
+    const uint8_t* tileClass , hipStream_t stream);
 uint32_t crt_pool_lds_bytes(uint32_t stackDepth, uint32_t streams);
 int crt_debug_pool_stamps(unsigned long long* out, int reset);
 int crt_debug_pool_density(unsigned long long* out, int reset);
diff --git a/cpu-ray-tracer_amd/csrc/device/layout.h b/cpu-ray-tracer_amd/csrc/device/layout.h
--- a/cpu-ray-tracer_amd/csrc/device/layout.h
+++ b/cpu-ray-tracer_amd/csrc/device/layout.h
@@ -93,6 +93,9 @@
     for (int k = 0; k < 3; k++) { s.primRight[k] = s.topRight[k] - s.topLeft[k]; s.primDown[k] = s.bottomLeft[k] - s.topLeft[k]; }
 }
 
+constexpr uint32_t kTileNoLight = 1u, kTileNoFloor = 2u, kTileNoTree = 4u;
+constexpr uint32_t kTileSky = kTileNoLight | kTileNoFloor | kTileNoTree;
+
 struct Counters { unsigned long long v[8]; };
 
 struct alignas(16) RefitPlanRec { uint32_t pair, child[2], pad; };
diff --git a/cpu-ray-tracer_amd/csrc/device/render_pool.hip b/cpu-ray-tracer_amd/csrc/device/render_pool.hip
--- a/cpu-ray-tracer_amd/csrc/device/render_pool.hip
+++ b/cpu-ray-tracer_amd/csrc/device/render_pool.hip
@@ -71,7 +71,7 @@
                                                              unsigned long long* __restrict__ tileClocks, const uint32_t* __restrict__ tileOrder,
                                                              uint32_t tileFirst, uint32_t tileStride, uint32_t tileCount, uint32_t tilesX,
                                                              uint32_t sppFirst, uint32_t frames, uint32_t passes, uint32_t groups, uint32_t waveFrames, const uint32_t* __restrict__ waveTab, uint32_t tabBlocks, uint32_t longFrames,
-                                                             uint32_t rankFirst, uint32_t* __restrict__ tileCost, unsigned long long* __restrict__ launchClk)
+                                                             uint32_t rankFirst, uint32_t* __restrict__ tileCost, unsigned long long* __restrict__ launchClk, const uint8_t* __restrict__ tileClass)
 {
     extern __shared__ uint32_t lds[];
     const uint32_t lane = threadIdx.x;
@@ -97,6 +97,12 @@
     const uint32_t nStreams = nOwn < (uint32_t)S ? nOwn : (uint32_t)S;
     const uint32_t tile = tileFirst + tl * tileStride;
     const uint32_t tx = tile % tilesX, ty = tile / tilesX;
+#ifdef CRT_NO_TILE_CLASS
+    constexpr uint32_t tcls = 0u;
+#else
+    const uint32_t tcls = tileClass ? __builtin_amdgcn_readfirstlane((uint32_t)tileClass[tl]) : 0u;
+#endif
+    const bool skyTile = tcls == kTileSky;
     const char* __restrict__ geom = sc.geom;
     float* __restrict__ fac = facScratch + (size_t)blockIdx.x * (15u * (uint32_t)S);
 
@@ -142,14 +148,17 @@
 #else
         constexpr bool PRIM = decltype(primary)::value;
 #endif
+        constexpr bool FROM_CAM = decltype(primary)::value;
+        const bool sky = FROM_CAM && skyTile;
+        const bool noLight = FROM_CAM && (tcls & kTileNoLight) != 0u, noFloor = FROM_CAM && (tcls & kTileNoFloor) != 0u, noTree = FROM_CAM && (tcls & kTileNoTree) != 0u;
         f3 D = v, rD = v; Hit nh; nh.t = 1e34f; nh.u = 0; nh.v = 0; nh.objIdx = -1; nh.triIdx = -1;
         uint32_t ncur = kRefDone, pend = 0u;
         if (act) {
             const float inv = rcp_exact(sqrt_exact(dot3(v, v)));
             D = norm ? v * inv : v;
-            rD = rcp_exact3(D);
             cn.rays++;
-            {
+            if (!sky) {
+                rD = rcp_exact3(D);
                 const kernarg_f lp = scene_floats(offsetof(Scene, lightInvT));
                 const kernarg_f ax = scene_floats(offsetof(Scene, lightAxis));
                 LightFloor lf;
@@ -162,9 +171,11 @@
                     constexpr size_t pl = (offsetof(Scene, primLight) - offsetof(Scene, lightInvT)) / 4;
                     lf.preOy = lp[pl]; lf.preOx = lp[pl + 1]; lf.preOz = lp[pl + 2]; lf.preNum = lp[pl + 3];
                 }
-                hit_light_floor<PRIM>(lf, O, D, nh);
-            }
-            if (sc.rootIsPair) {
+                hit_light_floor<PRIM>(lf, O, D, nh, noLight, noFloor);
+            }
+            if (noTree) {
+                if (COUNT) { if (KIND == 0) cn.interior++; else cn.tlas++; }
+            } else if (sc.rootIsPair) {
                 const kernarg_f rp = scene_floats(offsetof(Scene, rootPair));
                 const rec4 a0 = {rp[0], rp[1], rp[2], rp[3]}, a1 = {rp[4], rp[5], rp[6], rp[7]};
                 const rec4 b0 = {rp[8], rp[9], rp[10], rp[11]}, b1 = {rp[12], rp[13], rp[14], rp[15]};
@@ -185,23 +196,31 @@
                 if (COUNT) { if (KIND == 0) cn.interior++; else cn.tlas++; }
             } else ncur = sc.rootRef16;
             if (COUNT && KIND == 0 && (ncur & kRef16TagMask) == 0u && ncur != kRefDone) cn.leaf++;
-            stf[F_OX * S + s] = O.x; stf[F_OY * S + s] = O.y; stf[F_OZ * S + s] = O.z;
+            if (!sky) {
+                stf[F_OX * S + s] = O.x; stf[F_OY * S + s] = O.y; stf[F_OZ * S + s] = O.z;
+                stf[F_RX * S + s] = rD.x; stf[F_RY * S + s] = rD.y; stf[F_RZ * S + s] = rD.z;
+                stf[F_T * S + s] = nh.t;
+                st[F_CUR * S + s] = ncur; st[F_PEND * S + s] = pend;
+            }
             stf[F_DX * S + s] = D.x; stf[F_DY * S + s] = D.y; stf[F_DZ * S + s] = D.z;
-            stf[F_RX * S + s] = rD.x; stf[F_RY * S + s] = rD.y; stf[F_RZ * S + s] = rD.z;
-            stf[F_T * S + s] = nh.t;
             st[F_SEED * S + s] = seed; st[F_META * S + s] = meta | ((uint32_t)(nh.objIdx + 1) << kMetaObjShift);
-            st[F_CUR * S + s] = ncur; st[F_PEND * S + s] = pend;
-        }
-        const uint32_t depth = (meta >> kMetaDepthShift) & 7u;
+        }
         const uint64_t mAct = __builtin_amdgcn_ballot_w64(act);
-        const uint64_t mW = mAct & __builtin_amdgcn_ballot_w64(ncur != kRefDone);
-        const uint64_t mStop = __builtin_amdgcn_ballot_w64((uint32_t)(nh.objIdx + 1) <= 1u) | __builtin_amdgcn_ballot_w64((int)depth >= sc.depthLimit);
-        const uint64_t mE = mAct & ~mW & mStop, mB = mAct & ~mW & ~mStop;
+        uint64_t mW = 0ull, mE = mAct, mB = 0ull;
+        if (!sky) {
+            const uint32_t depth = (meta >> kMetaDepthShift) & 7u;
+            mW = mAct & __builtin_amdgcn_ballot_w64(ncur != kRefDone);
+            const uint64_t mStop = __builtin_amdgcn_ballot_w64((uint32_t)(nh.objIdx + 1) <= 1u) | __builtin_amdgcn_ballot_w64((int)depth >= sc.depthLimit);
+            mE = mAct & ~mW & mStop; mB = mAct & ~mW & ~mStop;
+        }
         CRT_DENS(20, __popcll(mAct)); CRT_DENS(19, __popcll(mW));
-        if (lane_in(mW)) qRdy[(rdyT + rank_in(mW)) & kQueueMask] = (uint8_t)s;
+        if (!sky) {
+            if (lane_in(mW)) qRdy[(rdyT + rank_in(mW)) & kQueueMask] = (uint8_t)s;
+            if (lane_in(mB)) qBnc[(bncT + rank_in(mB)) & kQueueMask] = (uint8_t)s;
+            rdyT += (uint32_t)__popcll(mW); bncT += (uint32_t)__popcll(mB);
+        }
         if (lane_in(mE)) qEnd[(endT + rank_in(mE)) & kQueueMask] = (uint8_t)s;
-        if (lane_in(mB)) qBnc[(bncT + rank_in(mB)) & kQueueMask] = (uint8_t)s;
-        rdyT += (uint32_t)__popcll(mW); endT += (uint32_t)__popcll(mE); bncT += (uint32_t)__popcll(mB);
+        endT += (uint32_t)__popcll(mE);
     };
     auto world_ray = [&]() {
         tO = mk3(stf[F_OX * S + sid], stf[F_OY * S + sid], stf[F_OZ * S + sid]);
@@ -410,7 +429,7 @@
 #pragma unroll
                 for (int k = 0; k < 5; k++) {
                     fk[3 * k] = fk[3 * k + 1] = fk[3 * k + 2] = 0.0f;
-                    if (ended && depth > k) {
+                    if (!skyTile) if (ended && depth > k) {
 #pragma unroll
                         for (int j = 0; j < 3; j++) fk[3 * k + j] = __hip_atomic_load(fac + (3 * k + j) * S + s, __ATOMIC_RELAXED, __HIP_MEMORY_SCOPE_AGENT);
                     }
@@ -477,9 +496,11 @@
                 CRT_PSTAMP(e2); CRT_PACC(3, e1, e2);
                 if (ended) {
                     f3 L = miss ? tex_unpack(skyTexel) : ((depth >= sc.depthLimit) ? mk3(0, 0, 0) : mk3(24, 24, 22));
+                    if (!skyTile) {
 #pragma unroll
-                    for (int k = 4; k >= 0; k--)
-                        if (depth > k) L = mk3(fk[3 * k], fk[3 * k + 1], fk[3 * k + 2]) * L;
+                        for (int k = 4; k >= 0; k--)
+                            if (depth > k) L = mk3(fk[3 * k], fk[3 * k + 1], fk[3 * k + 2]) * L;
+                    }
                     slab[sampleAt] = make_float4(L.x, L.y, L.z, 0.0f);
                 }
 #ifdef CRT_POOL_STAMPS
@@ -679,7 +700,7 @@
 extern "C" hipError_t crt_launch_render_pool(const crt::Scene* sc, void* slab, void* facScratch, crt::Counters* counters, unsigned long long* tileClocks, const uint32_t* tileOrder,
                                              uint32_t tileFirst, uint32_t tileStride, uint32_t tileCount, uint32_t tilesX, uint32_t sppFirst,
                                              uint32_t frames, uint32_t passes, int collectStats, uint32_t rankFirst, uint32_t waveFrames, const uint32_t* waveTab, uint32_t tabBlocks, uint32_t longFrames,
-                                             uint32_t* tileCost, unsigned long long* launchClk, hipStream_t stream)
+                                             uint32_t* tileCost, unsigned long long* launchClk, const uint8_t* tileClass, hipStream_t stream)
 {
     if (tileCount == 0 || frames == 0) return hipSuccess;
     if (!sc->ref16ok) return hipErrorInvalidValue;
@@ -698,7 +719,7 @@
       (void)hipMemsetAsync(buf, 0, (size_t)grid.x * 24, stream); g_timelineHost = buf; g_timelineCount = grid.x; }
 #endif
     const uint32_t ldsBytes = crt_pool_lds_bytes(sc->stackDepth, S);
-#define CRT_LAUNCH(K, C, SS) hipLaunchKernelGGL((crt::render_pool_kernel<K, C, SS>), grid, block, ldsBytes, stream, *sc, (float4*)slab, (float*)facScratch, counters, tileClocks, tileOrder, tileFirst, tileStride, tileCount, tilesX, sppFirst, frames, passes, groups, wf, waveTab, tabBlocks, longFrames, rankFirst, tileCost, launchClk)
+#define CRT_LAUNCH(K, C, SS) hipLaunchKernelGGL((crt::render_pool_kernel<K, C, SS>), grid, block, ldsBytes, stream, *sc, (float4*)slab, (float*)facScratch, counters, tileClocks, tileOrder, tileFirst, tileStride, tileCount, tilesX, sppFirst, frames, passes, groups, wf, waveTab, tabBlocks, longFrames, rankFirst, tileCost, launchClk, tileClass)
 #define CRT_LAUNCH_S(K, C) do { if (S == 64u) CRT_LAUNCH(K, C, 64); else CRT_LAUNCH(K, C, CRT_POOL_STREAMS); } while (0)
     if (sc->kind == 0) { if (collectStats) CRT_LAUNCH_S(0, true); else CRT_LAUNCH_S(0, false); }
     else { if (collectStats) CRT_LAUNCH_S(1, true); else CRT_LAUNCH_S(1, false); }
diff --git a/cpu-ray-tracer_amd/csrc/device/tile_class.h b/cpu-ray-tracer_amd/csrc/device/tile_class.h
--- /dev/null
+++ b/cpu-ray-tracer_amd/csrc/device/tile_class.h
@@ -0,0 +1,88 @@
+#pragma once
+#include <cmath>
+#include <cstring>
+#include "layout.h"
+
+namespace crt {
+
+inline void classify_tiles(const Scene& s, int W, int H, uint32_t tilesX, uint32_t tileFirst, uint32_t tileStride, uint32_t tileCount, uint8_t* cls)
+{
+    if (tileCount == 0) return;
+    memset(cls, 0, tileCount);
+    if (W <= 0 || H <= 0 || tilesX == 0) return;
+    const double cam[3] = {s.camPos[0], s.camPos[1], s.camPos[2]};
+    double TL[3], R[3], Dn[3];
+    for (int k = 0; k < 3; k++) { TL[k] = s.topLeft[k]; R[k] = (double)s.topRight[k] - s.topLeft[k]; Dn[k] = (double)s.bottomLeft[k] - s.topLeft[k]; }
+    const bool wantTree = s.rootIsPair != 0, wantFloor = s.floorAxisY != 0, wantLight = s.lightAxis != 0;
+    if (!wantTree && !wantFloor && !wantLight) return;
+
+    double mag = 0; bool finite = true;
+    auto see = [&](double x) { if (!std::isfinite(x)) finite = false; else if (std::fabs(x) > mag) mag = std::fabs(x); };
+    for (int k = 0; k < 3; k++) { see(cam[k]); see(TL[k]); see(s.topRight[k]); see(s.bottomLeft[k]); see(TL[k] + R[k] + Dn[k]); }
+    if (wantTree) for (int c = 0; c < 2; c++) for (int k = 0; k < 3; k++) { see(s.rootPair[8 * c + k]); see(s.rootPair[8 * c + 4 + k]); }
+    if (wantLight) { see(s.lightInvT[3]); see(s.lightInvT[7]); see(s.lightInvT[11]); see(s.lightSize); see(s.primLight[0]); see(s.primLight[1]); see(s.primLight[2]); }
+    if (wantFloor) { see(s.floorD); see(s.primFloor); }
+    see(s.invW); see(s.invH);
+    const double rr = R[0] * R[0] + R[1] * R[1] + R[2] * R[2], dd = Dn[0] * Dn[0] + Dn[1] * Dn[1] + Dn[2] * Dn[2], rd = R[0] * Dn[0] + R[1] * Dn[1] + R[2] * Dn[2];
+    if (!finite || !(rr > 0) || !(dd > 0)) return;
+    const double invW = s.invW, invH = s.invH;
+    const double step = std::fmin(std::sqrt(rr) * std::fabs(invW), std::sqrt(dd) * std::fabs(invH));
+    if (!(step >= std::ldexp(mag, -16)) || !(invW > 0) || !(invH > 0)) return;
+    const double tau = std::ldexp(mag, -18);
+
+    auto ray = [&](double px, double py, double v[3]) { for (int k = 0; k < 3; k++) v[k] = TL[k] + (px * invW) * R[k] + (py * invH) * Dn[k] - cam[k]; };
+
+    bool tree = wantTree; double bx0 = 1e300, bx1 = -1e300, by0 = 1e300, by1 = -1e300;
+    if (tree) {
+        const double N[3] = {R[1] * Dn[2] - R[2] * Dn[1], R[2] * Dn[0] - R[0] * Dn[2], R[0] * Dn[1] - R[1] * Dn[0]};
+        const double num = (TL[0] - cam[0]) * N[0] + (TL[1] - cam[1]) * N[1] + (TL[2] - cam[2]) * N[2];
+        const double det = rr * dd - rd * rd;
+        if (!(det > 1e-12 * rr * dd) || num == 0) tree = false;
+        for (int c = 0; c < 2 && tree; c++)
+            for (int i = 0; i < 8 && tree; i++) {
+                double d[3];
+                for (int k = 0; k < 3; k++) d[k] = (double)s.rootPair[8 * c + ((i >> k) & 1 ? 4 : 0) + k] - cam[k];
+                const double den = d[0] * N[0] + d[1] * N[1] + d[2] * N[2];
+                const double t = den != 0 ? num / den : -1;
+                if (!(t > 0) || !(t <= 16)) { tree = false; break; }
+                double Q[3]; for (int k = 0; k < 3; k++) Q[k] = cam[k] + t * d[k] - TL[k];
+                const double qr = Q[0] * R[0] + Q[1] * R[1] + Q[2] * R[2], qd = Q[0] * Dn[0] + Q[1] * Dn[1] + Q[2] * Dn[2];
+                const double px = (qr * dd - qd * rd) / det / invW, py = (qd * rr - qr * rd) / det / invH;
+                if (!std::isfinite(px) || !std::isfinite(py)) { tree = false; break; }
+                bx0 = std::fmin(bx0, px); bx1 = std::fmax(bx1, px); by0 = std::fmin(by0, py); by1 = std::fmax(by1, py);
+            }
+    }
+
+    const double fnum = s.primFloor;
+    const bool floorOk = wantFloor && fnum != 0;
+    const double lOy = s.primLight[0], lOx = s.primLight[1], lOz = s.primLight[2], lsize = s.lightSize;
+    const bool lightOk = wantLight && lOy != 0;
+
+    for (uint32_t i = 0; i < tileCount; i++) {
+        const uint32_t tile = tileFirst + i * tileStride;
+        const double x0 = 16.0 * (tile % tilesX) - 1.0, x1 = x0 + 18.0, y0 = 16.0 * (tile / tilesX) - 1.0, y1 = y0 + 18.0;
+        double v[4][3];
+        ray(x0, y0, v[0]); ray(x1, y0, v[1]); ray(x0, y1, v[2]); ray(x1, y1, v[3]);
+        double vyMin = v[0][1], vyMax = v[0][1];
+        for (int j = 1; j < 4; j++) { vyMin = std::fmin(vyMin, v[j][1]); vyMax = std::fmax(vyMax, v[j][1]); }
+        const bool up = vyMin >= tau, down = vyMax <= -tau;
+        uint8_t b = 0;
+        if (tree && (x1 < bx0 || x0 > bx1 || y1 < by0 || y0 > by1)) b |= kTileNoTree;
+        if (floorOk && (fnum > 0 ? up : down)) b |= kTileNoFloor;
+        if (lightOk) {
+            double q[4], qMax = 0, vMax = 0;
+            for (int j = 0; j < 4; j++) { q[j] = -v[j][1] / lOy; qMax = std::fmax(qMax, std::fabs(q[j])); vMax = std::fmax(vMax, std::fmax(std::fabs(v[j][0]), std::fabs(v[j][2]))); }
+            const double m = std::ldexp(qMax * (std::fabs(lOx) + std::fabs(lOz) + std::fabs(lsize)) + vMax, -16), qTau = tau / std::fabs(lOy);
+            bool behind = true, xHi = true, xLo = true, zHi = true, zLo = true;
+            for (int j = 0; j < 4; j++) {
+                behind = behind && q[j] <= -qTau;
+                xHi = xHi && v[j][0] - (lsize - lOx) * q[j] >= m; xLo = xLo && v[j][0] + (lsize + lOx) * q[j] <= -m;
+                zHi = zHi && v[j][2] - (lsize - lOz) * q[j] >= m; zLo = zLo && v[j][2] + (lsize + lOz) * q[j] <= -m;
+            }
+            if (std::isfinite(m) && (behind || xHi || xLo || zHi || zLo)) b |= kTileNoLight;
+        }
+        cls[i] = b;
+    }
+}
+
+}
```

Result: faster. 31340 Mrays/s, median of 6 (+2.6%).
